# wendongbi/Bridged-GNN

Hardware: AMD Instinct MI355X
Metric: aggregated_edges_per_sec_ktgnn_fwd (higher is better)
Workload: dtype f32; 1 GPU; C4 synthetic bridged graph (local) N=1000000 E'=20991058, 2-layer KT-GNN eval fwd F=128 hidden=128 C=2; parallelism=single, execution=eager launches

## Files before the change

### bridged_gnn_amd/_lib.py

```python
import ctypes as C
import os

import torch

_HERE = os.path.dirname(os.path.abspath(__file__))
SO_PATH = os.path.join(_HERE, "csrc", "libbgnn_hip.so")
_lib = None

_P, _I64, _I32, _F32, _SZ, _INT = C.c_void_p, C.c_int64, C.c_int32, C.c_float, C.c_size_t, C.c_int

SIGNATURES = {
    "bgnn_version": (_INT, []),
    "bgnn_source_hash": (C.c_char_p, []),
    "bgnn_error_string": (C.c_char_p, [_INT]),
    "bgnn_csr_workspace_bytes": (_SZ, [_I64, _I64]),
    "bgnn_build_dst_csr": (_INT, [_P, _I64, _I64, _INT, _P, _P, _P, _P, _P, _SZ, _P]),
    "bgnn_domain_sums_f64": (_INT, [_P, _I64, _I32, _I64, _P, _P, _P]),
    "bgnn_domain_sums_workspace_bytes": (_SZ, [_I32]),
    "bgnn_domain_sums_ws_f64": (_INT, [_P, _I64, _I32, _I64, _P, _P, _P, _SZ, _P]),
    "bgnn_domain_delta_f32": (_INT, [_P, _I32, _P, _P]),
    "bgnn_adaptedconv_transform_f32": (_INT, [_P, _I64, _I32, _I64, _P, _P, _I32, _I32, _P, _P, _P, _P,
                                               _P, _P, _P, _P, _I64, _I64, _P, _P]),
    "bgnn_adaptedconv_transform_sums_f32": (_INT, [_P, _I64, _I32, _I64, _P, _P, _I32, _I32, _P, _P, _P, _P,
                                                    _P, _P, _P, _P, _I64, _I64, _I64, _I64, _P, _P]),
    "bgnn_adaptedconv_transform_need_f32": (_INT, [_P, _I64, _I32, _I64, _P, _P, _I32, _I32, _P, _P, _P, _P,
                                                    _P, _P, _P, _P, _I64, _I64, _P, _P, _P]),
    "bgnn_classifier_stage_f32": (_INT, [_P, _I64, _I32, _I64, _P, _P, _I32, _I32, _P, _P, _P, _P, _P, _P, _P, _P, _I64, _I64,
                                          _P, _P, _I32, _INT, _P, _P, _P, _P, _P, _P]),
    "bgnn_linear_narrow_transform_f32": (_INT, [_P, _I64, _I32, _I64, _P, _P, _I32, _INT, _P, _P, _P, _P, _P, _P]),
    "bgnn_narrow_transform_finish_f32": (_INT, [_P, _I64, _P, _P, _I32, _P, _P, _P, _P, _P, _P, _I64, _P, _P]),
    "bgnn_gram_workspace_bytes": (C.c_size_t, [_I32, _I32]),
    "bgnn_gram_f32": (_INT, [_P, _I64, _I32, _P, _I64, _I32, _I64, _P, _P, C.c_size_t, _P]),
    "bgnn_transform_bwd_prep_workspace_bytes": (C.c_size_t, [_I64, _I32]),
    "bgnn_transform_bwd_prep_f32": (_INT, [_P, _I64, _I64, _I32, _P, _P, _I64, _I32, _P, _P, _P, _P, _P, _P, _I32, _I64, _P, _I64, _P, _P, C.c_size_t, _P]),
    "bgnn_bn_acc_doubles": (_I64, [_I32]),
    "bgnn_bn_relu_dropout_f32": (_INT, [_P, _I64, _I32, _I64, _P, _P, _F32, _INT, _F32, C.c_uint64, _P, _F32, _P, _P, _P, _I64, _P, _P]),
    "bgnn_bn_relu_dropout_bwd_f32": (_INT, [_P, _P, _I64, _I32, _I64, _I64, _P, _P, _P, _F32, _INT, _F32, C.c_uint64, _P, _P, _I64, _P, _P]),
    "bgnn_bn_colstats_f32": (_INT, [_P, _I64, _I32, _I64, _P, _P]),
    "bgnn_bn_apply_rows_f32": (_INT, [_P, _I64, _I32, _I64, _P, _I64, _P, _P, _F32, _INT, _F32, C.c_uint64, _P, _P, _I64, _F32, _P, _P, _P, _I64, _P]),
    "bgnn_bn_bwd_reduce_rows_f32": (_INT, [_P, _P, _I64, _I32, _I64, _I64, _P, _I64, _P, _P, _F32, _INT, _F32, C.c_uint64, _P, _P, _I64, _P, _P]),
    "bgnn_bn_bwd_apply_rows_f32": (_INT, [_P, _P, _I64, _I32, _I64, _I64, _P, _P, _I64, _P, _P, _F32, _INT, _F32, C.c_uint64, _P, _P, _I64, _P, _I64, _P]),
    "bgnn_transform_bwd_consts_f32": (_INT, [_P, _P, _P, _P, _P, _I32, _I32, _P, _P, _P, _P]),
    "bgnn_transform_bwd_finish_f32": (_INT, [_P, _P, _P, _P, _P, _P, _P, _I32, _I32, _I32, _P, _P, _P, _P, _P, _P, _P, _I64, _P]),
    "bgnn_rowdot_f32": (_INT, [_P, _I64, _I64, _I32, _P, _I64, _I32, _P, _P]),
    "bgnn_linear_f32": (_INT, [_P, _I64, _I32, _I64, _P, _P, _I32, _INT, _P, _P, _P, _I64, _P]),
    "bgnn_adaptedconv_aggregate_f32": (_INT, [_P, _P, _I64, _P, _P, _P, _P, _P, _I64, _I64, _I32, _F32,
                                               _P, _I64, _P, _P, _P, _INT, _P, _INT, _I64, _I32, _P, _P, _P]),
    "bgnn_adaptedconv_aggregate_bounded_f32": (_INT, [_P, _P, _I64, _P, _P, _P, _P, _P, _I64, _I64, _I32, _F32,
                                                       _P, _I64, _P, _P, _P, _INT, _P, _INT, _I64, _I32, _P, _P, _I64, _I32, _P]),
    "bgnn_aggregate_hub_workspace_bytes": (C.c_size_t, [_I64, _I32, _I64]),
    "bgnn_adaptedconv_aggregate_hub_f32": (_INT, [_P, _P, _I64, _P, _P, _P, _P, _P, _I64, _I32, _F32, _P, _I64, _P, _P, _INT, _P, _I32, _P,
                                                   _P, _I32, _P, _I64, _P, _P, _P, _I64, _P, _P, C.c_size_t, _P]),
    "bgnn_adaptedconv_aggregate_bwd_f32": (_INT, [_P, _P, _I64, _P, _P, _P, _P, _P, _I64, _I64, _I32, _F32,
                                                   _P, _I64, _P, _P, _I64, _P, _P, _P, _P, _P]),
    "bgnn_aggregate_bwd_pull_workspace_bytes": (C.c_size_t, [_I64, _I64, _I64]),
    "bgnn_adaptedconv_aggregate_bwd_pull_f32": (_INT, [_P, _P, _I64, _P, _P, _P, _P, _P, _P, _P, _P, _I64, _I64, _I32, _F32,
                                                        _P, _I64, _P, _P, _I64, _P, _P, _P, _P, _P, C.c_size_t, _P]),
    "bgnn_aggregate_bwd_pull_hub_workspace_bytes": (C.c_size_t, [_I64, _I64, _I64, _I64, _I64]),
    "bgnn_adaptedconv_aggregate_bwd_pull_hub_f32": (_INT, [_P, _P, _I64, _P, _P, _P, _P, _P, _P, _P, _P, _I64, _I64, _I32, _F32,
                                                            _P, _I64, _P, _P, _I64, _P, _P, _P, _P, _I32,
                                                            _P, _I64, _P, _P, _P, _I64, _P, _I64, _P, _P, _P, _I64, _P, C.c_size_t, _P]),
    "bgnn_aggregate_heads_bwd_workspace_bytes": (C.c_size_t, [_I64, _I64, _I32]),
    "bgnn_adaptedconv_aggregate_heads_bwd_f32": (_INT, [_P, _P, _P, _P, _P, _P, _P, _P, _P, _P, _I64, _I64, _I32, _I32, _F32,
                                                         _P, _P, _P, _INT, _P, _P, _P, _P, _P, C.c_size_t, _P]),
    "bgnn_aggregate_heads_bwd_hub_workspace_bytes": (C.c_size_t, [_I64, _I64, _I32, _I64, _I64]),
    "bgnn_adaptedconv_aggregate_heads_bwd_hub_f32": (_INT, [_P, _P, _P, _P, _P, _P, _P, _P, _P, _I64, _I64, _I32, _I32, _F32,
                                                             _P, _P, _P, _INT, _P, _P, _P, _P, _I32,
                                                             _P, _I64, _P, _P, _P, _I64, _P, _I64, _P, _P, _P, _I64, _P, C.c_size_t, _P]),
    "bgnn_adaptedconv_aggregate_heads_wide_f32": (_INT, [_P, _P, _I64, _P, _P, _P, _P, _P, _I64, _I32, _I32, _F32, _P, _P, _P]),
    "bgnn_aggregate_heads_wide_bwd_workspace_bytes": (C.c_size_t, [_I64, _I32, _I64]),
    "bgnn_adaptedconv_aggregate_heads_wide_bwd_f32": (_INT, [_P, _P, _I64, _P, _P, _P, _P, _P, _P, _P, _I64, _I32, _I32, _F32,
                                                              _P, _P, _P, _P, _P, _P, _P, _P, C.c_size_t, _P]),
    "bgnn_l2_normalize_rows_f32": (_INT, [_P, _I64, _I32, _F32, _P, _P]),
    "bgnn_topk_workspace_bytes": (_SZ, [_I64, _I64, _I32]),
    "bgnn_cosine_topk_f32": (_INT, [_P, _P, _I64, _I64, _I32, _I32, _INT, _P, _P, _P, _P, _SZ, _P]),
    "bgnn_mlp_pair_topk_f32": (_INT, [_P, _P, _P, _P, _P, _F32, _I64, _I64, _I32, _I32, _INT, _P, _P, _P,
                                       _P, _SZ, _P]),
    "bgnn_topk_edges_i64": (_INT, [_P, _I64, _I32, _I64, _I64, _P, _P]),
    "bgnn_topk_edges_coalesced_workspace_bytes": (_SZ, [_I64, _I32]),
    "bgnn_topk_edges_coalesced_i64": (_INT, [_P, _I64, _I32, _I64, _I64, _I64, _P, _P, _SZ, _P]),
    "bgnn_gather_rows_f32": (_INT, [_P, _I64, _I64, _P, _I64, _I32, _P, _I64, _P]),
    "bgnn_coalesce_workspace_bytes": (_SZ, [_I64]),
    "bgnn_coalesce_i64": (_INT, [_P, _I64, _I64, _P, _P, _SZ, _P]),
    "bgnn_sage_mean_aggregate_f32": (_INT, [_P, _I64, _I64, _P, _I64, _P, _P, _I64, _I32, _INT, _INT, _F32, C.c_uint64, _P,
                                             _P, _I64, _P]),
    "bgnn_sage_mean_aggregate_rows_f32": (_INT, [_P, _I64, _I64, _P, _I64, _P, _P, _I64, _I32, _INT, _INT, _F32, C.c_uint64, _P,
                                                  _P, _P, _I64, _P]),
    "bgnn_rows_segment_add_f32": (_INT, [_P, _I64, _I64, _P, _P, _P, _I64, _I32, _INT, _P, _I64, _I64, _P]),
    "bgnn_pair_mlp_workspace_bytes": (_SZ, [_I64]),
    "bgnn_pair_mlp_stats_f32": (_INT, [_P, _I64, _I64, _P, _I64, _I64, _P, _P, _I64, _F32, _P, _P, _P, _P, _SZ, _P]),
    "bgnn_pair_mlp_loss_f32": (_INT, [_P, _I64, _I64, _P, _I64, _I64, _P, _P, _P, _I64, _P, _P, _P, _P, _P, _F32, _P, _P, _P, _P,
                                       _SZ, _P]),
    "bgnn_pair_mlp_segsum_f32": (_INT, [_P, _I64, _I64, _P, _I64, _I64, _P, _P, _P, _I64, _P, _P, _P, _P, _P, _P, _F32, _P, _I64, _P]),
    "bgnn_pair_mlp_eval_f32": (_INT, [_P, _I64, _I64, _P, _I64, _I64, _P, _P, _P, _I64, _P, _P, _P, _P, _P, _P, _P, _SZ, _P]),
    "bgnn_pair_mlp_count_workspace_bytes": (_SZ, [_I64, _I64]),
    "bgnn_pair_mlp_count_f32": (_INT, [_P, _I64, _I64, _P, _I64, _I64, _P, _I64, _P, _I64, _P, _P, _P, _P, _P, _P, _P, _P, _SZ, _P]),
    "bgnn_pair_cos_loss_workspace_bytes": (_SZ, [_I64]),
    "bgnn_pair_cos_count_workspace_bytes": (_SZ, [_I64, _I64]),
    "bgnn_pair_cos_loss_f32": (_INT, [_P, _I64, _I64, _P, _I64, _I64, _P, _P, _P, _I64, _P, _P, _P, _P, _SZ, _P]),
    "bgnn_pair_cos_segsum_f32": (_INT, [_P, _I64, _I64, _P, _P, _P, _I64, _P, _I64, _P, _I64, _P]),
    "bgnn_pair_cos_count_f32": (_INT, [_P, _I64, _I64, _P, _I64, _I64, _P, _I64, _P, _I64, _P, _P, _P, _P, _SZ, _P]),
    "bgnn_sage_mean_aggregate_bwd_workspace_bytes": (_SZ, [_I64, _I32]),
# ... 138 lines not shown
```

### bridged_gnn_amd/csrc/bgnn_aggregate.hip

```cpp
#include <cstdlib>
#include "bgnn_common.h"

namespace {

struct AggParams {
  const float* h_t2s;
  const float* h_s2t;
  int64_t ldh;
  const float* a_t2s;
  const float* a_s2t;
  const int32_t* rowptr;
  const int32_t* col;
  const uint8_t* mask;
  int64_t row_begin;
  int64_t row_end;
  int32_t D;
  float slope;
  float* out;
  int64_t ldo;
  float* alpha;
  const float* ep_scale;
  const float* ep_shift;
  int ep_relu;
  unsigned int* tile_queue;
  double* colsum;
  int32_t heads;
  float* state_ms;
  int mode;
  int64_t park_begin;
  int tq_chunk;
  int tq_interleave;
  int xcd_segments;
  const int32_t* vrow_node;
  const int32_t* vrow_bounds;
  int64_t n_vrows;
  float* vout; float* vms;
  int32_t hub_threshold;
  const char* tbl_base;
  uint32_t tbl_bytes, off_t2s, off_s2t;
  int32_t gather_hint;
  uint32_t dead_off;
};

__device__ __forceinline__ float leaky(float v, float slope) { return v > 0.f ? v : v * slope; }

template <int LF, int EP, int U>
__global__ __launch_bounds__(256) void agg_kernel(AggParams p) {
  constexpr int GL = LF * EP;
  constexpr int GPW = 64 / GL;
  constexpr int RPB = 4 * GPW;
  const int lane = threadIdx.x & 63;
  const int wave = threadIdx.x >> 6;
  const int g = lane / GL;
  const int lg = lane % GL;
  const int sub = lg / LF;
  const int f0 = (lg % LF) * 4;
  const bool fvalid = f0 < p.D;

  const int64_t ntiles = ((p.row_end - p.row_begin) * p.heads + RPB - 1) / RPB;
  bgnn::XcdRange tr = bgnn::xcd_pos_range(ntiles);
  __shared__ float red[2][LF * 4 + 1];
  if (p.colsum != nullptr) {
    for (int t = threadIdx.x; t < 2 * (LF * 4 + 1); t += 256) (&red[0][0])[t] = 0.f;
    __syncthreads();
  }

  __shared__ unsigned int dyn_tile;
  const int64_t xbase = tr.begin - (blockIdx.x / 8);
  int64_t tile = tr.begin - tr.step;
  int64_t chunk_left = 0;
  const int TQ_CHUNK = p.tq_chunk;
  for (;;) {
    if (p.tile_queue != nullptr) {
      if (chunk_left == 0) {
        __syncthreads();
        if (threadIdx.x == 0) dyn_tile = atomicAdd(&p.tile_queue[blockIdx.x % 8], 1u);
        __syncthreads();
        tile = xbase + (int64_t)dyn_tile * TQ_CHUNK;
        chunk_left = TQ_CHUNK;
      } else {
        tile += 1;
      }
      --chunk_left;
    } else {
      tile += tr.step;
    }
    if (tile >= tr.end) break;
    const int64_t gt = bgnn::xcd_tile_of(tile, ntiles);
    if (gt < 0) continue;
    const int64_t i = p.row_begin * p.heads + gt * RPB + wave * GPW + g;
    const bool rvalid = i < p.row_end * p.heads;
    const int64_t ic = rvalid ? i : p.row_begin * p.heads;
    const int64_t node = ic / p.heads;
    const int head = (int)(ic - node * p.heads);
    const bool dom_s = p.mask[node] != 0;
// ... 76 lines not shown
    }

#pragma unroll
    for (int off = LF; off < GL; off <<= 1) {
      const float m2 = __shfl_xor(m, off);
      const float s2 = __shfl_xor(s, off);
      float4 b;
      b.x = __shfl_xor(acc.x, off); b.y = __shfl_xor(acc.y, off);
      b.z = __shfl_xor(acc.z, off); b.w = __shfl_xor(acc.w, off);
      const float mn = fmaxf(m, m2);
      const float c1 = (m == mn) ? 1.f : __expf(m - mn);
      const float c2 = (m2 == mn) ? 1.f : __expf(m2 - mn);
      s = s * c1 + s2 * c2;
      acc.x = acc.x * c1 + b.x * c2; acc.y = acc.y * c1 + b.y * c2;
      acc.z = acc.z * c1 + b.z * c2; acc.w = acc.w * c1 + b.w * c2;
      m = mn;
    }

    if (p.mode == 1 && node >= p.park_begin) {
      if (rvalid && sub == 0) {
        if (lg == 0) { p.state_ms[2 * i] = m; p.state_ms[2 * i + 1] = s; }
        if (f0 < p.ldo) *reinterpret_cast<float4*>(p.out + i * p.ldo + f0) = fvalid ? acc : make_float4(0.f, 0.f, 0.f, 0.f);
      }
      continue;
    }
    const float inv = 1.f / (s + 1e-16f);
    if (p.alpha != nullptr && (lg % LF) == 0) {
      for (int32_t e = beg + sub; e < end; e += EP) p.alpha[e] = __expf(p.alpha[e] - m) * inv;
    }
    if (rvalid && sub == 0 && f0 < p.ldo) {
      float4 o = make_float4(acc.x * inv, acc.y * inv, acc.z * inv, acc.w * inv);
      if (p.ep_scale != nullptr) {
        float sc4[4], sh4[4];
#pragma unroll
        for (int c = 0; c < 4; ++c) {
          const bool ok = f0 + c < p.D;
          sc4[c] = ok ? p.ep_scale[f0 + c] : 0.f;
          sh4[c] = ok ? p.ep_shift[f0 + c] : 0.f;
        }
        o.x = fmaf(o.x, sc4[0], sh4[0]); o.y = fmaf(o.y, sc4[1], sh4[1]);
        o.z = fmaf(o.z, sc4[2], sh4[2]); o.w = fmaf(o.w, sc4[3], sh4[3]);
      }
      if (p.ep_relu) { o.x = fmaxf(o.x, 0.f); o.y = fmaxf(o.y, 0.f); o.z = fmaxf(o.z, 0.f); o.w = fmaxf(o.w, 0.f); }
      if (!fvalid) o = make_float4(0.f, 0.f, 0.f, 0.f);
      *reinterpret_cast<float4*>(p.out + i * p.ldo + f0) = o;
      if (p.colsum != nullptr) {
        float* r = red[dom_s ? 0 : 1];
        unsafeAtomicAdd(&r[f0], o.x); unsafeAtomicAdd(&r[f0 + 1], o.y);
        unsafeAtomicAdd(&r[f0 + 2], o.z); unsafeAtomicAdd(&r[f0 + 3], o.w);
        if (lg == 0) unsafeAtomicAdd(&r[LF * 4], 1.f);
      }
    }
  }
  if (p.colsum != nullptr) {
    __syncthreads();
    for (int t = threadIdx.x; t < 2 * (LF * 4 + 1); t += 256) {
      const int d = t / (LF * 4 + 1), c = t % (LF * 4 + 1);
      const double sum = (double)red[d][c];
      if (c == LF * 4) unsafeAtomicAdd(&p.colsum[2 * p.ldo + d], sum);
      else if (c < p.ldo) unsafeAtomicAdd(&p.colsum[d * p.ldo + c], sum);
    }
  }
}

typedef float f2 __attribute__((ext_vector_type(2)));

template <int CTRL>
__device__ __forceinline__ int dpp_movi(int x) { return __builtin_amdgcn_update_dpp(0, x, CTRL, 0xF, 0xF, true); }

template <int K>
__device__ __forceinline__ float quad_bcast(float x) { return bgnn::dpp_mov<K * 0x55>(x); }
template <int K>
__device__ __forceinline__ int quad_bcasti(int x) { return dpp_movi<K * 0x55>(x); }

template <int CTRL>
__device__ __forceinline__ float bfly(bool hi_side, float t_lo, float t_hi) {
  const float keep = hi_side ? t_hi : t_lo;
  const float send = hi_side ? t_lo : t_hi;
  return keep + bgnn::dpp_mov<CTRL>(send);
}

template <int LF, int U>
__global__ __launch_bounds__(256) void agg_wide_kernel(AggParams p) {
  static_assert(LF == 16 || LF == 32 || LF == 64, "wide rows only");
  static_assert(U == 4 || U == 8, "U");
  constexpr int GPW = 64 / LF;
  constexpr int RPB = 4 * GPW;
  const int lane = threadIdx.x & 63;
  const int wave = threadIdx.x >> 6;
  const int g = lane / LF;
  const int lg = lane % LF;
  const int f0 = lg * 4;
  const bool fvalid = f0 < p.D;
  const int f0c = fvalid ? f0 : 0;
  const int k = lane & (U - 1);
  const bool b0 = lane & 1, b1 = lane & 2, b2 = lane & 4;

  const int64_t nrows_all = (p.row_end - p.row_begin) * p.heads + p.n_vrows;
  const int64_t ntiles = (nrows_all + RPB - 1) / RPB;
  bgnn::XcdRange tr = bgnn::xcd_tile_range(ntiles);
  __shared__ float red[2][LF * 4 + 1];
  if (p.colsum != nullptr) {
    for (int t = threadIdx.x; t < 2 * (LF * 4 + 1); t += 256) (&red[0][0])[t] = 0.f;
    __syncthreads();
  }
  __shared__ unsigned int dyn_tile;
// ... 169 lines not shown
      if constexpr (U == 8) {
        { const float w = quad_bcast<0>(ph); BGNN_ACC(4, w) }
        { const float w = quad_bcast<1>(ph); BGNN_ACC(5, w) }
        { const float w = quad_bcast<2>(ph); BGNN_ACC(6, w) }
        { const float w = quad_bcast<3>(ph); BGNN_ACC(7, w) }
      }
#undef BGNN_ACC
      m = mn;
    };
    auto slot_id = [&](int32_t e) { return e < end ? p.col[e] : -1; };

    int32_t e = beg + k;
    int32_t myid = slot_id(e);
    for (int32_t it = 0; it < niter; ++it) {
      float4 v[U];
      issue(v, myid);
      const int32_t nextid = slot_id(e + U);
      update(v, myid, e);
      e += U;
      myid = nextid;
    }
    s += bgnn::dpp_mov<0xB1>(s);
    s += bgnn::dpp_mov<0x4E>(s);
    if constexpr (U == 8) s += bgnn::dpp_mov<0x124>(s);

    if (virt || (p.mode == 1 && node >= p.park_begin)) {
      if (rvalid) {
        if (lg == 0) { msbase[2 * i] = m; msbase[2 * i + 1] = s; }
        if (f0 < p.ldo)
          *reinterpret_cast<float4*>(obase + i * p.ldo + f0) =
              fvalid ? make_float4(acc01.x, acc01.y, acc23.x, acc23.y) : make_float4(0.f, 0.f, 0.f, 0.f);
      }
      continue;
    }
    const float inv = 1.f / (s + 1e-16f);
    if (p.alpha != nullptr && lg < U) {
      for (int32_t e2 = beg + lg; e2 < end; e2 += U) p.alpha[e2] = __expf(p.alpha[e2] - m) * inv;
    }
    if (rvalid && f0 < p.ldo) {
      float4 o = make_float4(acc01.x * inv, acc01.y * inv, acc23.x * inv, acc23.y * inv);
      if (p.ep_scale != nullptr) {
        o.x = fmaf(o.x, sc4[0], sh4[0]); o.y = fmaf(o.y, sc4[1], sh4[1]);
        o.z = fmaf(o.z, sc4[2], sh4[2]); o.w = fmaf(o.w, sc4[3], sh4[3]);
      }
      if (p.ep_relu) { o.x = fmaxf(o.x, 0.f); o.y = fmaxf(o.y, 0.f); o.z = fmaxf(o.z, 0.f); o.w = fmaxf(o.w, 0.f); }
      if (!fvalid) o = make_float4(0.f, 0.f, 0.f, 0.f);
      *reinterpret_cast<float4*>(p.out + i * p.ldo + f0) = o;
      if (p.colsum != nullptr) {
        if (dom_s) { cs_s.x += o.x; cs_s.y += o.y; cs_s.z += o.z; cs_s.w += o.w; n_s += 1.f; }
        else       { cs_t.x += o.x; cs_t.y += o.y; cs_t.z += o.z; cs_t.w += o.w; n_t += 1.f; }
      }
    }
  }
  if (p.colsum != nullptr) {
    unsafeAtomicAdd(&red[0][f0], cs_s.x); unsafeAtomicAdd(&red[0][f0 + 1], cs_s.y);
    unsafeAtomicAdd(&red[0][f0 + 2], cs_s.z); unsafeAtomicAdd(&red[0][f0 + 3], cs_s.w);
    unsafeAtomicAdd(&red[1][f0], cs_t.x); unsafeAtomicAdd(&red[1][f0 + 1], cs_t.y);
    unsafeAtomicAdd(&red[1][f0 + 2], cs_t.z); unsafeAtomicAdd(&red[1][f0 + 3], cs_t.w);
    if (lg == 0) { unsafeAtomicAdd(&red[0][LF * 4], n_s); unsafeAtomicAdd(&red[1][LF * 4], n_t); }
    __syncthreads();
    for (int t = threadIdx.x; t < 2 * (LF * 4 + 1); t += 256) {
      const int d = t / (LF * 4 + 1), c = t % (LF * 4 + 1);
      const double sum = (double)red[d][c];
      if (c == LF * 4) unsafeAtomicAdd(&p.colsum[2 * p.ldo + d], sum);
      else if (c < p.ldo) unsafeAtomicAdd(&p.colsum[d * p.ldo + c], sum);
    }
  }
}

typedef unsigned int u32x4_t __attribute__((ext_vector_type(4)));

template <int CTRL>
__device__ __forceinline__ uint32_t dpp_movu(uint32_t x) { return (uint32_t)__builtin_amdgcn_update_dpp(0, (int)x, CTRL, 0xF, 0xF, true); }

template <int LF, bool ALPHA>
__global__ __launch_bounds__(256) void agg_wide_fast_kernel(AggParams p) {
  static_assert(LF == 16 || LF == 32 || LF == 64, "wide rows only");
  constexpr int U = 4;
  constexpr int GPW = 64 / LF;
  constexpr int RPB = 4 * GPW;
  const int lane = threadIdx.x & 63;
  const int wave = threadIdx.x >> 6;
  const int g = lane / LF;
  const int lg = lane % LF;
  const int f0 = lg * 4;
  const bool fvalid = f0 < p.D;
  const int f0c = fvalid ? f0 : 0;
  const int k = lane & (U - 1);
  const bool b0 = lane & 1, b1 = lane & 2;

  const int32_t row0 = (int32_t)p.row_begin, row1 = (int32_t)p.row_end;
  const int32_t ntiles = (row1 - row0 + RPB - 1) / RPB;
  __shared__ float red[2][LF * 4 + 1];
  if (p.colsum != nullptr) {
    for (int t = threadIdx.x; t < 2 * (LF * 4 + 1); t += 256) (&red[0][0])[t] = 0.f;
    __syncthreads();
  }
  __shared__ unsigned int dyn_tile;
  const uint32_t nstride = (uint32_t)(p.ldh * 4);
  const uint32_t ostride = (uint32_t)(p.ldo * 4);
  const __amdgpu_buffer_rsrc_t rt = __builtin_amdgcn_make_buffer_rsrc(const_cast<char*>(p.tbl_base), (short)0, (int)p.tbl_bytes, 0x00020000);
  const __amdgpu_buffer_rsrc_t ro = __builtin_amdgcn_make_buffer_rsrc(p.out, (short)0, (int)((uint32_t)row1 * ostride), 0x00020000);
  const f2 sl = {p.slope, p.slope};
  float sc4[4] = {0.f, 0.f, 0.f, 0.f}, sh4[4] = {0.f, 0.f, 0.f, 0.f};
  if (p.ep_scale != nullptr) {
#pragma unroll
// ... 132 lines not shown
    int32_t nw = __builtin_amdgcn_readlane(niter, 0);
    if constexpr (LF <= 32) nw = max(nw, __builtin_amdgcn_readlane(niter, 32));
    if constexpr (LF <= 16) nw = max(nw, max(__builtin_amdgcn_readlane(niter, 16), __builtin_amdgcn_readlane(niter, 48)));
    int32_t e = beg + k;
    bool ok = e < end;
    uint32_t myoff = p.dead_off;
    if (nw > 0) myoff = row_off((uint32_t)p.col[max(min(e, end - 1), 0)], ok);
    for (int32_t it = 0; it < nw; ++it) {
      float4 v[U];
      issue(v, myoff);
      const int32_t e_cur = e;
      e += U;
      const bool ok2 = e < end;
      uint32_t nextid = load_id(e);
      update(v, ok, e_cur);
      ok = ok2;
      take_id(nextid);
      myoff = row_off(nextid, ok);
    }
    s += bgnn::dpp_mov<0xB1>(s);
    s += bgnn::dpp_mov<0x4E>(s);

    const float inv = 1.f / (s + 1e-16f);
    if constexpr (ALPHA) {
      if (lg < U) {
        for (int32_t e2 = beg + lg; e2 < end; e2 += 4 * U) {
          float a[4];
#pragma unroll
          for (int j = 0; j < 4; ++j) a[j] = e2 + j * U < end ? p.alpha[e2 + j * U] : 0.f;
#pragma unroll
          for (int j = 0; j < 4; ++j)
            if (e2 + j * U < end) p.alpha[e2 + j * U] = __expf(a[j] - m) * inv;
        }
      }
    }
    if (rvalid && f0 < p.ldo) {
      float4 o = make_float4(acc01.x * inv, acc01.y * inv, acc23.x * inv, acc23.y * inv);
      if (p.ep_scale != nullptr) {
        o.x = fmaf(o.x, sc4[0], sh4[0]); o.y = fmaf(o.y, sc4[1], sh4[1]);
        o.z = fmaf(o.z, sc4[2], sh4[2]); o.w = fmaf(o.w, sc4[3], sh4[3]);
      }
      if (p.ep_relu) { o.x = fmaxf(o.x, 0.f); o.y = fmaxf(o.y, 0.f); o.z = fmaxf(o.z, 0.f); o.w = fmaxf(o.w, 0.f); }
      if (!fvalid) o = make_float4(0.f, 0.f, 0.f, 0.f);
      __builtin_amdgcn_raw_buffer_store_b128(__builtin_bit_cast(u32x4_t, o), ro, __umul24((uint32_t)i0, ostride) + (uint32_t)f0 * 4u, 0, 0);
      if (p.colsum != nullptr) {
        const float ws = dom_s ? 1.f : 0.f, wt = dom_s ? 0.f : 1.f;
        const f2 ws2 = {ws, ws}, wt2 = {wt, wt}, o01 = {o.x, o.y}, o23 = {o.z, o.w};
        cs_s01 = __builtin_elementwise_fma(o01, ws2, cs_s01); cs_s23 = __builtin_elementwise_fma(o23, ws2, cs_s23);
        cs_t01 = __builtin_elementwise_fma(o01, wt2, cs_t01); cs_t23 = __builtin_elementwise_fma(o23, wt2, cs_t23);
        n_s += ws; n_t += wt;
      }
    }
  }
  if (p.colsum != nullptr) {
    unsafeAtomicAdd(&red[0][f0], cs_s01.x); unsafeAtomicAdd(&red[0][f0 + 1], cs_s01.y);
    unsafeAtomicAdd(&red[0][f0 + 2], cs_s23.x); unsafeAtomicAdd(&red[0][f0 + 3], cs_s23.y);
    unsafeAtomicAdd(&red[1][f0], cs_t01.x); unsafeAtomicAdd(&red[1][f0 + 1], cs_t01.y);
    unsafeAtomicAdd(&red[1][f0 + 2], cs_t23.x); unsafeAtomicAdd(&red[1][f0 + 3], cs_t23.y);
    if (lg == 0) { unsafeAtomicAdd(&red[0][LF * 4], n_s); unsafeAtomicAdd(&red[1][LF * 4], n_t); }
    __syncthreads();
    for (int t = threadIdx.x; t < 2 * (LF * 4 + 1); t += 256) {
      const int d = t / (LF * 4 + 1), c = t % (LF * 4 + 1);
      const double sum = (double)red[d][c];
      if (c == LF * 4) unsafeAtomicAdd(&p.colsum[2 * p.ldo + d], sum);
      else if (c < p.ldo) unsafeAtomicAdd(&p.colsum[d * p.ldo + c], sum);
    }
  }
}

template <int HEADS, int EP, int U>
__global__ __launch_bounds__(256) void agg_heads_lanes_kernel(AggParams p) {
  constexpr int GL = EP * HEADS, GPW = 64 / GL, RPB = 4 * GPW;
  const int lane = threadIdx.x & 63, wave = threadIdx.x >> 6;
  const int g = lane / GL, lg = lane % GL;
  const int sub = lg / HEADS, h = lg % HEADS;
  const bool lane_on = g < GPW;
  const int64_t ntiles = (p.row_end - p.row_begin + p.n_vrows + RPB - 1) / RPB;
  bgnn::XcdRange tr = bgnn::xcd_pos_range(ntiles);
  const int64_t rs = (int64_t)HEADS * p.ldh;
  for (int64_t pos = tr.begin; pos < tr.end; pos += tr.step) {
    const int64_t tile = bgnn::xcd_tile_of(pos, ntiles);
    if (tile < 0) continue;
    const int64_t i = p.row_begin + tile * RPB + wave * GPW + g;
    const bool in_range = lane_on && i < p.row_end + p.n_vrows;
    const bool virt = in_range && i >= p.row_end;
    const int64_t vix = virt ? i - p.row_end : 0;
    const int64_t ic = in_range ? i : p.row_begin;
    const int64_t node = virt ? (int64_t)p.vrow_node[vix] : ic;
    const bool dom_s = p.mask[node] != 0;
    const float* __restrict__ H = dom_s ? p.h_t2s : p.h_s2t;
    const float* __restrict__ av = dom_s ? p.a_t2s : p.a_s2t;
    int32_t beg = in_range ? (virt ? p.vrow_bounds[2 * vix] : p.rowptr[ic]) : 0;
    int32_t end = in_range ? (virt ? p.vrow_bounds[2 * vix + 1] : p.rowptr[ic + 1]) : 0;
    const bool hub = !virt && p.hub_threshold > 0 && end - beg >= p.hub_threshold;
    const bool rvalid = in_range && !hub;
    const int64_t oi = virt ? vix : i;
    float* __restrict__ obase = virt ? p.vout : p.out;
    float* __restrict__ msbase = virt ? p.vms : p.state_ms;
    if (hub) { beg = 0; end = 0; }
    float4 a4;
    a4.x = av[h * p.D];
    a4.y = p.D > 1 ? av[h * p.D + 1] : 0.f;
    a4.z = p.D > 2 ? av[h * p.D + 2] : 0.f;
    a4.w = p.D > 3 ? av[h * p.D + 3] : 0.f;
    const float4 hi = *reinterpret_cast<const float4*>(H + node * rs + h * p.ldh);
    float4 acc = make_float4(0.f, 0.f, 0.f, 0.f);
// ... 349 lines not shown
    r.y = p.D > 1 ? r.y - mx - lse : 0.f;
    r.z = p.D > 2 ? r.z - mx - lse : 0.f;
    r.w = p.D > 3 ? r.w - mx - lse : 0.f;
  }
  *reinterpret_cast<float4*>(p.out + (node * p.heads + h) * p.ldo) = r;
}

static int dispatch_aggregate(const AggParams& p, hipStream_t st, int64_t table_rows = 0) {
  const int32_t D = p.D, heads = p.heads;
  if (heads == 3 && D <= 4 && p.ldh == 4 && p.ldo == 4) return launch_heads<3, 2, 4>(p, st);
  if (heads == 2 && D <= 4 && p.ldh == 4 && p.ldo == 4) return launch_heads<2, 2, 4>(p, st);
  const int nv = (D + 3) / 4;
  if (nv <= 1) return launch<1, 4, 4>(p, st);
  if (nv <= 2) return launch<2, 2, 4>(p, st);
  if (nv <= 4) return launch<4, 1, 8>(p, st);
  if (nv <= 8) return launch<8, 1, 4>(p, st);
  const bool wide_ok = p.slope >= 0.f && p.slope <= 1.f && (int64_t)heads * p.ldh * 4 < (int64_t)1 << 32;
  if (wide_ok) {
    AggParams q = p;
    if (fast_plan(q, table_rows)) {
      if (q.alpha != nullptr) {
        if (nv <= 16) return launch_wide_fast<16, true>(q, st);
        if (nv <= 32) return launch_wide_fast<32, true>(q, st);
        return launch_wide_fast<64, true>(q, st);
      }
      if (nv <= 16) return launch_wide_fast<16, false>(q, st);
      if (nv <= 32) return launch_wide_fast<32, false>(q, st);
      return launch_wide_fast<64, false>(q, st);
    }
    if (nv <= 16) return launch_wide<16, 4>(p, st);
    if (nv <= 32) return launch_wide<32, 4>(p, st);
    return launch_wide<64, 4>(p, st);
  }
  if (nv <= 16) return launch<16, 1, 8>(p, st);
  if (nv <= 32) return launch<32, 1, 4>(p, st);
  return launch<64, 1, 4>(p, st);
}

static bool hub_capable(int32_t D, int64_t ldh, int64_t ldo, int32_t heads, float slope) {
  if ((heads == 3 || heads == 2) && D <= 4 && ldh == 4 && ldo == 4) return true;
  const int nv = (D + 3) / 4;
  return heads == 1 && nv > 8 && slope >= 0.f && slope <= 1.f && ldh * 4 < (int64_t)1 << 32;
}

}

static int aggregate_impl(const float* h_t2s, const float* h_s2t, int64_t ldh,
                          const float* a_t2s, const float* a_s2t,
                          const int32_t* rowptr, const int32_t* col, const uint8_t* mask,
                          int64_t row_begin, int64_t row_end, int32_t D, float negative_slope,
                          float* out, int64_t ldo, float* alpha_opt,
                          const float* ep_scale_opt, const float* ep_shift_opt, int ep_relu,
                          float* state_ms_opt, int part, int64_t park_begin, int32_t heads,
                          double* colsum_opt, uint32_t* tile_queue_opt, int64_t table_rows, int32_t gather_hint, void* stream) {
  if (colsum_opt && heads != 1) return BGNN_E_SHAPE;
  if (part == 1 && (park_begin < row_begin || park_begin > row_end)) return BGNN_E_SHAPE;
  if (part < 0 || part > 3 || (part != 0 && (!state_ms_opt || alpha_opt))) return BGNN_E_NULL;
  if (part == 3 && !((heads == 3 || heads == 2) && D <= 4 && ldh == 4 && ldo == 4)) return BGNN_E_SHAPE;
  if (heads < 1 || heads > 8 || (heads > 1 && (alpha_opt || ep_scale_opt))) return BGNN_E_SHAPE;
  if (ep_relu < 0 || ep_relu > 2) return BGNN_E_SHAPE;
  if (ep_relu == 2 && !((heads == 3 || heads == 2) && D <= 4 && ldh == 4 && ldo == 4)) return BGNN_E_SHAPE;
  if (!h_t2s || !h_s2t || !a_t2s || !a_s2t || !rowptr || !col || !mask || !out) return BGNN_E_NULL;
  if (row_begin < 0 || row_end < row_begin || D <= 0 || D > 256 || ldh < D || ldo < D) return BGNN_E_SHAPE;
  if ((ldh & 3) || (ldo & 3) || !bgnn_aligned16(h_t2s) || !bgnn_aligned16(h_s2t) || !bgnn_aligned16(out))
    return BGNN_E_ALIGN;
  if ((ep_scale_opt == nullptr) != (ep_shift_opt == nullptr)) return BGNN_E_NULL;
  if (row_end == row_begin) return 0;
  AggParams p{h_t2s, h_s2t, ldh, a_t2s, a_s2t, rowptr, col, mask, row_begin, row_end, D, negative_slope,
              out, ldo, alpha_opt, ep_scale_opt, ep_shift_opt, ep_relu, tile_queue_opt, colsum_opt, heads, state_ms_opt, part,
              park_begin, 4};
  p.gather_hint = gather_hint;
  hipStream_t st = (hipStream_t)stream;
  if (tile_queue_opt) {
    hipError_t e = bgnn_zero_async(tile_queue_opt, 8 * sizeof(uint32_t), st);
    if (e != hipSuccess) return (int)e;
  }
  return dispatch_aggregate(p, st, table_rows);
}

extern "C" int bgnn_adaptedconv_aggregate_f32(const float* h_t2s, const float* h_s2t, int64_t ldh,
                                              const float* a_t2s, const float* a_s2t,
                                              const int32_t* rowptr, const int32_t* col, const uint8_t* mask,
                                              int64_t row_begin, int64_t row_end, int32_t D, float negative_slope,
                                              float* out, int64_t ldo, float* alpha_opt,
                                              const float* ep_scale_opt, const float* ep_shift_opt, int ep_relu,
                                              float* state_ms_opt, int part, int64_t park_begin, int32_t heads,
                                              double* colsum_opt, uint32_t* tile_queue_opt, void* stream) {
  return aggregate_impl(h_t2s, h_s2t, ldh, a_t2s, a_s2t, rowptr, col, mask, row_begin, row_end, D, negative_slope, out, ldo, alpha_opt,
                        ep_scale_opt, ep_shift_opt, ep_relu, state_ms_opt, part, park_begin, heads, colsum_opt, tile_queue_opt, 0, 0, stream);
}

extern "C" int bgnn_adaptedconv_aggregate_bounded_f32(const float* h_t2s, const float* h_s2t, int64_t ldh,
                                                      const float* a_t2s, const float* a_s2t,
                                                      const int32_t* rowptr, const int32_t* col, const uint8_t* mask,
                                                      int64_t row_begin, int64_t row_end, int32_t D, float negative_slope,
                                                      float* out, int64_t ldo, float* alpha_opt,
                                                      const float* ep_scale_opt, const float* ep_shift_opt, int ep_relu,
                                                      float* state_ms_opt, int part, int64_t park_begin, int32_t heads,
                                                      double* colsum_opt, uint32_t* tile_queue_opt, int64_t table_rows, int32_t gather_hint,
                                                      void* stream) {
  if (table_rows < row_end || gather_hint < 0 || gather_hint > 2) return BGNN_E_SHAPE;
  return aggregate_impl(h_t2s, h_s2t, ldh, a_t2s, a_s2t, rowptr, col, mask, row_begin, row_end, D, negative_slope, out, ldo, alpha_opt,
                        ep_scale_opt, ep_shift_opt, ep_relu, state_ms_opt, part, park_begin, heads, colsum_opt, tile_queue_opt, table_rows, gather_hint, stream);
}

extern "C" size_t bgnn_aggregate_hub_workspace_bytes(int64_t n_segments, int32_t heads, int64_t ldo) {
  const size_t nv = (size_t)(n_segments > 0 ? n_segments : 0), h = (size_t)(heads > 0 ? heads : 1);
  return bgnn_align_up(sizeof(float) * nv * h * (size_t)(ldo > 0 ? ldo : 0), 256) + bgnn_align_up(sizeof(float) * 2 * nv * h, 256) + 256;
}

extern "C" int bgnn_adaptedconv_aggregate_hub_f32(const float* h_t2s, const float* h_s2t, int64_t ldh,
                                                  const float* a_t2s, const float* a_s2t,
                                                  const int32_t* rowptr, const int32_t* col, const uint8_t* mask,
                                                  int64_t N, int32_t D, float negative_slope, float* out, int64_t ldo,
                                                  const float* ep_scale_opt, const float* ep_shift_opt, int ep_relu,
                                                  float* state_ms_opt, int32_t heads, double* colsum_opt,
                                                  uint32_t* tile_queue_opt, int32_t hub_threshold, const int32_t* hub_rows,
                                                  int64_t n_hubs, const int32_t* hub_seg_ptr, const int32_t* seg_bounds,
                                                  const int32_t* seg_node, int64_t n_segments, float* alpha_opt,
                                                  void* ws, size_t ws_bytes, void* stream) {
  if (!h_t2s || !h_s2t || !a_t2s || !a_s2t || !rowptr || !col || !mask || !out) return BGNN_E_NULL;
  if (alpha_opt && heads != 1) return BGNN_E_SHAPE;
  if (n_hubs > 0 && (!hub_rows || !hub_seg_ptr || !seg_bounds || !seg_node || !ws)) return BGNN_E_NULL;
  if (N < 0 || D <= 0 || D > 256 || ldh < D || ldo < D || (ldh & 3) || (ldo & 3) || hub_threshold < 2 || n_hubs < 0 || n_segments < n_hubs)
    return BGNN_E_SHAPE;
  if (!hub_capable(D, ldh, ldo, heads, negative_slope)) return BGNN_E_SHAPE;
  if (colsum_opt && heads != 1) return BGNN_E_SHAPE;
  if (heads > 1 && ep_scale_opt) return BGNN_E_SHAPE;
  if (ep_relu < 0 || ep_relu > 2 || (ep_relu == 2 && heads == 1)) return BGNN_E_SHAPE;
  if ((ep_scale_opt == nullptr) != (ep_shift_opt == nullptr)) return BGNN_E_NULL;
  if (!bgnn_aligned16(h_t2s) || !bgnn_aligned16(h_s2t) || !bgnn_aligned16(out) || (ws && !bgnn_aligned16(ws))) return BGNN_E_ALIGN;
  if (n_hubs > 0 && ws_bytes < bgnn_aggregate_hub_workspace_bytes(n_segments, heads, ldo)) return BGNN_E_WORKSPACE;
  if (N == 0) return 0;
  hipStream_t st = (hipStream_t)stream;
  const int part = (state_ms_opt && heads > 1) ? 3 : 0;
  AggParams p{h_t2s, h_s2t, ldh, a_t2s, a_s2t, rowptr, col, mask, 0, N, D, negative_slope,
              out, ldo, alpha_opt, ep_scale_opt, ep_shift_opt, ep_relu, tile_queue_opt, colsum_opt, heads, state_ms_opt, part,
              0, 4};
  p.hub_threshold = n_hubs > 0 ? hub_threshold : 0;
  if (tile_queue_opt) {
    hipError_t e = bgnn_zero_async(tile_queue_opt, 8 * sizeof(uint32_t), st);
    if (e != hipSuccess) return (int)e;
  }
  float* part_acc = n_hubs > 0 ? (float*)ws : nullptr;
  float* part_ms = n_hubs > 0 ? (float*)((char*)ws + bgnn_align_up(sizeof(float) * (size_t)n_segments * (size_t)heads * (size_t)ldo, 256)) : nullptr;
  if (n_hubs > 0) {
    p.vrow_node = seg_node; p.vrow_bounds = seg_bounds; p.n_vrows = n_segments; p.vout = part_acc; p.vms = part_ms;
  }
  int rc = dispatch_aggregate(p, st, N);
  if (rc || n_hubs == 0) return rc;
  HubMergeParams mp{hub_rows, hub_seg_ptr, n_hubs, part_acc, part_ms, mask, D, ldo, heads, out, ep_scale_opt, ep_shift_opt,
                    ep_relu, colsum_opt, part == 3 ? state_ms_opt : nullptr, alpha_opt, rowptr};
  if (heads > 1) {
    hipLaunchKernelGGL(hub_merge_heads_kernel, dim3((unsigned)((n_hubs * heads + 255) / 256)), dim3(256), 0, st, mp);
  } else {
    const int nvs = (D + 3) / 4;
    int64_t grid = n_hubs < 2048 ? n_hubs : 2048;
    if (nvs <= 16) hipLaunchKernelGGL(hub_merge_wide_kernel<16>, dim3((unsigned)((grid + 15) / 16)), dim3(256), 0, st, mp);
    else if (nvs <= 32) hipLaunchKernelGGL(hub_merge_wide_kernel<32>, dim3((unsigned)((grid + 7) / 8)), dim3(256), 0, st, mp);
    else hipLaunchKernelGGL(hub_merge_wide_kernel<64>, dim3((unsigned)((grid + 3) / 4)), dim3(256), 0, st, mp);
  }
  BGNN_LAUNCH_CHECK();
  return 0;
}

#ifdef BGNN_TUNING
extern "C" int bgnn_tune_reset_counters(void* stream) { (void)stream; return 0; }
extern "C" int bgnn_tune_aggregate(const float* h_t2s, const float* h_s2t, int64_t ldh, const float* a_t2s,
                                   const float* a_s2t, const int32_t* rowptr, const int32_t* col, const uint8_t* mask,
                                   int64_t row_begin, int64_t row_end, int32_t D, float slope, float* out, int64_t ldo,
                                   int variant, uint32_t* tile_queue, void* stream) {
  AggParams p{h_t2s, h_s2t, ldh, a_t2s, a_s2t, rowptr, col, mask, row_begin, row_end, D, slope,
              out, ldo, nullptr, nullptr, nullptr, 0, tile_queue, nullptr, 1, nullptr, 0};
  hipStream_t st = (hipStream_t)stream;
  if (tile_queue && bgnn_zero_async(tile_queue, 32, st) != hipSuccess) return -1;
  switch (variant) {
    case 40: return launch_wide<32, 4>(p, st);
    case 41: return launch_wide<32, 8>(p, st);
    case 42: return launch_wide<16, 4>(p, st);
    case 43: return launch_wide<16, 8>(p, st);
    case 44: return launch_wide<64, 4>(p, st);
    case 45: return launch_wide<64, 8>(p, st);
    case 0: return launch<32, 1, 4>(p, st);
    case 1: return launch<32, 1, 8>(p, st);
    case 2: return launch<32, 2, 4>(p, st);
    case 3: return launch<32, 2, 2>(p, st);
    case 4: return launch<32, 1, 2>(p, st);
    case 5: return launch<32, 2, 8>(p, st);
    case 6: return launch<64, 1, 4>(p, st);
    case 10: return launch<1, 8, 2>(p, st);
    case 11: return launch<1, 4, 4>(p, st);
    case 12: return launch<1, 2, 4>(p, st);
    case 13: return launch<1, 1, 4>(p, st);
    case 14: return launch<1, 1, 8>(p, st);
    case 15: return launch<1, 4, 2>(p, st);
    case 16: return launch<1, 2, 8>(p, st);
    case 17: return launch<1, 16, 2>(p, st);
    case 20: return launch<16, 2, 4>(p, st);
    case 21: return launch<16, 1, 4>(p, st);
    case 22: return launch<16, 4, 2>(p, st);
    case 23: return launch<16, 1, 8>(p, st);
    case 30: return launch<8, 2, 4>(p, st);
    case 31: return launch<8, 4, 2>(p, st);
    case 32: return launch<8, 1, 4>(p, st);
    case 33: return launch<8, 8, 2>(p, st);
    default: return BGNN_E_RANGE;
  }
}
#endif
```

### bridged_gnn_amd/csrc/bgnn_transform.hip

```cpp
#include <cstdlib>
#include <type_traits>
#include "bgnn_common.h"
#include "bgnn_transform_params.h"

using bgnn_tf::GemmParams;
using bgnn_tf::MAXH;
using bgnn_tf::f32x16;
using bgnn_tf::tanh_fast;

namespace {

constexpr int DS_NT = 1024;
__global__ __launch_bounds__(DS_NT) void domain_sums_kernel(const float* __restrict__ x, int64_t N, int32_t Din,
                                                          int64_t ldx, const uint8_t* __restrict__ mask,
                                                          double* __restrict__ sums, double* __restrict__ part) {
  if (part != nullptr) sums = part + (int64_t)blockIdx.x * (2 * Din + 2);
  const int nc4 = Din >> 2;
  const int cw = nc4 < 256 ? nc4 : 256;
  const int rl = DS_NT / cw;
  const int tid = threadIdx.x;
  const int cl = tid % cw, r0 = tid / cw;
  const bool active = r0 < rl;
  const int64_t rows_per_block = (N + gridDim.x - 1) / gridDim.x;
  const int64_t rb = blockIdx.x * rows_per_block;
  const int64_t re = min(rb + rows_per_block, N);
  extern __shared__ double sh[];
  for (int cb = 0; cb < nc4; cb += cw) {
    const int c4 = cb + cl;
    const bool cok = active && c4 < nc4;
    double as[4] = {0, 0, 0, 0}, at[4] = {0, 0, 0, 0};
    if (cok) {
      int64_t r = rb + r0;
      for (; r + 3 * rl < re; r += 4 * rl) {
        float4 v[4];
        bool m[4];
#pragma unroll
        for (int u = 0; u < 4; ++u) {
          v[u] = *reinterpret_cast<const float4*>(x + (r + u * rl) * ldx + c4 * 4);
          m[u] = mask[r + u * rl] != 0;
        }
#pragma unroll
        for (int u = 0; u < 4; ++u) {
          const double a = v[u].x, b = v[u].y, c = v[u].z, d = v[u].w;
          if (m[u]) { as[0] += a; as[1] += b; as[2] += c; as[3] += d; }
          else      { at[0] += a; at[1] += b; at[2] += c; at[3] += d; }
        }
      }
      for (; r < re; r += rl) {
        const float4 v = *reinterpret_cast<const float4*>(x + r * ldx + c4 * 4);
        if (mask[r]) { as[0] += v.x; as[1] += v.y; as[2] += v.z; as[3] += v.w; }
        else         { at[0] += v.x; at[1] += v.y; at[2] += v.z; at[3] += v.w; }
      }
    }
    if (active) {
#pragma unroll
      for (int e = 0; e < 4; ++e) { sh[((r0 * 2 + 0) * cw + cl) * 4 + e] = as[e]; sh[((r0 * 2 + 1) * cw + cl) * 4 + e] = at[e]; }
    }
    __syncthreads();
    if (cok && r0 == 0) {
      for (int q = 1; q < rl; ++q)
#pragma unroll
// ... 720 lines not shown
  hipStream_t st = (hipStream_t)stream;
  if (ws != nullptr) {
    if (ws_bytes < sizeof(double) * 256 * (size_t)ncol) return BGNN_E_WORKSPACE;
    int64_t grid = (N + 255) / 256;
    if (grid > 256) grid = 256;
    hipLaunchKernelGGL(domain_sums_kernel, dim3((unsigned)grid), dim3(DS_NT), sizeof(double) * rl * 2 * cw * 4, st,
                       x, N, Din, ldx, mask, sums_io, (double*)ws);
    BGNN_LAUNCH_CHECK();
    hipLaunchKernelGGL(domain_sums_reduce_kernel, dim3((unsigned)((ncol + 255) / 256)), dim3(256), 0, st,
                       (const double*)ws, (int)grid, ncol, sums_io);
    BGNN_LAUNCH_CHECK();
    return 0;
  }
  static const int64_t rpb = [] { const char* e = getenv("BGNN_DS_ROWS"); return e ? atoll(e) : 2048ll; }();
  int64_t grid = (N + rpb - 1) / rpb;
  static const int64_t gcap = [] { const char* e = getenv("BGNN_DS_GRID"); return e ? atoll(e) : 256ll; }();
  if (grid > gcap) grid = gcap;
  if (grid < 1) grid = 1;
  hipLaunchKernelGGL(domain_sums_kernel, dim3((unsigned)grid), dim3(DS_NT), sizeof(double) * rl * 2 * cw * 4, st,
                     x, N, Din, ldx, mask, sums_io, (double*)nullptr);
  BGNN_LAUNCH_CHECK();
  return 0;
}

extern "C" int bgnn_domain_sums_f64(const float* x, int64_t N, int32_t Din, int64_t ldx, const uint8_t* mask,
                                    double* sums_io, void* stream) {
  return domain_sums_impl(x, N, Din, ldx, mask, sums_io, nullptr, 0, stream);
}

extern "C" size_t bgnn_domain_sums_workspace_bytes(int32_t Din) {
  return Din > 0 ? sizeof(double) * 256 * (size_t)(2 * Din + 2) : 0;
}

extern "C" int bgnn_domain_sums_ws_f64(const float* x, int64_t N, int32_t Din, int64_t ldx, const uint8_t* mask,
                                       double* sums_io, void* ws, size_t ws_bytes, void* stream) {
  if (!ws) return BGNN_E_NULL;
  return domain_sums_impl(x, N, Din, ldx, mask, sums_io, ws, ws_bytes, stream);
}

extern "C" int bgnn_domain_delta_f32(const double* sums, int32_t Din, float* delta, void* stream) {
  if (!sums || !delta) return BGNN_E_NULL;
  if (Din <= 0) return BGNN_E_SHAPE;
  hipLaunchKernelGGL(domain_delta_kernel, dim3((Din + 255) / 256), dim3(256), 0, (hipStream_t)stream, sums, Din, delta);
  BGNN_LAUNCH_CHECK();
  return 0;
}

static int transform_impl(const float* x, int64_t N, int32_t Din, int64_t ldx,
                          const uint8_t* mask, const float* delta, const double* sums,
                          int32_t n_heads, int32_t D, const float* Wp, const float* bias_p,
                          const float* gates, const float* gate_const_opt,
                          float* h_s2t_0, float* h_t2s_0, float* h_s2t_1, float* h_t2s_1,
                          int64_t ldh, int64_t row_stride, float* small_ws, void* stream,
                          int64_t n_tail_t2s = 0, int64_t n_tail_s2t = 0, const int32_t* tile_need = nullptr) {
  if (n_tail_t2s < 0 || n_tail_s2t < 0 || n_tail_t2s + n_tail_s2t > N) return BGNN_E_SHAPE;
  if (!x || !mask || (!delta && !sums) || !Wp || !bias_p || !gates || !h_s2t_0 || !h_t2s_0 || !small_ws) return BGNN_E_NULL;
  if (n_heads < 1 || n_heads > MAXH || (n_heads == 2 && (!h_s2t_1 || !h_t2s_1))) return BGNN_E_NULL;
  if (N < 0 || Din <= 0 || D <= 0 || ldx < Din || ldh < D) return BGNN_E_SHAPE;
  if ((Din & 3) || (ldx & 3) || (ldh & 3) || (row_stride & 3) || row_stride < ldh) return BGNN_E_SHAPE;
  if (!bgnn_aligned16(x) || !bgnn_aligned16(Wp) || !bgnn_aligned16(gates)) return BGNN_E_ALIGN;
  if (N == 0) return 0;
  hipStream_t st = (hipStream_t)stream;
  const int NC = n_heads * 2 * (int)ldh;
  float* wd = small_ws;
  float* gc = small_ws + NC;
  hipLaunchKernelGGL(wd_kernel, dim3((unsigned)((NC + 2 * n_heads + 3) / 4)), dim3(256), 0, st, Wp, NC, Din, delta, sums, gates,
                     gate_const_opt, n_heads, wd, gc);
  BGNN_LAUNCH_CHECK();
  GemmParams p{};
  p.x = x; p.ldx = ldx; p.N = N; p.Din = Din; p.mask = mask; p.Wp = Wp; p.bias = bias_p; p.wd = wd; p.g = gates; p.gc = gc;
  p.out[0][0] = h_s2t_0; p.out[0][1] = h_t2s_0; p.out[1][0] = h_s2t_1; p.out[1][1] = h_t2s_1;
  p.ldh = ldh; p.row_stride = row_stride; p.NC = NC; p.n_heads = n_heads; p.relu = 0; p.colsum = nullptr; p.col_off = 0;
  const int64_t nrt = (N + BM - 1) / BM;
  const int64_t nrt8 = (nrt + 7) / 8 * 8;
  static const int n_cu = [] {
    int dev = 0; hipDeviceProp_t prop;
    return (hipGetDevice(&dev) == hipSuccess && hipGetDeviceProperties(&prop, dev) == hipSuccess) ? prop.multiProcessorCount : 256;
  }();
  static const bool use_wreg = [] { const char* e = getenv("BGNN_GEMM_WREG"); return !e || atoi(e) != 0; }();
  p.tail_t2s_begin = 0; p.tail_s2t_begin = 0;
  if ((n_tail_t2s || n_tail_s2t) && use_wreg && n_heads == 1 && NC % 64 == 0 && Din <= 128) {
    p.tail_t2s_begin = N - n_tail_t2s - n_tail_s2t;
    p.tail_s2t_begin = N - n_tail_s2t;
    if (p.tail_s2t_begin == 0) p.tail_s2t_begin = 1, p.tail_t2s_begin = p.tail_t2s_begin > 1 ? 1 : p.tail_t2s_begin;
  }
  static const bool use_stream = [] { const char* e = getenv("BGNN_GEMM_STREAM"); return !e || atoi(e) != 0; }();
  p.tile_need = tile_need;
  if (use_stream && bgnn_tf_stream_supported(p, 0)) return bgnn_tf_stream_launch(p, 0, st, n_cu);
  if (use_wreg && NC % 64 == 0 && Din <= 128) {
    const int nct = NC % 256 == 0 ? 8 : NC % 128 == 0 ? 4 : 2;
    const int nw = nct == 2 ? 4 : 8;
    const int bmw = 32 * (nw / nct);
    const int64_t ntiles = (N + bmw - 1) / bmw;
    const int ncg = (NC + 32 * nct - 1) / (32 * nct);
    const int64_t gx = (int64_t)n_cu * (nw == 4 ? 2 : 1);
    const dim3 grid((unsigned)(ntiles < gx ? ntiles : gx), (unsigned)ncg);
    static const bool bf3 = [] { const char* e = getenv("BGNN_GEMM_BF3"); return !e || atoi(e) != 0; }();
#define BGNN_WREG(DK, NCT, NW) do { if (bf3 && NCT >= 4) hipLaunchKernelGGL((transform_wreg_kernel<DK, NCT, NW, true, 0>), grid, dim3(64 * NW), 0, st, p); \
                                     else hipLaunchKernelGGL((transform_wreg_kernel<DK, NCT, NW, false, 0>), grid, dim3(64 * NW), 0, st, p); } while (0)
#define BGNN_WREG_DK(NCT, NW) do { if (Din <= 64) BGNN_WREG(64, NCT, NW); else BGNN_WREG(128, NCT, NW); } while (0)
    if (nct == 2) BGNN_WREG_DK(2, 4); else if (nct == 4) BGNN_WREG_DK(4, 8); else BGNN_WREG_DK(8, 8);
#undef BGNN_WREG_DK
#undef BGNN_WREG
  } else if (use_wreg && NC <= 24 && Din <= 128) {
    const int64_t nt = (N + 31) / 32, nb = (nt + 3) / 4;
    const unsigned grid = (unsigned)(nb < 2 * n_cu ? nb : 2 * n_cu);
    if (Din <= 64) hipLaunchKernelGGL((transform_skinny_kernel<64>), dim3(grid), dim3(256), 0, st, p);
    else hipLaunchKernelGGL((transform_skinny_kernel<128>), dim3(grid), dim3(256), 0, st, p);
  } else if (NC <= 32) {
    hipLaunchKernelGGL((transform_gemm_kernel<32, 4, 1, 1, 1>), dim3((unsigned)nrt8), dim3(256), 0, st, p);
  } else if (NC <= 64) {
    hipLaunchKernelGGL((transform_gemm_kernel<64, 2, 2, 2, 1>), dim3((unsigned)nrt8), dim3(256), 0, st, p);
  } else {
    const int nct = (NC + 127) / 128;
    hipLaunchKernelGGL((transform_gemm_kernel<128, 2, 2, 2, 2>), dim3((unsigned)(nrt8 * nct)), dim3(256), 0, st, p);
  }
  BGNN_LAUNCH_CHECK();
  return 0;
}

extern "C" int bgnn_adaptedconv_transform_f32(const float* x, int64_t N, int32_t Din, int64_t ldx,
                                              const uint8_t* mask, const float* delta,
                                              int32_t n_heads, int32_t D, const float* Wp, const float* bias_p,
                                              const float* gates, const float* gate_const_opt,
                                              float* h_s2t_0, float* h_t2s_0, float* h_s2t_1, float* h_t2s_1,
                                              int64_t ldh, int64_t row_stride, float* small_ws, void* stream) {
  if (!delta) return BGNN_E_NULL;
  if (!bgnn_aligned16(delta)) return BGNN_E_ALIGN;
  return transform_impl(x, N, Din, ldx, mask, delta, nullptr, n_heads, D, Wp, bias_p, gates, gate_const_opt,
                        h_s2t_0, h_t2s_0, h_s2t_1, h_t2s_1, ldh, row_stride, small_ws, stream);
}

extern "C" int bgnn_adaptedconv_transform_sums_f32(const float* x, int64_t N, int32_t Din, int64_t ldx,
                                                   const uint8_t* mask, const double* sums,
                                                   int32_t n_heads, int32_t D, const float* Wp, const float* bias_p,
                                                   const float* gates, const float* gate_const_opt,
                                                   float* h_s2t_0, float* h_t2s_0, float* h_s2t_1, float* h_t2s_1,
                                                   int64_t ldh, int64_t row_stride, int64_t n_tail_t2s, int64_t n_tail_s2t,
                                                   float* small_ws, void* stream) {
  if (!sums) return BGNN_E_NULL;
  return transform_impl(x, N, Din, ldx, mask, nullptr, sums, n_heads, D, Wp, bias_p, gates, gate_const_opt,
                        h_s2t_0, h_t2s_0, h_s2t_1, h_t2s_1, ldh, row_stride, small_ws, stream, n_tail_t2s, n_tail_s2t);
}

extern "C" int bgnn_adaptedconv_transform_need_f32(const float* x, int64_t N, int32_t Din, int64_t ldx,
                                                   const uint8_t* mask, const double* sums,
                                                   int32_t n_heads, int32_t D, const float* Wp, const float* bias_p,
                                                   const float* gates, const float* gate_const_opt,
                                                   float* h_s2t_0, float* h_t2s_0, float* h_s2t_1, float* h_t2s_1,
                                                   int64_t ldh, int64_t row_stride, const int32_t* tile_need_opt,
                                                   float* small_ws, void* stream) {
  if (!sums) return BGNN_E_NULL;
  return transform_impl(x, N, Din, ldx, mask, nullptr, sums, n_heads, D, Wp, bias_p, gates, gate_const_opt,
                        h_s2t_0, h_t2s_0, h_s2t_1, h_t2s_1, ldh, row_stride, small_ws, stream, 0, 0, tile_need_opt);
}

extern "C" int bgnn_linear_f32(const float* x, int64_t N, int32_t Din, int64_t ldx, const float* W, const float* bias,
                               int32_t Dout, int relu, const uint8_t* mask_opt, double* colsum_opt,
                               float* out, int64_t ldo, void* stream) {
  if (!x || !W || !bias || !out || (colsum_opt && !mask_opt)) return BGNN_E_NULL;
  if (N < 0 || Din <= 0 || Din > 128 || (Din & 3) || (ldx & 3) || ldx < Din || Dout <= 0 || (Dout & 63) || ldo < Dout || (ldo & 3))
    return BGNN_E_SHAPE;
  if (!bgnn_aligned16(x) || !bgnn_aligned16(W) || !bgnn_aligned16(bias) || !bgnn_aligned16(out)) return BGNN_E_ALIGN;
  if (N == 0) return 0;
  hipStream_t st = (hipStream_t)stream;
  GemmParams p{};
  p.x = x; p.ldx = ldx; p.N = N; p.Din = Din; p.mask = mask_opt; p.Wp = W; p.bias = bias; p.wd = nullptr; p.g = nullptr; p.gc = nullptr;
  p.out[0][0] = out; p.out[0][1] = out; p.out[1][0] = out; p.out[1][1] = out;
  p.ldh = Dout;
  p.row_stride = ldo; p.NC = Dout; p.n_heads = 1; p.relu = relu; p.colsum = colsum_opt;
  static const int n_cu = [] {
    int dev = 0; hipDeviceProp_t prop;
    return (hipGetDevice(&dev) == hipSuccess && hipGetDeviceProperties(&prop, dev) == hipSuccess) ? prop.multiProcessorCount : 256;
  }();
  const int nct = Dout % 256 == 0 ? 8 : Dout % 128 == 0 ? 4 : 2;
  const int nw = nct == 2 ? 4 : 8;
  const int bmw = 32 * (nw / nct);
  const int64_t ntiles = (N + bmw - 1) / bmw;
  const int64_t gx = (int64_t)n_cu * (nw == 4 ? 2 : 1);
  const dim3 grid((unsigned)(ntiles < gx ? ntiles : gx), (unsigned)(Dout / (32 * nct)));
#define BGNN_LIN(DK, NCT, NW, BF) hipLaunchKernelGGL((transform_wreg_kernel<DK, NCT, NW, BF, 1>), grid, dim3(64 * NW), 0, st, p)
#define BGNN_LIN_DK(NCT, NW, BF) do { if (Din <= 64) BGNN_LIN(64, NCT, NW, BF); else BGNN_LIN(128, NCT, NW, BF); } while (0)
  if (nct == 2) BGNN_LIN_DK(2, 4, false); else if (nct == 4) BGNN_LIN_DK(4, 8, true); else BGNN_LIN_DK(8, 8, true);
#undef BGNN_LIN_DK
#undef BGNN_LIN
  BGNN_LAUNCH_CHECK();
  return 0;
}

namespace {
__global__ __launch_bounds__(256) void narrow_finish_kernel(const float* __restrict__ raw, int64_t N,
                                                            const uint8_t* __restrict__ mask,
                                                            const float* __restrict__ bias, const float* __restrict__ wd,
                                                            const float* __restrict__ gc, float* __restrict__ out_s2t,
                                                            float* __restrict__ out_t2s, int64_t row_stride) {
  const float4 b0 = *reinterpret_cast<const float4*>(bias), b1 = *reinterpret_cast<const float4*>(bias + 4);
  const float4 w0 = *reinterpret_cast<const float4*>(wd), w1 = *reinterpret_cast<const float4*>(wd + 4);
  const float g0 = gc[0], g1 = gc[1];
  for (int64_t r = blockIdx.x * (int64_t)blockDim.x + threadIdx.x; r < N; r += (int64_t)gridDim.x * blockDim.x) {
    const float4 a = *reinterpret_cast<const float4*>(raw + r * 12);
    const float4 b = *reinterpret_cast<const float4*>(raw + r * 12 + 4);
    const float2 pg = *reinterpret_cast<const float2*>(raw + r * 12 + 8);
    const bool sdom = mask[r] != 0;
    const float c0 = sdom ? -tanh_fast(pg.x + g0) : 0.f;
    const float c1 = sdom ? 0.f : tanh_fast(pg.y + g1);
    float4 o0, o1;
    o0.x = fmaf(c0, w0.x, a.x + b0.x); o0.y = fmaf(c0, w0.y, a.y + b0.y);
    o0.z = fmaf(c0, w0.z, a.z + b0.z); o0.w = fmaf(c0, w0.w, a.w + b0.w);
    o1.x = fmaf(c1, w1.x, b.x + b1.x); o1.y = fmaf(c1, w1.y, b.y + b1.y);
    o1.z = fmaf(c1, w1.z, b.z + b1.z); o1.w = fmaf(c1, w1.w, b.w + b1.w);
    *reinterpret_cast<float4*>(out_s2t + r * row_stride) = o0;
    *reinterpret_cast<float4*>(out_t2s + r * row_stride) = o1;
  }
}
}

extern "C" int bgnn_linear_narrow_transform_f32(const float* x, int64_t N, int32_t Din, int64_t ldx, const float* W,
                                                const float* bias, int32_t Dout, int relu, const uint8_t* mask,
                                                double* colsum, const float* Wp2, const float* gates2,
                                                float* raw, void* stream) {
  if (!x || !W || !bias || !mask || !colsum || !Wp2 || !gates2 || !raw) return BGNN_E_NULL;
  if (N < 0 || Din <= 0 || Din > 128 || (Din & 3) || (ldx & 3) || ldx < Din || (Dout != 64 && Dout != 128 && Dout != 256))
    return BGNN_E_SHAPE;
  if (!bgnn_aligned16(x) || !bgnn_aligned16(W) || !bgnn_aligned16(bias) || !bgnn_aligned16(raw)) return BGNN_E_ALIGN;
  if (N == 0) return 0;
  hipStream_t st = (hipStream_t)stream;
  GemmParams p{};
  p.x = x; p.ldx = ldx; p.N = N; p.Din = Din; p.mask = mask; p.Wp = W; p.bias = bias;
  p.ldh = Dout; p.row_stride = Dout; p.NC = Dout; p.n_heads = 1; p.relu = relu ? 1 : 0; p.colsum = colsum;
  p.w2 = Wp2; p.g2 = gates2; p.raw = raw;
  static const int n_cu = [] {
    int dev = 0; hipDeviceProp_t prop;
    return (hipGetDevice(&dev) == hipSuccess && hipGetDeviceProperties(&prop, dev) == hipSuccess) ? prop.multiProcessorCount : 256;
  }();
  static const bool use_stream2 = [] { const char* e = getenv("BGNN_GEMM_STREAM2"); return e && atoi(e) != 0; }();
  if (use_stream2 && bgnn_tf_stream_supported(p, 2)) return bgnn_tf_stream_launch(p, 2, st, n_cu);
  const int nct = Dout == 256 ? 8 : Dout == 128 ? 4 : 2;
  const int nw = nct == 2 ? 4 : 8;
  const int bmw = 32 * (nw / nct);
  const int64_t ntiles = (N + bmw - 1) / bmw;
  const int64_t gx = (int64_t)n_cu * (nw == 4 ? 2 : 1);
  const dim3 grid((unsigned)(ntiles < gx ? ntiles : gx), 1u);
#define BGNN_LIN2(DK, NCT, NW, BF) hipLaunchKernelGGL((transform_wreg_kernel<DK, NCT, NW, BF, 2>), grid, dim3(64 * NW), 0, st, p)
#define BGNN_LIN2_DK(NCT, NW, BF) do { if (Din <= 64) BGNN_LIN2(64, NCT, NW, BF); else BGNN_LIN2(128, NCT, NW, BF); } while (0)
  if (nct == 2) BGNN_LIN2_DK(2, 4, false); else if (nct == 4) BGNN_LIN2_DK(4, 8, true); else BGNN_LIN2_DK(8, 8, true);
#undef BGNN_LIN2_DK
#undef BGNN_LIN2
  BGNN_LAUNCH_CHECK();
  return 0;
}

extern "C" int bgnn_classifier_stage_f32(const float* x, int64_t N, int32_t Din, int64_t ldx, const uint8_t* mask,
                                         const double* sums_x, int32_t sk_heads, int32_t sk_D, const float* sk_Wp,
                                         const float* sk_bias, const float* sk_gates, const float* sk_gate_const_opt,
                                         float* h_s2t_0, float* h_t2s_0, float* h_s2t_1, float* h_t2s_1, int64_t sk_ldh,
                                         int64_t sk_row_stride, const float* W, const float* bias, int32_t Dout, int relu,
                                         double* colsum, const float* Wp2, const float* gates2, float* raw, float* small_ws,
                                         void* stream) {
  if (!x || !mask || !sums_x || !sk_Wp || !sk_bias || !sk_gates || !h_s2t_0 || !h_t2s_0 || !W || !bias || !colsum || !Wp2 || !gates2 ||
      !raw || !small_ws) return BGNN_E_NULL;
  if (sk_heads < 1 || sk_heads > MAXH || (sk_heads == 2 && (!h_s2t_1 || !h_t2s_1))) return BGNN_E_NULL;
  if (N < 0 || Din <= 0 || (Din & 3) || (ldx & 3) || ldx < Din || sk_D <= 0 || sk_ldh < sk_D || (sk_ldh & 3) || (sk_row_stride & 3) ||
      sk_row_stride < sk_ldh) return BGNN_E_SHAPE;
  if (!bgnn_aligned16(x) || !bgnn_aligned16(sk_Wp) || !bgnn_aligned16(sk_bias) || !bgnn_aligned16(raw) || !bgnn_aligned16(small_ws))
    return BGNN_E_ALIGN;
  if (N == 0) return 0;
  hipStream_t st = (hipStream_t)stream;
  const int sk_NC = sk_heads * 2 * (int)sk_ldh;
  float* wd = small_ws;
  float* gc = small_ws + sk_NC;
  GemmParams p{};
  p.x = x; p.ldx = ldx; p.N = N; p.Din = Din; p.mask = mask; p.Wp = W; p.bias = bias;
  p.ldh = Dout; p.row_stride = Dout; p.NC = Dout; p.n_heads = 1; p.relu = relu ? 1 : 0; p.colsum = colsum;
  p.w2 = Wp2; p.g2 = gates2; p.raw = raw;
  p.sk_Wp = sk_Wp; p.sk_bias = sk_bias; p.sk_wd = wd; p.sk_g = sk_gates; p.sk_gc = gc;
  p.sk_out[0][0] = h_s2t_0; p.sk_out[0][1] = h_t2s_0; p.sk_out[1][0] = h_s2t_1; p.sk_out[1][1] = h_t2s_1;
  p.sk_ldh = sk_ldh; p.sk_row_stride = sk_row_stride; p.sk_NC = sk_NC; p.sk_heads = sk_heads;
  if (!bgnn_tf_cls_supported(p)) return BGNN_E_SHAPE;
  hipLaunchKernelGGL(wd_kernel, dim3((unsigned)((sk_NC + 2 * sk_heads + 3) / 4)), dim3(256), 0, st, sk_Wp, sk_NC, Din, (const float*)nullptr,
                     sums_x, sk_gates, sk_gate_const_opt, sk_heads, wd, gc);
  BGNN_LAUNCH_CHECK();
  static const int n_cu = [] {
    int dev = 0; hipDeviceProp_t prop;
    return (hipGetDevice(&dev) == hipSuccess && hipGetDeviceProperties(&prop, dev) == hipSuccess) ? prop.multiProcessorCount : 256;
  }();
  return bgnn_tf_cls_launch(p, st, n_cu);
}

extern "C" int bgnn_narrow_transform_finish_f32(const float* raw, int64_t N, const uint8_t* mask, const double* sums,
                                                int32_t Din, const float* Wp2, const float* bias2, const float* gates2,
                                                const float* gate_const_opt, float* h_s2t, float* h_t2s,
                                                int64_t row_stride, float* small_ws, void* stream) {
  if (!raw || !mask || !sums || !Wp2 || !bias2 || !gates2 || !h_s2t || !h_t2s || !small_ws) return BGNN_E_NULL;
  if (N < 0 || Din <= 0 || (Din & 3) || row_stride < 4 || (row_stride & 3)) return BGNN_E_SHAPE;
  if (!bgnn_aligned16(raw) || !bgnn_aligned16(h_s2t) || !bgnn_aligned16(h_t2s) || !bgnn_aligned16(bias2) ||
      !bgnn_aligned16(small_ws)) return BGNN_E_ALIGN;
  if (N == 0) return 0;
  hipStream_t st = (hipStream_t)stream;
  float* wd = small_ws;
  float* gc = small_ws + 8;
  hipLaunchKernelGGL(wd_kernel, dim3(3), dim3(256), 0, st, Wp2, 8, Din, (const float*)nullptr, sums, gates2, gate_const_opt, 1, wd, gc);
  BGNN_LAUNCH_CHECK();
  const int64_t nb = (N + 255) / 256;
  hipLaunchKernelGGL(narrow_finish_kernel, dim3((unsigned)(nb < 4096 ? nb : 4096)), dim3(256), 0, st, raw, N, mask, bias2, wd, gc,
                     h_s2t, h_t2s, row_stride);
  BGNN_LAUNCH_CHECK();
  return 0;
}
```

### bridged_gnn_amd/csrc/bgnn_transform_cls.hip

```cpp
#include <cstdio>
#include <cstdlib>
#include "bgnn_common.h"
#include "bgnn_transform_params.h"

using bgnn_tf::GemmParams;
using bgnn_tf::MAXH;
using bgnn_tf::f32x16;
using bgnn_tf::tanh_fast;

namespace {

typedef _Float16 h8 __attribute__((ext_vector_type(8)));
typedef _Float16 h4 __attribute__((ext_vector_type(4)));

constexpr int CLS_TARGET_EXP = 10;
constexpr int DK = 128, KB16 = DK / 16, NCT = 4;
constexpr int PIECE = 32 * DK * 2;
constexpr int SLOT = 32 * 36 * 4 + 2 * 32 * 4;
constexpr int T_LD = 36;

__device__ __forceinline__ int chunk_off(int r, int c) { return r * 256 + ((c ^ (r & 15)) << 4); }
__device__ __forceinline__ void pow2_scales(float mx, float& sc, float& inv) {
  int E = (__builtin_bit_cast(int, mx) >> 23) & 0xff;
  E = E < 40 ? 40 : E;
  sc = __builtin_bit_cast(float, (127 + CLS_TARGET_EXP + 127 - E) << 23);
  inv = __builtin_bit_cast(float, (E - CLS_TARGET_EXP) << 23);
}

constexpr int CLS_NW = 4;

__global__ __launch_bounds__(64 * CLS_NW) void cls_stage_kernel(GemmParams p) {
  __shared__ __attribute__((aligned(16))) unsigned char wl[(NCT + 1) * 2 * PIECE];
  __shared__ __attribute__((aligned(16))) unsigned char slots[CLS_NW * SLOT];
  __shared__ __attribute__((aligned(16))) h8 w2lds[NCT][2][2][64];
  __shared__ __attribute__((aligned(16))) float skc[2][32];
  __shared__ __attribute__((aligned(16))) float bias1[DK];
  __shared__ uint32_t wmax[3];
  __shared__ float red[2][DK + 1];
  const int tid = threadIdx.x, lane = tid & 63;
  const int wave = __builtin_amdgcn_readfirstlane(tid >> 6);
  const int fr = lane & 31, fh = lane >> 5;
  const int NC = p.NC;
  const bool din_full = p.Din == DK;
#ifdef CLS_STAMP
  uint32_t st_acc[8] = {0, 0, 0, 0, 0, 0, 0, 0};
  uint32_t st_last = 0;
#define CLS_MARK(k) do { const uint32_t t__ = (uint32_t)__builtin_amdgcn_s_memtime(); st_acc[k] += t__ - st_last; st_last = t__; } while (0)
#else
#define CLS_MARK(k) do { } while (0)
#endif

  if (tid < 3) wmax[tid] = 0u;
  for (int t = tid; t < 2 * (DK + 1); t += 64 * CLS_NW) (&red[0][0])[t] = 0.f;
  if (tid < 32) { skc[0][tid] = tid < p.sk_NC ? p.sk_bias[tid] : 0.f; skc[1][tid] = tid < p.sk_NC ? p.sk_wd[tid] : 0.f; }
  if (tid < DK) bias1[tid] = tid < NC ? p.bias[tid] : 0.f;
  __syncthreads();
  auto src_row = [&](int ct, int r) -> const float* {
    if (ct < NCT) return (32 * ct + r) < NC ? p.Wp + (int64_t)(32 * ct + r) * p.Din : nullptr;
    if (r < p.sk_NC) return p.sk_Wp + (int64_t)r * p.Din;
    if (r >= 24 && ((r - 24) & 3) < 2 * p.sk_heads) return p.sk_g + (int64_t)((r - 24) & 3) * 2 * p.Din;
    return nullptr;
  };
  float mx1 = 0.f, mxs = 0.f;
  for (int it = tid; it < (NCT + 1) * 32 * 16; it += 64 * CLS_NW) {
    const int ct = it / 512, r = (it >> 4) & 31, c = it & 15;
    const float* s = src_row(ct, r);
    float m = 0.f;
    if (s != nullptr) {
#pragma unroll
      for (int e = 0; e < 8; ++e) { const int k = 8 * c + e; m = fmaxf(m, k < p.Din ? fabsf(s[k]) : 0.f); }
    }
    if (ct < NCT) mx1 = fmaxf(mx1, m); else mxs = fmaxf(mxs, m);
  }
  float w2v[NCT][16];
  float mx2 = 0.f;
#pragma unroll
  for (int ct = 0; ct < NCT; ++ct)
#pragma unroll
    for (int r = 0; r < 16; ++r) {
      const int c = 32 * ct + 8 * (r >> 2) + 4 * fh + (r & 3);
      float v = 0.f;
      if (c < NC) {
        if (fr < 8) v = p.w2[(int64_t)fr * NC + c];
        else if (fr < 10) v = p.g2[(int64_t)(fr - 8) * 2 * NC + c];
      }
      w2v[ct][r] = v;
      mx2 = fmaxf(mx2, fabsf(v));
    }
  mx1 = bgnn::group_max<64>(mx1); mxs = bgnn::group_max<64>(mxs); mx2 = bgnn::group_max<64>(mx2);
  if (lane == 0) {
    atomicMax(&wmax[0], __builtin_bit_cast(unsigned, mx1));
    atomicMax(&wmax[1], __builtin_bit_cast(unsigned, mxs));
    atomicMax(&wmax[2], __builtin_bit_cast(unsigned, mx2));
  }
  __syncthreads();
  float scW, cinvW, scS, cinvS, sc2w, cinv2;
  pow2_scales(__builtin_bit_cast(float, wmax[0]), scW, cinvW);
  pow2_scales(__builtin_bit_cast(float, wmax[1]), scS, cinvS);
  pow2_scales(__builtin_bit_cast(float, wmax[2]), sc2w, cinv2);
  for (int it = tid; it < (NCT + 1) * 32 * 16; it += 64 * CLS_NW) {
    const int ct = it / 512, r = (it >> 4) & 31, c = it & 15;
    const float* s = src_row(ct, r);
    const float sc = ct < NCT ? scW : scS;
    h8 hi, lo;
#pragma unroll
    for (int e = 0; e < 8; ++e) {
      const int k = 8 * c + e;
      const float v = (s != nullptr && k < p.Din) ? s[k] : 0.f;
      const _Float16 h = (_Float16)(v * sc);
      hi[e] = h;
      lo[e] = (_Float16)fmaf(v, sc, -(float)h);
    }
    unsigned char* base = wl + (ct * 2) * PIECE + chunk_off(r, c);
    *reinterpret_cast<h8*>(base) = hi;
    *reinterpret_cast<h8*>(base + PIECE) = lo;
  }
  if (wave == 0) {
#pragma unroll
    for (int ct = 0; ct < NCT; ++ct) {
      h8 hh[2], ll[2];
#pragma unroll
      for (int r = 0; r < 16; ++r) {
        const _Float16 h = (_Float16)(w2v[ct][r] * sc2w);
        hh[r >> 3][r & 7] = h;
        ll[r >> 3][r & 7] = (_Float16)fmaf(w2v[ct][r], sc2w, -(float)h);
      }
#pragma unroll
      for (int kb = 0; kb < 2; ++kb) { w2lds[ct][kb][0][lane] = hh[kb]; w2lds[ct][kb][1][lane] = ll[kb]; }
    }
  }
  __syncthreads();

  float* optr[3];
  int hsel[3];
#pragma unroll
  for (int q = 0; q < 3; ++q) {
    const int c = 8 * q + 4 * fh;
    optr[q] = nullptr; hsel[q] = 0;
    if (c < p.sk_NC) {
      const int ld2 = 2 * (int)p.sk_ldh;
      const int h = c / ld2, rem = c % ld2, t = rem >= p.sk_ldh ? 1 : 0;
      float* base = h == 0 ? (t == 0 ? p.sk_out[0][0] : p.sk_out[0][1]) : (t == 0 ? p.sk_out[1][0] : p.sk_out[1][1]);
      optr[q] = base + (rem - t * (int)p.sk_ldh);
      hsel[q] = h * 2 + t;
    }
  }
  float gcs[4];
#pragma unroll
  for (int h = 0; h < 4; ++h) gcs[h] = h < 2 * p.sk_heads ? p.sk_gc[h] : 0.f;

  unsigned char* const sb = slots + wave * SLOT;
  float* const tsc = reinterpret_cast<float*>(sb);
  float* const cfs = reinterpret_cast<float*>(sb + 32 * T_LD * 4);
  const int roff0 = chunk_off(fr, fh);
  auto roff = [&](int kb) { return roff0 ^ (kb << 5); };
  const int64_t ntiles = (p.N + 31) / 32;
  const int64_t stride = (int64_t)gridDim.x * CLS_NW;
  int64_t tile = (int64_t)blockIdx.x * CLS_NW + wave;
  float4 ra[KB16][2];
  uint8_t rmk = 0;
  auto gload = [&](int64_t tl) {
    int64_t r = tl * 32 + fr;
    r = r < p.N ? r : p.N - 1;
    const float* src = p.x + r * p.ldx;
#pragma unroll
    for (int kb = 0; kb < KB16; ++kb)
#pragma unroll
      for (int c = 0; c < 2; ++c) {
        const int k = 16 * kb + 8 * fh + 4 * c;
        ra[kb][c] = *reinterpret_cast<const float4*>(src + (din_full || k < p.Din ? k : 0));
      }
    rmk = p.mask[r];
  };
  float cs_s[NCT], cs_t[NCT], cnt_s = 0.f, cnt_t = 0.f;
#pragma unroll
  for (int ct = 0; ct < NCT; ++ct) cs_s[ct] = cs_t[ct] = 0.f;

  if (tile < ntiles) gload(tile);
  for (; tile < ntiles; tile += stride) {
    CLS_MARK(0);
    const bool sdom = rmk != 0;
    const int64_t row = tile * 32 + fr;
    const bool valid = row < p.N;
    float mx = 0.f;
#pragma unroll
    for (int kb = 0; kb < KB16; ++kb)
#pragma unroll
      for (int c = 0; c < 2; ++c) {
        if (!din_full && 16 * kb + 8 * fh + 4 * c >= p.Din) ra[kb][c] = make_float4(0.f, 0.f, 0.f, 0.f);
        mx = fmaxf(fmaxf(fabsf(ra[kb][c].x), fabsf(ra[kb][c].y)), mx);
        mx = fmaxf(fmaxf(fabsf(ra[kb][c].z), fabsf(ra[kb][c].w)), mx);
      }
    mx = fmaxf(mx, __shfl_xor(mx, 32));
    float scx, s_row;
    pow2_scales(mx, scx, s_row);
    h8 xh[KB16], xl[KB16];
#pragma unroll
    for (int kb = 0; kb < KB16; ++kb)
#pragma unroll
      for (int c = 0; c < 2; ++c) {
        const float f[4] = {ra[kb][c].x, ra[kb][c].y, ra[kb][c].z, ra[kb][c].w};
#pragma unroll
// ... 145 lines not shown
      } else {
#pragma unroll
        for (int j = 0; j < 8; ++j) stage2_step(q2, ct, j);
        CLS_MARK(7);
      }
    }
    if (valid) {
      float* rr = p.raw + row * 12;
      if (fh == 0) {
        *reinterpret_cast<float4*>(rr) = make_float4(o2[0], o2[1], o2[2], o2[3]);
        *reinterpret_cast<float4*>(rr + 8) = make_float4(o2[4], o2[5], 0.f, 0.f);
      } else {
        *reinterpret_cast<float4*>(rr + 4) = make_float4(o2[0], o2[1], o2[2], o2[3]);
      }
    }
  }
#ifdef CLS_STAMP
  if (lane == 0 && p.wd != nullptr) {
    float* o = const_cast<float*>(p.wd) + ((int64_t)blockIdx.x * CLS_NW + wave) * 8;
    for (int k = 0; k < 8; ++k) o[k] = (float)st_acc[k];
  }
  return;
#endif
  if (p.colsum != nullptr) {
#pragma unroll
    for (int ct = 0; ct < NCT; ++ct) {
      const float a = cs_s[ct] + __shfl_xor(cs_s[ct], 32), b = cs_t[ct] + __shfl_xor(cs_t[ct], 32);
      if (fh == 0) {
        unsafeAtomicAdd(&red[0][32 * ct + fr], a);
        unsafeAtomicAdd(&red[1][32 * ct + fr], b);
      }
    }
    {
      float a = cnt_s, b = cnt_t;
#pragma unroll
      for (int m = 32; m >= 1; m >>= 1) { a += __shfl_xor(a, m); b += __shfl_xor(b, m); }
      if (lane == 0) { unsafeAtomicAdd(&red[0][DK], a); unsafeAtomicAdd(&red[1][DK], b); }
    }
    __syncthreads();
    for (int t = tid; t < 2 * (DK + 1); t += 64 * CLS_NW) {
      const int d = t / (DK + 1), c = t % (DK + 1);
      const double v = (double)red[d][c];
      if (c == DK) unsafeAtomicAdd(&p.colsum[2 * NC + d], v);
      else if (c < NC) unsafeAtomicAdd(&p.colsum[d * NC + c], v);
    }
  }
}

}

bool bgnn_tf_cls_supported(const GemmParams& p) {
  if (p.NC != 128 || p.Din > 128 || p.Din <= 64 || (p.Din & 3) || !p.mask || !p.w2 || !p.g2 || !p.raw) return false;
  if (p.sk_NC < 0 || p.sk_NC > 24 || (p.sk_NC & 3) || p.sk_heads < 0 || p.sk_heads > 2) return false;
  if (p.sk_NC > 0 && (!p.sk_Wp || !p.sk_bias || !p.sk_wd || !p.sk_g || !p.sk_gc || (p.sk_ldh & 3) || p.sk_NC != p.sk_heads * 2 * p.sk_ldh)) return false;
  return true;
}

int bgnn_tf_cls_launch(const GemmParams& p, hipStream_t st, int n_cu) {
  if (!bgnn_tf_cls_supported(p)) return BGNN_E_SHAPE;
  const int64_t nt = (p.N + 31) / 32, nb = (nt + CLS_NW - 1) / CLS_NW;
#ifdef CLS_STAMP
  {
    GemmParams q = p;
    static float* dbuf = nullptr;
    if (!dbuf) (void)hipMalloc((void**)&dbuf, sizeof(float) * 256 * 8 * 8);
    q.wd = dbuf;
    const unsigned g = (unsigned)(nb < n_cu ? nb : n_cu);
    hipLaunchKernelGGL(cls_stage_kernel, dim3(g), dim3(64 * CLS_NW), 0, st, q);
    (void)hipDeviceSynchronize();
    static float host[256 * 8 * 8];
    (void)hipMemcpy(host, dbuf, sizeof(float) * g * CLS_NW * 8, hipMemcpyDeviceToHost);
    double acc[8] = {0};
    for (unsigned w = 0; w < g * CLS_NW; ++w) for (int k = 0; k < 8; ++k) acc[k] += host[w * 8 + k];
    const double d = (double)nt;
    fprintf(stderr, "[cls stamp] cycles per tile: loop %.0f convert %.0f skinny-chain %.0f skinny-epilogue %.0f first-chain %.0f activation(x4) %.0f chain+stage2(x3) %.0f last-stage2 %.0f\n",
            acc[0] / d, acc[1] / d, acc[2] / d, acc[3] / d, acc[4] / d, acc[5] / d, acc[6] / d, acc[7] / d);
    return 0;
  }
#endif
  hipLaunchKernelGGL(cls_stage_kernel, dim3((unsigned)(nb < n_cu ? nb : n_cu)), dim3(64 * CLS_NW), 0, st, p);
  BGNN_LAUNCH_CHECK();
  return 0;
}
```

### bridged_gnn_amd/csrc/bgnn_transform_params.h

```cpp
#pragma once
#include "bgnn_common.h"

namespace bgnn_tf {

typedef float f32x16 __attribute__((ext_vector_type(16)));
constexpr int MAXH = 2;

struct GemmParams {
  const float* x; int64_t ldx; int64_t N; int32_t Din;
  const uint8_t* mask;
  const float* Wp;
  const float* bias;
  const float* wd;
  const float* g;
  const float* gc;
  float* out[MAXH][2];
  int64_t ldh; int64_t row_stride; int32_t NC; int32_t n_heads;
  int32_t relu;
  double* colsum;
  int32_t col_off;
  const float* w2;
  const float* g2;
  float* raw;
  int64_t tail_t2s_begin, tail_s2t_begin;
  const int32_t* tile_need;
  const float* sk_Wp; const float* sk_bias; const float* sk_wd; const float* sk_g; const float* sk_gc;
  float* sk_out[MAXH][2]; int64_t sk_ldh; int64_t sk_row_stride; int32_t sk_NC; int32_t sk_heads;
};

__device__ __forceinline__ float tanh_fast(float z) { return 1.f - 2.f * __builtin_amdgcn_rcpf(__expf(2.f * z) + 1.f); }

}

int bgnn_tf_stream_launch(const bgnn_tf::GemmParams& p, int mode, hipStream_t st, int n_cu);
bool bgnn_tf_stream_supported(const bgnn_tf::GemmParams& p, int mode);

int bgnn_tf_cls_launch(const bgnn_tf::GemmParams& p, hipStream_t st, int n_cu);
bool bgnn_tf_cls_supported(const bgnn_tf::GemmParams& p);
```

### bridged_gnn_amd/csrc/bgnn_transform_stream.hip

```cpp
#include <cstdio>
#include <cstdlib>
#include "bgnn_common.h"
#include "bgnn_transform_params.h"

using bgnn_tf::GemmParams;
using bgnn_tf::f32x16;
using bgnn_tf::tanh_fast;

namespace {

typedef _Float16 h8 __attribute__((ext_vector_type(8)));
typedef _Float16 h4 __attribute__((ext_vector_type(4)));
typedef float f2 __attribute__((ext_vector_type(2)));
typedef unsigned int u32x4 __attribute__((ext_vector_type(4)));

#ifndef TS_SLOTS
#define TS_SLOTS 6
#endif
#ifndef TS_AHEAD
#define TS_AHEAD 2
#endif
#ifndef TS_DEPTH
#define TS_DEPTH 2
#endif
constexpr int TS_TARGET_EXP = 10;

__device__ __forceinline__ __amdgpu_buffer_rsrc_t make_rsrc(const void* base, int64_t bytes) {
  const int64_t cap = 0x7fffffff;
  const int nrec = (int)(bytes < 0 ? 0 : (bytes > cap ? cap : bytes));
  return __builtin_amdgcn_make_buffer_rsrc(const_cast<void*>(base), (short)0, nrec, 0x00020000);
}

template <int DK>
struct Slot {
  static constexpr int PIECE = 32 * DK * 2;
  static constexpr int COEF = 2 * PIECE;
  static constexpr int BYTES = COEF + 5 * 32 * 4;
  __device__ static __forceinline__ int chunk_off(int r, int c) {
    if constexpr (DK == 128) return r * 256 + ((c ^ (r & 15)) << 4);
    else return (r >> 1) * 256 + (((((r & 1) << 3) | c) ^ ((r >> 1) & 15)) << 4);
  }
};

__device__ __forceinline__ unsigned lds_addr(const void* p) {
  return (unsigned)(uintptr_t)(__attribute__((address_space(3))) const void*)p;
}
__device__ __forceinline__ void lds_inc(uint32_t* ctr) {
  if ((threadIdx.x & 63) == 0) asm volatile("ds_add_u32 %0, %1" :: "v"(lds_addr(ctr)), "v"(1u) : "memory");
}
__device__ __forceinline__ void lds_arrive(uint32_t* ctr) {
  __builtin_amdgcn_fence(__ATOMIC_RELEASE, "workgroup", "local");
  lds_inc(ctr);
}
__device__ __forceinline__ uint32_t lds_peek(uint32_t* flag) {
  return __hip_atomic_load(flag, __ATOMIC_RELAXED, __HIP_MEMORY_SCOPE_WORKGROUP);
}
__device__ __forceinline__ void lds_wait_ge(uint32_t* flag, uint32_t v) {
  while (lds_peek(flag) < v) __builtin_amdgcn_s_sleep(1);
  __builtin_amdgcn_fence(__ATOMIC_ACQUIRE, "workgroup", "local");
}
// ... 5 lines not shown
  __builtin_amdgcn_fence(__ATOMIC_ACQUIRE, "workgroup", "local");
}

__device__ __forceinline__ void pow2_scales(float mx, float& sc, float& inv) {
  int E = (__builtin_bit_cast(int, mx) >> 23) & 0xff;
  E = E < 40 ? 40 : E;
  sc = __builtin_bit_cast(float, (127 + TS_TARGET_EXP + 127 - E) << 23);
  inv = __builtin_bit_cast(float, (E - TS_TARGET_EXP) << 23);
}

__device__ __forceinline__ void split4(const float4 v, const float sc, h4& hi, h4& lo) {
  const float f[4] = {v.x, v.y, v.z, v.w};
#pragma unroll
  for (int e = 0; e < 4; ++e) {
    const _Float16 h = (_Float16)(f[e] * sc);
    hi[e] = h;
    lo[e] = (_Float16)fmaf(f[e], sc, -(float)h);
  }
}

template <int DK, int NW, int NCW, int SLOTS, int AHEAD, int DEPTH, int MODE>
__global__ __launch_bounds__(64 * NW) void transform_stream_kernel(GemmParams p) {
  using SL = Slot<DK>;
  static_assert(AHEAD >= 1 && AHEAD < SLOTS && NCW <= NW && 32 % (4 * NW) == 0, "pipeline shape");
  constexpr int KB16 = DK / 16;
  constexpr int CPT = DK / 64;
  constexpr int GPW = 32 / (4 * NW);
  constexpr int RPW = 32 / NW;
  __shared__ __attribute__((aligned(16))) unsigned char ring[SLOTS * SL::BYTES];
  __shared__ uint32_t ready[SLOTS], done[SLOTS];
  __shared__ __attribute__((aligned(16))) float gtab[MODE == 0 ? 2 * DK : 4];
  const int tid = threadIdx.x, lane = tid & 63;
  const int wave = __builtin_amdgcn_readfirstlane(tid >> 6);
  if (tid < SLOTS) { ready[tid] = 0u; done[tid] = 0u; }
  const int64_t ntiles = (p.N + 31) / 32;
  const int64_t nlocal = (ntiles - blockIdx.x + gridDim.x - 1) / gridDim.x;
  const bool consumer = wave < NCW;
#ifdef TS_STAMP
  uint32_t st_acc[8] = {0, 0, 0, 0, 0, 0, 0, 0};
  uint32_t st_last = (uint32_t)__builtin_amdgcn_s_memtime();
#define TS_MARK(k) do { const uint32_t t__ = (uint32_t)__builtin_amdgcn_s_memtime(); st_acc[k] += t__ - st_last; st_last = t__; } while (0)
#else
#define TS_MARK(k) do { } while (0)
#endif

  const int l16 = lane & 15, rsub = lane >> 4;
  float gcs[2] = {0.f, 0.f};
  if constexpr (MODE == 0) {
    for (int k = tid; k < DK; k += 64 * NW) {
      gtab[2 * k] = k < p.Din ? p.g[k] : 0.f;
      gtab[2 * k + 1] = k < p.Din ? p.g[2 * p.Din + k] : 0.f;
    }
  }
  if constexpr (MODE == 0) { gcs[0] = p.gc[0]; gcs[1] = p.gc[1]; }
  __syncthreads();
  const bool din_full = p.Din == DK;
  int woff[GPW][CPT], xoff[GPW][CPT], moff[GPW], coff[GPW];
#pragma unroll
  for (int g = 0; g < GPW; ++g) {
    const int row = RPW * wave + 4 * g + rsub;
    moff[g] = row;
    coff[g] = l16 < 4 ? 32 * l16 + row : 128 + row;
#pragma unroll
    for (int c = 0; c < CPT; ++c) {
      const int c4 = l16 + 16 * c, k = c4 * 4;
      woff[g][c] = SL::chunk_off(row, c4 >> 1) + ((c4 & 1) << 3);
      xoff[g][c] = (int)((row * p.ldx + (din_full || k < p.Din ? k : 0)) * 4);
    }
  }
  u32x4 ra[DEPTH][GPW][CPT];
  uint8_t rm[DEPTH][GPW];
  const int64_t tstep = (int64_t)gridDim.x * 32;
  int64_t rq_left = p.N - (int64_t)blockIdx.x * 32;
  const float* rq_x = p.x + (int64_t)blockIdx.x * 32 * p.ldx;
  const uint8_t* rq_m = p.mask + (int64_t)blockIdx.x * 32;
  const bool has_mask = MODE == 0 || p.mask != nullptr;
  auto request = [&](int set) {
    const int rows_here = rq_left > 32 ? 32 : (rq_left < 0 ? 0 : (int)rq_left);
    const __amdgpu_buffer_rsrc_t rx = __builtin_amdgcn_make_buffer_rsrc(const_cast<float*>(rq_x), (short)0, rows_here * (int)p.ldx * 4, 0x00020000);
    const __amdgpu_buffer_rsrc_t rmk = __builtin_amdgcn_make_buffer_rsrc(const_cast<uint8_t*>(rq_m), (short)0, has_mask ? rows_here : 0, 0x00020000);
#pragma unroll
    for (int g = 0; g < GPW; ++g) {
#pragma unroll
      for (int c = 0; c < CPT; ++c) ra[set][g][c] = __builtin_amdgcn_raw_buffer_load_b128(rx, xoff[g][c], 0, 0);
      rm[set][g] = __builtin_amdgcn_raw_buffer_load_b8(rmk, moff[g], 0, 0);
    }
    rq_left -= tstep; rq_x += tstep * p.ldx; rq_m += tstep;
  };
  struct StageState { float f[4 * CPT]; bool sdom; f2 d; float mx, sc, inv, t; h4 hi[CPT], lo[CPT]; };
  constexpr int STAGE_STEPS = CPT + 4 + 3 * CPT + 4;
  auto stage_step = [&](StageState& q, int m, unsigned char* sb, int g) {
    if (m < CPT) {
      if constexpr (MODE == 0) {
        const float4 ga = *reinterpret_cast<const float4*>(&gtab[8 * (l16 + 16 * m)]);
        const float4 gb = *reinterpret_cast<const float4*>(&gtab[8 * (l16 + 16 * m) + 4]);
        q.d = __builtin_elementwise_fma(f2{q.f[4 * m], q.f[4 * m]}, f2{ga.x, ga.y}, q.d);
        q.d = __builtin_elementwise_fma(f2{q.f[4 * m + 1], q.f[4 * m + 1]}, f2{ga.z, ga.w}, q.d);
        q.d = __builtin_elementwise_fma(f2{q.f[4 * m + 2], q.f[4 * m + 2]}, f2{gb.x, gb.y}, q.d);
        q.d = __builtin_elementwise_fma(f2{q.f[4 * m + 3], q.f[4 * m + 3]}, f2{gb.z, gb.w}, q.d);
      }
    } else if (m == CPT) {
#pragma unroll
      for (int c = 0; c < CPT; ++c) {
        q.mx = fmaxf(fmaxf(fabsf(q.f[4 * c]), fabsf(q.f[4 * c + 1])), q.mx);
        q.mx = fmaxf(fmaxf(fabsf(q.f[4 * c + 2]), fabsf(q.f[4 * c + 3])), q.mx);
      }
    } else if (m == CPT + 1) {
// ... 53 lines not shown
    TS_MARK(1);
    unsigned char* const sb = ring + slot * SL::BYTES;
#pragma unroll
    for (int g = 0; g < GPW; ++g) {
      StageState q;
      stage_init(q, rv[g], mk[g]);
#pragma unroll
      for (int m = 0; m < STAGE_STEPS; ++m) stage_step(q, m, sb, g);
    }
    lds_arrive(&ready[slot]);
    TS_MARK(3);
  };

  const int fr = lane & 31, fh = lane >> 5;
  const int col_base = p.col_off + wave * 32;
  const int n = col_base + fr;
  h8 whi[KB16], wlo[KB16];
  float cinv = 0.f;
  float bias_n = 0.f, wd_n = 0.f;
  const float* otab = nullptr;
  int ooff = 0;
  int my_table = 0;
  const int roff0 = SL::chunk_off(fr, fh);
  static_assert(DK == 128, "fragment offsets: roff0 ^ (kb << 5) holds for 256-byte rows");
  auto roff = [&](int kb) { return roff0 ^ (kb << 5); };
  if (consumer) {
    float4 w[KB16][2];
    float mx = 0.f;
#pragma unroll
    for (int kb = 0; kb < KB16; ++kb)
#pragma unroll
      for (int hf = 0; hf < 2; ++hf) {
        const int k = 16 * kb + 8 * fh + 4 * hf;
        float4 t = make_float4(0.f, 0.f, 0.f, 0.f);
        if (n < p.NC && k < p.Din) t = *reinterpret_cast<const float4*>(p.Wp + (int64_t)n * p.Din + k);
        w[kb][hf] = t;
        mx = fmaxf(fmaxf(mx, fmaxf(fabsf(t.x), fabsf(t.y))), fmaxf(fabsf(t.z), fabsf(t.w)));
      }
    mx = fmaxf(mx, __shfl_xor(mx, 32));
    float sc;
    pow2_scales(mx, sc, cinv);
#pragma unroll
    for (int kb = 0; kb < KB16; ++kb)
#pragma unroll
      for (int hf = 0; hf < 2; ++hf) {
        h4 hi, lo;
        split4(w[kb][hf], sc, hi, lo);
#pragma unroll
        for (int e = 0; e < 4; ++e) { whi[kb][4 * hf + e] = hi[e]; wlo[kb][4 * hf + e] = lo[e]; }
      }
    const int ld2 = 2 * (int)p.ldh;
    const int h = col_base / ld2, rem = col_base % ld2, t = rem >= p.ldh ? 1 : 0;
    bias_n = p.bias[n];
    if constexpr (MODE == 0) wd_n = p.wd[n];
    otab = h == 0 ? (t == 0 ? p.out[0][0] : p.out[0][1]) : (t == 0 ? p.out[1][0] : p.out[1][1]);
    ooff = (int)((4 * fh * p.row_stride + (rem - t * (int)p.ldh) + fr) * 4);
    if constexpr (MODE == 0) my_table = __builtin_amdgcn_readfirstlane(t);
  }
  const int rs4 = (int)(p.row_stride * 4);
  auto consume = [&](int64_t i, int slot, uint32_t round, float (&res)[16]) -> bool {
    if (!consumer || i >= nlocal) return false;
    const int64_t tile = blockIdx.x + i * (int64_t)gridDim.x;
    const unsigned char* const sb = ring + slot * SL::BYTES;
    TS_MARK(0);
    lds_wait_ge(&ready[slot], (uint32_t)NW * (round + 1));
    TS_MARK(4);
    bool skip = false;
    if constexpr (MODE == 0) {
      const int64_t tb = tile * 32, te = tb + 32;
      skip = p.tail_s2t_begin > 0 && ((my_table == 0 && tb >= p.tail_t2s_begin && te <= p.tail_s2t_begin) || (my_table == 1 && tb >= p.tail_s2t_begin));
      if (p.tile_need != nullptr) skip = skip || ((p.tile_need[tile] >> my_table) & 1) == 0;
    }
    if (skip) {
      lds_arrive(&done[slot]);
      return false;
    }
    f32x16 acc;
#pragma unroll
    for (int r = 0; r < 16; ++r) acc[r] = 0.f;
    constexpr int NB = KB16 / 2;
    h8 fa[2][2][2];
    auto fetch = [&](int b, int buf) {
#pragma unroll
      for (int t = 0; t < 2; ++t) {
        fa[buf][t][0] = *reinterpret_cast<const h8*>(sb + roff(2 * b + t));
        fa[buf][t][1] = *reinterpret_cast<const h8*>(sb + SL::PIECE + roff(2 * b + t));
      }
    };
    fetch(0, 0);
    if constexpr (NB > 1) fetch(1, 1);
#pragma unroll
    for (int b = 0; b < NB; ++b) {
      __builtin_amdgcn_sched_barrier(0);
#pragma unroll
      for (int t = 0; t < 2; ++t) {
        const int kb = 2 * b + t;
        acc = __builtin_amdgcn_mfma_f32_32x32x16_f16(fa[b & 1][t][1], whi[kb], acc, 0, 0, 0);
        acc = __builtin_amdgcn_mfma_f32_32x32x16_f16(fa[b & 1][t][0], wlo[kb], acc, 0, 0, 0);
        acc = __builtin_amdgcn_mfma_f32_32x32x16_f16(fa[b & 1][t][0], whi[kb], acc, 0, 0, 0);
      }
      __builtin_amdgcn_sched_barrier(0);
      if (b + 2 < NB) fetch(b + 2, b & 1);
    }
    const float* cf = reinterpret_cast<const float*>(sb + SL::COEF);
    float4 cq[4], sq[4];
#pragma unroll
    for (int q = 0; q < 4; ++q) {
// ... 552 lines not shown
        if (s >= 0) {
          stage(s, rv, mk, ss, sr);
          bump(ss, sr);
        }
        if (i >= 0) {
          if (my_turn) live = consume(i, cs, cr, o0, o1);
          bump(cs, cr);
        }
      }
      TS_MARK(6);
      store_raw(live, o0, o1);
      pf_done = lds_peek(&done[ss]);
      pf_ready = lds_peek(&ready[cs]);
      TS_MARK(7);
    }
  }
#ifdef TS_STAMP
  if (lane == 0 && p.sk_out[0][0] != nullptr) {
    float* o = p.sk_out[0][0] + ((int64_t)blockIdx.x * NW + wave) * 8;
#pragma unroll
    for (int k2 = 0; k2 < 8; ++k2) o[k2] = (float)st_acc[k2];
  }
#endif
  if (consumer && p.colsum != nullptr) {
#pragma unroll
    for (int r = 0; r < 16; ++r) {
      float a = cs_s[r], b = cs_t[r];
#pragma unroll
      for (int m = 16; m >= 1; m >>= 1) { a += __shfl_xor(a, m); b += __shfl_xor(b, m); }
      if (fr == 0) {
        const int c = col_base + 8 * (r >> 2) + 4 * fh + (r & 3);
        unsafeAtomicAdd(&p.colsum[c], (double)a);
        unsafeAtomicAdd(&p.colsum[NC + c], (double)b);
      }
    }
    if (cw == 0) {
      float a = cnt_s, b = cnt_t;
#pragma unroll
      for (int m = 32; m >= 1; m >>= 1) { a += __shfl_xor(a, m); b += __shfl_xor(b, m); }
      if (lane == 0) { unsafeAtomicAdd(&p.colsum[2 * NC], (double)a); unsafeAtomicAdd(&p.colsum[2 * NC + 1], (double)b); }
    }
  }
}

}

static bool stream2_supported(const GemmParams& p);

bool bgnn_tf_stream_supported(const GemmParams& p, int mode) {
  if (mode == 2) return stream2_supported(p);
  if (mode != 0) return false;
  if (p.n_heads != 1 || p.Din > 128 || p.Din <= 64 || (p.Din & 3) || (p.ldh & 31)) return false;
  if (p.NC != 2 * p.ldh || (p.NC != 256 && p.NC != 128) || p.col_off != 0) return false;
  if (p.ldx * 4 * 32 > 0x7fffffff || p.row_stride * 4 * 36 > 0x7fffffff) return false;
  return true;
}

static bool stream2_supported(const GemmParams& p) {
  return p.NC == 128 && p.Din <= 128 && p.Din > 64 && (p.Din & 3) == 0 && p.mask && p.w2 && p.g2 && p.raw && p.ldx * 4 * 32 <= 0x7fffffff;
}

int bgnn_tf_stream_launch(const GemmParams& p, int mode, hipStream_t st, int n_cu) {
  if (mode == 2) {
    if (!stream2_supported(p)) return BGNN_E_SHAPE;
    const int64_t nt = (p.N + 31) / 32;
    const dim3 g2((unsigned)(nt < n_cu ? nt : n_cu), 1u);
#ifdef TS_STAMP
    {
      GemmParams q = p;
      static float* dbuf2 = nullptr;
      if (!dbuf2) (void)hipMalloc((void**)&dbuf2, sizeof(float) * 256 * 8 * 8);
      q.sk_out[0][0] = dbuf2;
      hipLaunchKernelGGL((transform_stream2_kernel<128, 8, 4, TS_SLOTS, TS_AHEAD, TS_DEPTH>), g2, dim3(512), 0, st, q);
      static int calls2 = 0;
      if (++calls2 % 12 == 0) {
        (void)hipDeviceSynchronize();
        static float host[256 * 8 * 8];
        (void)hipMemcpy(host, dbuf2, sizeof(float) * g2.x * 8 * 8, hipMemcpyDeviceToHost);
        double acc[8] = {0};
        for (unsigned w = 0; w < g2.x * 8; ++w) for (int k = 0; k < 8; ++k) acc[k] += host[w * 8 + k];
        const double d = (double)g2.x * 8 * ((double)nt / g2.x);
        fprintf(stderr, "[ts2 stamp] cycles per tile and wave (mean): other %.0f  flags %.0f  request %.0f  chain(+stage, fused turn) %.0f  post %.0f  reduce/flush %.0f  pre-store %.0f  stores+peek %.0f\n",
                acc[0] / d, acc[1] / d, acc[2] / d, acc[3] / d, acc[4] / d, acc[5] / d, acc[6] / d, acc[7] / d);
      }
      BGNN_LAUNCH_CHECK();
      return 0;
    }
#endif
    hipLaunchKernelGGL((transform_stream2_kernel<128, 8, 4, TS_SLOTS, TS_AHEAD, TS_DEPTH>), g2, dim3(512), 0, st, p);
    BGNN_LAUNCH_CHECK();
    return 0;
  }
  if (!bgnn_tf_stream_supported(p, mode)) return BGNN_E_SHAPE;
  const int64_t ntiles = (p.N + 31) / 32;
  const dim3 grid((unsigned)(ntiles < n_cu ? ntiles : n_cu), 1u);
#ifdef TS_STAMP
  GemmParams q = p;
  static float* dbuf = nullptr;
  if (!dbuf) (void)hipMalloc((void**)&dbuf, sizeof(float) * 256 * 8 * 8);
  q.raw = dbuf;
  if (p.NC == 256) hipLaunchKernelGGL((transform_stream_kernel<128, 8, 8, TS_SLOTS, TS_AHEAD, TS_DEPTH, 0>), grid, dim3(512), 0, st, q);
  else hipLaunchKernelGGL((transform_stream_kernel<128, 8, 4, TS_SLOTS, TS_AHEAD, TS_DEPTH, 0>), grid, dim3(512), 0, st, q);
  static int calls = 0;
  if (++calls % 12 == 0) {
    (void)hipDeviceSynchronize();
    static float host[256 * 8 * 8];
// ... 17 lines not shown
```

### bridged_gnn_amd/ktgnn.py

```python
import math
import os
import weakref

import torch
import torch.nn.functional as F
from torch import nn

from . import ops

__all__ = ["Linear", "AdaptedConv", "KTGNN_no_complement"]


def _plist(module):
    pl = module.__dict__.get("_bgnn_plist")
    if pl is None:
        pl = list(module.parameters())
        module.__dict__["_bgnn_plist"] = pl
    return pl


def _forget_plists(root):
    for m in root.modules():
        m.__dict__.pop("_bgnn_plist", None)

# ... 640 lines not shown
                        x = self.bns[ind](x)
                    x = F.relu(x)
                    x = F.dropout(x, p=self.dropout, training=self.training)
        self._arena = arena
        return (x, sums) if want_sums else x

    def _input_sums_miss(self, x, central_mask):
        if torch.cuda.is_current_stream_capturing() or not getattr(self, "cache_input_sums", True):
            return True
        c = getattr(self, "_xsum_cache", None)
        return not (c is not None and c[0]() is x and c[1] == x._version and c[2]() is central_mask and c[3] == central_mask._version)

    def _input_domain_sums(self, x, central_mask, arena):
        if torch.cuda.is_current_stream_capturing() or not getattr(self, "cache_input_sums", True):
            return ops.domain_sums(x, _as_u8(central_mask).contiguous(), out=arena.take(2 * x.shape[1] + 2))
        c = getattr(self, "_xsum_cache", None)
        if (c is not None and c[0]() is x and c[1] == x._version and c[2]() is central_mask and c[3] == central_mask._version):
            return c[4]
        sums = ops.domain_sums(x, _as_u8(central_mask).contiguous(), out=arena.take(2 * x.shape[1] + 2)).clone()
        self._xsum_cache = (weakref.ref(x), x._version, weakref.ref(central_mask), central_mask._version, sums)
        return sums

    def _transformer_to_target_tables(self, x, mask_u8, out, arena=None, sums_out=None):
        return self._stage.target_tables(x, mask_u8, out, arena, sums_out)

    def _composed_target_pack(self, din_pad):
        return self._stage.composed_target_pack(din_pad)

    def forward(self, data):
        x, central_mask = data.x, data.central_mask
        csr = self._prepare(data)
        x, sums_h = self._hidden(x, csr, central_mask, want_sums=True)
        x = x.contiguous()
        mask_u8 = _as_u8(central_mask).contiguous()
        stage = self._stage
        train = self.training and torch.is_grad_enabled()
        walk = stage.train_walk(opt_in=True) if (train and stage.plain and x.dtype == torch.float32) else None
        if walk is not None:
            sums_x = ops.domain_sums(_pad_cols4(x.detach()), mask_u8)
            tabs = stage.train_tables(x, mask_u8, sums_x, bn_relu_dropout_train)
            return (*stage.train_aggregate(walk, csr, mask_u8, tabs), None)
        if not stage.plain or torch.is_grad_enabled() or self.training:
            logits_base = self.clf_base(x, None, central_mask=central_mask, csr=csr)
            logits_target = self.clf_target(x, None, central_mask=central_mask, csr=csr)
            needs_grad = torch.is_grad_enabled() and (x.requires_grad or any(p.requires_grad for p in _plist(self.clf_transformer)))
            if train:
                l0, bn, _, l3 = self.clf_transformer
                xt = l3(bn_relu_dropout_train(l0(x), bn, True, 0.0))
            else:
                xt = self.clf_transformer(x) if (self.training or needs_grad) else stage.transformer_eval(x)
            logits_hat = self.clf_target(xt.contiguous(), None, central_mask=central_mask, csr=csr)
            return (F.log_softmax(logits_base, dim=1), F.log_softmax(logits_target, dim=1),
                    F.log_softmax(logits_hat, dim=1), None)
        t2s = torch.empty(x.shape[0], 3 * stage.ld, dtype=torch.float32, device=x.device)
        s2t = torch.empty_like(t2s)
        stage.eval_tables(x, mask_u8, sums_h, stage.views(t2s, s2t), self._arena)
        a_t2s, a_s2t = stage.attention()
        out3 = ops.adaptedconv_aggregate(t2s, s2t, a_t2s, a_s2t, csr, mask_u8, stage.C, stage.slope, heads=3,
                                         log_softmax=stage.fused_log_softmax)
        return (*stage.finish(out3), None)

    def graphed(self, data, warmup=2):
        if self.training:
            raise RuntimeError("graphed() captures the eval forward; call model.eval() first")
        with torch.no_grad():
            for _ in range(max(int(warmup), 1)):
                self.forward(data)
            torch.cuda.synchronize()
            g = torch.cuda.CUDAGraph()
            with torch.cuda.graph(g):
                out = self.forward(data)

        def replay():
            g.replay()
            return out
        replay.graph = g
        return replay

    def _drop_param_caches(self):
        for c in list(self.convs) + [self.clf_base, self.clf_target]:
            c._pack_key = None
        self._stage.drop_caches()
        for bn in list(self.bns) + [self.clf_transformer[1]]:
            bn._bgnn_affine = None
        _forget_plists(self)

    def invalidate_input_cache(self):
        self._xsum_cache = None

    def graphed_train_step(self, data, loss_fn, optimizer, warmup=3):
        if not self.training:
            raise RuntimeError("graphed_train_step() captures a training step; call model.train() first")
        if any(not g["capturable"] for g in optimizer.param_groups if "capturable" in g):
            raise RuntimeError("graphed_train_step() needs a capturable optimizer, e.g. torch.optim.Adam(params, capturable=True)")
        dev = data.x.device
        step = torch.zeros(1, dtype=torch.int64, device=dev)
        side = torch.cuda.Stream(device=dev)
        side.wait_stream(torch.cuda.current_stream(dev))
        _DROPOUT_STEP[0] = step
        try:
            with torch.cuda.stream(side):
                for _ in range(max(int(warmup), 1)):
                    step.add_(1)
                    optimizer.zero_grad(set_to_none=True)
                    loss_fn(self(data)).backward()
                    optimizer.step()
            torch.cuda.current_stream(dev).wait_stream(side)
            torch.cuda.synchronize(dev)
# ... 24 lines not shown
```

### bridged_gnn_amd/ops.py

```python
import os

import torch

from . import _lib as L

__all__ = ["DstCSR", "build_dst_csr", "domain_delta", "pack_transform_heads", "adaptedconv_transform", "adaptedconv_aggregate", "linear", "linear_supported", "linear_narrow_supported", "linear_narrow_transform", "narrow_transform_finish", "gram", "gram_supported", "rowdot", "transform_bwd_prep", "topk_edges_coalesced",
           "l2_normalize_rows", "cosine_topk", "mlp_pair_topk", "topk_edges", "coalesce", "gather_rows", "pad4",
           "sage_mean_aggregate", "sage_mean_aggregate_bwd", "rows_segment_add", "gcn_aggregate", "gcn_aggregate_bwd", "wide_heads_supported",
           "adaptedconv_aggregate_heads_wide", "adaptedconv_aggregate_heads_wide_bwd", "pair_csr", "pair_mlp_stats", "pair_mlp_loss",
           "pair_mlp_segsum", "pair_mlp_eval", "pair_mlp_count", "PAIR_MLP_WIDTH", "pair_cos_loss", "pair_cos_segsum", "pair_cos_count",
           "PAIR_COS_WIDTH"]


def pad4(n):
    return (int(n) + 3) // 4 * 4


HUB_THRESHOLD = 128
HUB_SEGMENT = 64


class DstCSR:

    def __init__(self, rowptr, col, eperm, num_edges, num_nodes):
# ... 163 lines not shown

    @staticmethod
    def backward(ctx, g):
        return g.expand(ctx.shape)


def domain_delta(sums, Din):
    delta = torch.empty(Din, dtype=torch.float32, device=sums.device)
    rc = L.lib().bgnn_domain_delta_f32(L.ptr(sums), Din, L.ptr(delta), L.stream())
    L.check(rc, "bgnn_domain_delta_f32")
    return delta


def linear_supported(din, dout):
    return din <= 128 and din % 4 == 0 and dout % 64 == 0


def linear(x, weight, bias, relu=False, mask_u8=None, colsum=None):
    N, din = x.shape
    dout = weight.shape[0]
    out = torch.empty(N, dout, dtype=torch.float32, device=x.device)
    rc = L.lib().bgnn_linear_f32(L.ptr_rows(x), N, din, x.stride(0), L.ptr(weight), L.ptr(bias), dout, 1 if relu else 0,
                                 L.ptr(mask_u8), L.ptr(colsum), L.ptr(out), dout, L.stream())
    L.check(rc, "bgnn_linear_f32")
    return out


def linear_narrow_supported(din, dout, packed):
    Wp, bp, gates, D, ldh, gconst = packed
    return (din <= 128 and din % 4 == 0 and dout in (64, 128, 256) and gates.shape[0] == 1 and ldh == 4
            and Wp.shape == (8, dout))


def linear_narrow_transform(x, weight, bias, mask_u8, colsum, packed, relu=True):
    N, din = x.shape
    dout = weight.shape[0]
    Wp, bp, gates, D, ldh, gconst = packed
    raw = torch.empty(N, 12, dtype=torch.float32, device=x.device)
    rc = L.lib().bgnn_linear_narrow_transform_f32(L.ptr_rows(x), N, din, x.stride(0), L.ptr(weight), L.ptr(bias), dout,
                                                  1 if relu else 0, L.ptr(mask_u8), L.ptr(colsum), L.ptr(Wp), L.ptr(gates),
                                                  L.ptr(raw), L.stream())
    L.check(rc, "bgnn_linear_narrow_transform_f32")
    return raw


def classifier_stage_supported(x, packed_pair, weight, packed_t):
    Wp, bp, gates, D, ldh, gconst = packed_pair
    din = x.shape[1]
    return (x.is_cuda and x.dtype == torch.float32 and x.stride(1) == 1 and 64 < din <= 128 and din % 4 == 0
            and weight.shape == (128, din) and Wp.shape[0] <= 24 and Wp.shape[1] == din and packed_t[0].shape == (8, 128)
            and os.environ.get("BGNN_FUSED_CLS", "1") != "0")


def classifier_stage(x, mask_u8, sums_x, packed_pair, outs, weight, bias, colsum, packed_t, relu=True):
    N, din = x.shape
    Wp, bp, gates, D, ldh, gconst = packed_pair
    H = gates.shape[0]
    Wp2, _, gates2, _, _, _ = packed_t
    raw = torch.empty(N, 12, dtype=torch.float32, device=x.device)
    small = torch.empty(H * (2 * ldh + 2) + 8, dtype=torch.float32, device=x.device)
    row_stride = outs[0][0].stride(0)
    for a, b in outs:
        assert a.shape[0] >= N and b.shape[0] >= N and a.stride(0) == row_stride and b.stride(0) == row_stride
    o1 = outs[1] if H > 1 else (None, None)
    rc = L.lib().bgnn_classifier_stage_f32(L.ptr_rows(x), N, din, x.stride(0), L.ptr(mask_u8), L.ptr(sums_x), H, D, L.ptr(Wp), L.ptr(bp),
                                           L.ptr(gates), L.ptr(gconst), L.ptr_rows(outs[0][1]), L.ptr_rows(outs[0][0]),
                                           L.ptr_rows(o1[1]), L.ptr_rows(o1[0]), ldh, row_stride, L.ptr(weight), L.ptr(bias),
                                           weight.shape[0], 1 if relu else 0, L.ptr(colsum), L.ptr(Wp2), L.ptr(gates2), L.ptr(raw),
                                           L.ptr(small), L.stream())
    L.check(rc, "bgnn_classifier_stage_f32")
    return raw


def narrow_transform_finish(raw, mask_u8, sums, packed, out):
    Wp, bp, gates, D, ldh, gconst = packed
    h_t2s, h_s2t = out
    N = raw.shape[0]
    assert h_t2s.stride(0) == h_s2t.stride(0) and sums.dtype == torch.float64 and sums.numel() == 2 * Wp.shape[1] + 2
    small = torch.empty(16, dtype=torch.float32, device=raw.device)
    rc = L.lib().bgnn_narrow_transform_finish_f32(L.ptr(raw), N, L.ptr(mask_u8), L.ptr(sums), Wp.shape[1], L.ptr(Wp), L.ptr(bp),
                                                  L.ptr(gates), L.ptr(gconst), L.ptr_rows(h_s2t), L.ptr_rows(h_t2s),
                                                  h_t2s.stride(0), L.ptr(small), L.stream())
    L.check(rc, "bgnn_narrow_transform_finish_f32")
    return out


def transform_bwd_prep(x, G_s2t, G_t2s, D, mask_u8, gx, gconst, wd, counts, out=None, want_ex=False):
    N, din = x.shape
    p = pad4(2 * D + 3)
    assert counts.dtype == torch.float64 and counts.numel() == 2
    if out is None:
        Gall = torch.empty(N, p, dtype=torch.float32, device=x.device)
        side = None if want_ex else torch.empty(N, 4, dtype=torch.float32, device=x.device)
    else:
        Gall, side = out
        assert Gall.shape == (N, p) and (side is None or side.shape == (N, 4))
    assert G_s2t.stride(0) == G_t2s.stride(0) and G_s2t.stride(1) == 1 and G_t2s.stride(1) == 1
    lib = L.lib()
    ex = ws = None
    wsb = 0
    if want_ex:
        ex = torch.empty(p, 4, dtype=torch.float32, device=x.device)
        wsb = lib.bgnn_transform_bwd_prep_workspace_bytes(N, p)
        ws = torch.empty(wsb, dtype=torch.uint8, device=x.device)
    rc = lib.bgnn_transform_bwd_prep_f32(L.ptr_rows(x), x.stride(0), N, din, L.ptr_rows(G_s2t), L.ptr_rows(G_t2s),
                                         G_s2t.stride(0), D, L.ptr(mask_u8), L.ptr(gx), L.ptr(gconst), L.ptr(wd),
                                         L.ptr(counts), L.ptr_rows(Gall), p, Gall.stride(0),
                                         L.ptr_rows(side) if side is not None else None, side.stride(0) if side is not None else 4,
                                         L.ptr(ex), L.ptr(ws), wsb, L.stream())
    L.check(rc, "bgnn_transform_bwd_prep_f32")
    return (Gall, ex) if want_ex else (Gall, side)


def transform_bwd_consts(W_s, W_t, g1, g2, delta, din):
    D = W_s.shape[0]
    dev = W_s.device
    gx = torch.empty(2, din, dtype=torch.float32, device=dev)
    gconst = torch.empty(2, dtype=torch.float32, device=dev)
    wd = torch.empty(2, 2 * D, dtype=torch.float32, device=dev)
    rc = L.lib().bgnn_transform_bwd_consts_f32(L.ptr(W_s), L.ptr(W_t), L.ptr(g1), L.ptr(g2), L.ptr(delta), D, din,
                                               L.ptr(gx), L.ptr(gconst), L.ptr(wd), L.stream())
    L.check(rc, "bgnn_transform_bwd_consts_f32")
    return gx, gconst, wd


def transform_bwd_finish(dWall, ex, W_s, W_t, g1, g2, delta, din, wcat_t):
    D = W_s.shape[0]
    p = dWall.shape[0]
    dev = W_s.device
    dW_s, dW_t = torch.empty(D, din, dtype=torch.float32, device=dev), torch.empty(D, din, dtype=torch.float32, device=dev)
    dg1, dg2 = torch.empty(2 * din, dtype=torch.float32, device=dev), torch.empty(2 * din, dtype=torch.float32, device=dev)
# ... 91 lines not shown
    rc = L.lib().bgnn_bn_bwd_reduce_rows_f32(L.ptr_rows(x), L.ptr_rows(grad_y), N, D, x.stride(0), grad_y.stride(0), *a, L.ptr(gacc), L.stream())
    L.check(rc, "bgnn_bn_bwd_reduce_rows_f32")
    return gacc.view(-1, 2 * D).sum(0)


def bn_bwd_apply_rows(x, grad_y, totals, gtotals, n_total, gamma, beta, eps, relu, p_drop, seed, row_ids=None, row_base=0, seed_dev=None):
    N, D = x.shape
    if gtotals.dtype != torch.float64 or gtotals.numel() != 2 * D:
        raise RuntimeError(f"gtotals must be {2 * D} doubles (sum g' | sum g'.xhat over all ranks' rows)")
    gx = torch.empty(N, D, dtype=torch.float32, device=x.device)
    a = _bn_rows_args(x, totals, n_total, gamma, beta, eps, relu, p_drop, seed, seed_dev, row_ids, row_base)
    rc = L.lib().bgnn_bn_bwd_apply_rows_f32(L.ptr_rows(x), L.ptr_rows(grad_y), N, D, x.stride(0), grad_y.stride(0), a[0], L.ptr(gtotals), *a[1:],
                                            L.ptr(gx), D, L.stream())
    L.check(rc, "bgnn_bn_bwd_apply_rows_f32")
    return gx


def rowdot(X, V):
    N, d = X.shape
    nv = V.shape[0]
    out = torch.empty(N, nv, dtype=torch.float32, device=X.device)
    rc = L.lib().bgnn_rowdot_f32(L.ptr_rows(X), X.stride(0), N, d, L.ptr(V), V.stride(0), nv, L.ptr(out), L.stream())
    L.check(rc, "bgnn_rowdot_f32")
    return out


def pack_transform_heads(heads, din_pad):
    D = heads[0]["W_s"].shape[0]
    din = heads[0]["W_s"].shape[1]
    ldh = pad4(D)
    dev = heads[0]["W_s"].device
    H = len(heads)
    Wp = torch.zeros(H * 2 * ldh, din_pad, dtype=torch.float32, device=dev)
    bp = torch.zeros(H * 2 * ldh, dtype=torch.float32, device=dev)
    gates = torch.zeros(H, 2, 2 * din_pad, dtype=torch.float32, device=dev)
    gconst = torch.zeros(H, 2, dtype=torch.float32, device=dev)
    for h, hd in enumerate(heads):
        if hd.get("gate_const") is not None:
            gconst[h, 0], gconst[h, 1] = hd["gate_const"]
        base = h * 2 * ldh
        Wp[base: base + D, :din] = hd["W_t"]
        Wp[base + ldh: base + ldh + D, :din] = hd["W_s"]
        if hd.get("b_t") is not None:
            bp[base: base + D] = hd["b_t"]
        if hd.get("b_s") is not None:
            bp[base + ldh: base + ldh + D] = hd["b_s"]
        for t, key in enumerate(("g_s2t", "g_t2s")):
            g = hd[key].reshape(-1)
            gates[h, t, :din] = g[:din]
            gates[h, t, din_pad: din_pad + din] = g[din:]
    return Wp, bp, gates, D, ldh, gconst


def adaptedconv_transform(x, mask_u8, delta, packed, out=None, sums=None, tail_single=(0, 0), tile_need=None):
    lib = L.lib()
    Wp, bp, gates, D, ldh, gconst = packed
    H = gates.shape[0]
    N, Din = x.shape
    dev = x.device
    if out is None:
        out = [(torch.empty(N, ldh, dtype=torch.float32, device=dev), torch.empty(N, ldh, dtype=torch.float32, device=dev))
               for _ in range(H)]
    row_stride = out[0][0].stride(0)
    for a, b in out:
        assert a.shape[0] >= N and b.shape[0] >= N and a.stride(0) == row_stride and b.stride(0) == row_stride
    small = torch.empty(H * (2 * ldh + 2) + 8, dtype=torch.float32, device=dev)
    o1 = out[1] if H > 1 else (None, None)
    if delta is None:
        if sums is None or sums.dtype != torch.float64 or sums.numel() != 2 * Din + 2:
            raise ValueError("adaptedconv_transform needs delta [Din] or the float64 domain sums [2*Din+2]")
        fn, first, name = lib.bgnn_adaptedconv_transform_sums_f32, sums, "bgnn_adaptedconv_transform_sums_f32"
    else:
        fn, first, name = lib.bgnn_adaptedconv_transform_f32, delta, "bgnn_adaptedconv_transform_f32"
    tail = (int(tail_single[0]), int(tail_single[1])) if delta is None else ()
    if delta is not None and tuple(tail_single) != (0, 0):
        raise ValueError("tail_single needs the sums form of the transform")
    if tile_need is not None:
        if delta is not None or tuple(tail_single) != (0, 0):
            raise ValueError("tile_need needs the sums form of the transform and no tail_single")
        if tile_need.dtype != torch.int32 or tile_need.numel() != (N + 31) // 32:
            raise ValueError("tile_need: one int32 per 32-row tile")
        fn, name, tail = lib.bgnn_adaptedconv_transform_need_f32, "bgnn_adaptedconv_transform_need_f32", (L.ptr(tile_need),)
    rc = fn(L.ptr(x), N, Din, x.stride(0), L.ptr(mask_u8), L.ptr(first), H, D, L.ptr(Wp), L.ptr(bp), L.ptr(gates), L.ptr(gconst),
            L.ptr_rows(out[0][1]), L.ptr_rows(out[0][0]), L.ptr_rows(o1[1]), L.ptr_rows(o1[0]), ldh, row_stride, *tail,
            L.ptr(small), L.stream())
    L.check(rc, name)
    return out


_P2_STATIC = os.environ.get("BGNN_P2_STATIC", "1") != "0"


def _tile_queue(dev):
    return torch.empty(8, dtype=torch.int32, device=dev)


def heads_log_softmax_supported(heads, D):
    return heads in (2, 3) and D <= 4


def _hub_shape_ok(D, ldh, ldo, heads, slope):
    if heads in (2, 3) and D <= 4 and ldh == 4 and ldo == 4:
        return True
    return heads == 1 and D > 32 and 0.0 <= slope <= 1.0


def adaptedconv_aggregate(h_t2s, h_s2t, a_t2s, a_s2t, csr, mask_u8, D, negative_slope=0.1, n_dst=None,
                          want_alpha=False, ep_scale=None, ep_shift=None, ep_relu=False, out=None,
                          row_begin=0, row_end=None, state_ms=None, part=0, heads=1, colsum=None, log_softmax=False,
                          park_begin=None):
    lib = L.lib()
    n_dst = csr.num_nodes if n_dst is None else int(n_dst)
    row_end = n_dst if row_end is None else int(row_end)
    ldh = h_t2s.stride(0) // heads
    ldo = pad4(D)
    dev = h_t2s.device
    if out is None:
        out = torch.empty(n_dst, heads * ldo, dtype=torch.float32, device=dev)
    assert h_t2s.stride(0) == h_s2t.stride(0) and h_t2s.stride(0) % heads == 0 and out.stride(0) % heads == 0
    alpha = torch.empty(csr.num_edges, dtype=torch.float32, device=dev) if want_alpha else None
    tq = _tile_queue(dev) if heads == 1 else None
    if row_end <= int(row_begin):
        return (out, alpha) if want_alpha else out
    if ((not want_alpha or heads == 1) and part in (0, 3) and int(row_begin) == 0 and row_end == csr.num_nodes == n_dst and h_t2s.shape[0] == n_dst
            and (ep_scale is None or heads == 1) and _hub_shape_ok(D, ldh, out.stride(0) // heads, heads, negative_slope)
            and os.environ.get("BGNN_HUB_ROWS", "1") != "0"):
        hubs = csr.hub_tables()
        if hubs is not None:
            hub_rows, seg_ptr, seg_bounds, seg_node = hubs
            nseg = int(seg_node.numel())
            wsb = lib.bgnn_aggregate_hub_workspace_bytes(nseg, heads, out.stride(0) // heads)
            ws = torch.empty(wsb, dtype=torch.uint8, device=dev)
            rc = lib.bgnn_adaptedconv_aggregate_hub_f32(
                L.ptr_rows(h_t2s), L.ptr_rows(h_s2t), ldh, L.ptr(a_t2s), L.ptr(a_s2t), L.ptr(csr.rowptr), L.ptr(csr.col),
                L.ptr(mask_u8), n_dst, D, float(negative_slope), L.ptr_rows(out), out.stride(0) // heads,
                L.ptr(ep_scale), L.ptr(ep_shift), 2 if log_softmax else (1 if ep_relu else 0),
                L.ptr(state_ms) if part == 3 else None, int(heads), L.ptr(colsum),
                L.ptr(tq), HUB_THRESHOLD, L.ptr(hub_rows), int(hub_rows.numel()),
                L.ptr(seg_ptr), L.ptr(seg_bounds), L.ptr(seg_node), nseg, L.ptr(alpha), L.ptr(ws), wsb, L.stream())
            L.check(rc, "bgnn_adaptedconv_aggregate_hub_f32")
            return (out, alpha) if want_alpha else out
    rc = lib.bgnn_adaptedconv_aggregate_bounded_f32(
        L.ptr_rows(h_t2s), L.ptr_rows(h_s2t), ldh, L.ptr(a_t2s), L.ptr(a_s2t), L.ptr(csr.rowptr), L.ptr(csr.col),
        L.ptr(mask_u8), int(row_begin), row_end, D, float(negative_slope), L.ptr_rows(out), out.stride(0) // heads, L.ptr(alpha),
        L.ptr(ep_scale), L.ptr(ep_shift), 2 if log_softmax else (1 if ep_relu else 0), L.ptr(state_ms), int(part),
        int(row_begin) if park_begin is None else int(park_begin), int(heads), L.ptr(colsum),
        L.ptr(tq) if not (part == 2 and _P2_STATIC) else None, min(int(h_t2s.shape[0]), int(h_s2t.shape[0])),
        csr.gather_hint() if (heads == 1 and D > 32 and part == 0) else 0, L.stream())
    L.check(rc, "bgnn_adaptedconv_aggregate_bounded_f32")
    return (out, alpha) if want_alpha else out


def adaptedconv_aggregate_bwd(h_t2s, h_s2t, a_t2s, a_s2t, csr, mask_u8, D, out, alpha, grad_out, negative_slope=0.1):
    lib = L.lib()
    dev = h_t2s.device
    da_t2s = torch.zeros(D, dtype=torch.float32, device=dev)
    da_s2t = torch.zeros(D, dtype=torch.float32, device=dev)
    grad_out = grad_out.contiguous()
    if D <= 128 and grad_out.stride(0) % 4 == 0 and grad_out.data_ptr() % 16 == 0 and h_t2s.shape[0] == csr.num_nodes:
        t_rowptr, t_eid, t_dst = csr.transposed()
        dh_t2s, dh_s2t = torch.empty_like(h_t2s), torch.empty_like(h_s2t)
        narrow = D <= 4 and h_t2s.stride(0) == 4 and out.stride(0) == 4 and grad_out.stride(0) == 4
        dh_, sh_ = (csr.hub_tables(), csr.transposed_hub_tables()) if (not narrow and os.environ.get("BGNN_HUB_ROWS", "1") != "0") else (None, None)
        if dh_ is not None or sh_ is not None:
            none4 = (None, None, None, None)
            d_rows, d_ptr, d_bounds, d_node = dh_ if dh_ is not None else none4
            s_rows, s_ptr, s_bounds, s_node = sh_ if sh_ is not None else none4
            nd = 0 if dh_ is None else int(d_node.numel())
            ns = 0 if sh_ is None else int(s_node.numel())
            wsb = lib.bgnn_aggregate_bwd_pull_hub_workspace_bytes(csr.num_nodes, csr.num_edges, h_t2s.stride(0), nd, ns)
            ws = torch.empty(wsb, dtype=torch.uint8, device=dev)
            rc = lib.bgnn_adaptedconv_aggregate_bwd_pull_hub_f32(
                L.ptr(h_t2s), L.ptr(h_s2t), h_t2s.stride(0), L.ptr(a_t2s), L.ptr(a_s2t), L.ptr(csr.rowptr), L.ptr(csr.col),
                L.ptr(mask_u8), L.ptr(t_rowptr), L.ptr(t_eid), L.ptr(t_dst), csr.num_nodes, csr.num_edges, D, float(negative_slope),
                L.ptr(out), out.stride(0), L.ptr(alpha), L.ptr(grad_out), grad_out.stride(0),
                L.ptr(dh_t2s), L.ptr(dh_s2t), L.ptr(da_t2s), L.ptr(da_s2t), HUB_THRESHOLD,
                L.ptr(d_rows), 0 if dh_ is None else int(d_rows.numel()), L.ptr(d_ptr), L.ptr(d_bounds), L.ptr(d_node), nd,
                L.ptr(s_rows), 0 if sh_ is None else int(s_rows.numel()), L.ptr(s_ptr), L.ptr(s_bounds), L.ptr(s_node), ns,
                L.ptr(ws), wsb, L.stream())
            L.check(rc, "bgnn_adaptedconv_aggregate_bwd_pull_hub_f32")
            return dh_t2s, dh_s2t, da_t2s, da_s2t
        wsb = lib.bgnn_aggregate_bwd_pull_workspace_bytes(csr.num_nodes, csr.num_edges, h_t2s.stride(0))
        ws = torch.empty(wsb, dtype=torch.uint8, device=dev)
        rc = lib.bgnn_adaptedconv_aggregate_bwd_pull_f32(
            L.ptr(h_t2s), L.ptr(h_s2t), h_t2s.stride(0), L.ptr(a_t2s), L.ptr(a_s2t), L.ptr(csr.rowptr), L.ptr(csr.col),
            L.ptr(mask_u8), L.ptr(t_rowptr), L.ptr(t_eid), L.ptr(t_dst), csr.num_nodes, csr.num_edges, D, float(negative_slope),
            L.ptr(out), out.stride(0), L.ptr(alpha), L.ptr(grad_out), grad_out.stride(0),
            L.ptr(dh_t2s), L.ptr(dh_s2t), L.ptr(da_t2s), L.ptr(da_s2t), L.ptr(ws), wsb, L.stream())
        L.check(rc, "bgnn_adaptedconv_aggregate_bwd_pull_f32")
        return dh_t2s, dh_s2t, da_t2s, da_s2t
    dh_t2s, dh_s2t = torch.zeros_like(h_t2s), torch.zeros_like(h_s2t)
    rc = lib.bgnn_adaptedconv_aggregate_bwd_f32(
        L.ptr(h_t2s), L.ptr(h_s2t), h_t2s.stride(0), L.ptr(a_t2s), L.ptr(a_s2t), L.ptr(csr.rowptr), L.ptr(csr.col),
        L.ptr(mask_u8), 0, csr.num_nodes, D, float(negative_slope), L.ptr(out), out.stride(0), L.ptr(alpha),
        L.ptr(grad_out), grad_out.stride(0), L.ptr(dh_t2s), L.ptr(dh_s2t), L.ptr(da_t2s), L.ptr(da_s2t), L.stream())
    L.check(rc, "bgnn_adaptedconv_aggregate_bwd_f32")
    return dh_t2s, dh_s2t, da_t2s, da_s2t


def adaptedconv_aggregate_heads_bwd(t2s, s2t, a_t2s, a_s2t, csr, mask_u8, D, heads, out, state_ms, grad_out, log_softmax,
                                    negative_slope=0.1):
    lib = L.lib()
# ... 641 lines not shown
```

### include/bgnn.h

```cpp
#ifndef BGNN_H_
#define BGNN_H_
#include <stddef.h>
#include <stdint.h>

#ifdef __cplusplus
extern "C" {
#endif

#define BGNN_VERSION 113
#define BGNN_E_NULL (-1)
#define BGNN_E_SHAPE (-2)
#define BGNN_E_WORKSPACE (-3)
#define BGNN_E_ALIGN (-4)
#define BGNN_E_RANGE (-5)

int bgnn_version(void);
const char* bgnn_error_string(int code);
const char* bgnn_source_hash(void);

size_t bgnn_csr_workspace_bytes(int64_t N, int64_t E);
int bgnn_build_dst_csr(const int64_t* edge_index, int64_t E, int64_t N, int rewrite_self_loops,
                       int32_t* rowptr, int32_t* col, int32_t* eperm_opt, int64_t* E_out_dev,
                       void* ws, size_t ws_bytes, void* stream);

int bgnn_domain_sums_f64(const float* x, int64_t N, int32_t Din, int64_t ldx, const uint8_t* mask,
                         double* sums_io , void* stream);
size_t bgnn_domain_sums_workspace_bytes(int32_t Din);
int bgnn_domain_sums_ws_f64(const float* x, int64_t N, int32_t Din, int64_t ldx, const uint8_t* mask,
                            double* sums_io , void* ws, size_t ws_bytes, void* stream);
int bgnn_domain_delta_f32(const double* sums , int32_t Din, float* delta, void* stream);
int bgnn_linear_f32(const float* x, int64_t N, int32_t Din, int64_t ldx, const float* W, const float* bias,
                    int32_t Dout, int relu, const uint8_t* mask_opt, double* colsum_opt,
                    float* out, int64_t ldo, void* stream);
int bgnn_linear_narrow_transform_f32(const float* x, int64_t N, int32_t Din, int64_t ldx, const float* W,
                                     const float* bias, int32_t Dout, int relu, const uint8_t* mask,
                                     double* colsum, const float* Wp2, const float* gates2, float* raw, void* stream);
int bgnn_classifier_stage_f32(const float* x, int64_t N, int32_t Din, int64_t ldx, const uint8_t* mask,
                              const double* sums_x, int32_t sk_heads, int32_t sk_D, const float* sk_Wp,
                              const float* sk_bias, const float* sk_gates, const float* sk_gate_const_opt,
                              float* h_s2t_0, float* h_t2s_0, float* h_s2t_1, float* h_t2s_1, int64_t sk_ldh,
                              int64_t sk_row_stride, const float* W, const float* bias, int32_t Dout, int relu,
                              double* colsum, const float* Wp2, const float* gates2, float* raw, float* small_ws,
                              void* stream);
int bgnn_narrow_transform_finish_f32(const float* raw, int64_t N, const uint8_t* mask, const double* sums,
                                     int32_t Din, const float* Wp2, const float* bias2, const float* gates2,
                                     const float* gate_const_opt, float* h_s2t, float* h_t2s, int64_t row_stride,
                                     float* small_ws, void* stream);
size_t bgnn_gram_workspace_bytes(int32_t p, int32_t q);
int bgnn_gram_f32(const float* A, int64_t lda, int32_t p, const float* B, int64_t ldb, int32_t q, int64_t N,
                  float* out , void* ws, size_t ws_bytes, void* stream);
int64_t bgnn_bn_acc_doubles(int32_t D);
int bgnn_bn_relu_dropout_f32(const float* x, int64_t N, int32_t D, int64_t ldx, const float* gamma_opt,
                             const float* beta_opt, float eps, int relu, float p_drop, uint64_t seed, const uint64_t* seed_dev_opt,
                             float momentum, float* running_mean_opt, float* running_var_opt,
                             float* y, int64_t ldy, double* stats, void* stream);
int bgnn_bn_relu_dropout_bwd_f32(const float* x, const float* grad_y, int64_t N, int32_t D, int64_t ldx, int64_t ldg,
                                 const double* stats, const float* gamma_opt, const float* beta_opt, float eps,
                                 int relu, float p_drop, uint64_t seed, const uint64_t* seed_dev_opt, float* grad_x, int64_t ldgx,
                                 double* gsum, void* stream);
int bgnn_bn_colstats_f32(const float* x, int64_t n_rows, int32_t D, int64_t ldx, double* acc, void* stream);
int bgnn_bn_apply_rows_f32(const float* x, int64_t n_rows, int32_t D, int64_t ldx, const double* totals, int64_t n_total,
                           const float* gamma_opt, const float* beta_opt, float eps, int relu, float p_drop, uint64_t seed,
                           const uint64_t* seed_dev_opt, const int64_t* row_ids_opt, int64_t row_base,
                           float momentum, float* running_mean_opt, float* running_var_opt,
                           float* y, int64_t ldy, void* stream);
int bgnn_bn_bwd_reduce_rows_f32(const float* x, const float* grad_y, int64_t n_rows, int32_t D, int64_t ldx, int64_t ldg,
                                const double* totals, int64_t n_total, const float* gamma_opt, const float* beta_opt,
                                float eps, int relu, float p_drop, uint64_t seed, const uint64_t* seed_dev_opt,
                                const int64_t* row_ids_opt, int64_t row_base, double* gacc, void* stream);
int bgnn_bn_bwd_apply_rows_f32(const float* x, const float* grad_y, int64_t n_rows, int32_t D, int64_t ldx, int64_t ldg,
                               const double* totals, const double* gtotals, int64_t n_total, const float* gamma_opt,
                               const float* beta_opt, float eps, int relu, float p_drop, uint64_t seed,
                               const uint64_t* seed_dev_opt, const int64_t* row_ids_opt, int64_t row_base,
                               float* grad_x, int64_t ldgx, void* stream);
size_t bgnn_transform_bwd_prep_workspace_bytes(int64_t N, int32_t p);
int bgnn_transform_bwd_prep_f32(const float* x, int64_t ldx, int64_t N, int32_t din, const float* G_s2t, const float* G_t2s,
                                int64_t ldg, int32_t D, const uint8_t* mask, const float* gx ,
                                const float* gconst , const float* wd , const double* counts ,
                                float* Gall, int32_t p, int64_t ld_gall, float* side_opt, int64_t ld_side,
                                float* ex_opt , void* ws_opt, size_t ws_bytes, void* stream);
int bgnn_transform_bwd_consts_f32(const float* W_s, const float* W_t, const float* g1, const float* g2, const float* delta,
                                  int32_t D, int32_t din, float* gx, float* gconst, float* wd, void* stream);
int bgnn_transform_bwd_finish_f32(const float* dWall, const float* ex, const float* W_s, const float* W_t, const float* g1,
                                  const float* g2, const float* delta, int32_t D, int32_t din, int32_t p, float* dW_s,
                                  float* dW_t, float* dg1, float* dg2, float* db_s_opt, float* db_t_opt, float* wcat_t,
                                  int64_t ld_wcat, void* stream);
int bgnn_rowdot_f32(const float* X, int64_t ldx, int64_t N, int32_t d, const float* V, int64_t ldv, int32_t nv,
                    float* out , void* stream);
int bgnn_adaptedconv_transform_f32(const float* x, int64_t N, int32_t Din, int64_t ldx,
                                   const uint8_t* mask, const float* delta,
                                   int32_t n_heads, int32_t D, const float* Wp, const float* bias_p,
                                   const float* gates, const float* gate_const_opt,
                                   float* h_s2t_0, float* h_t2s_0, float* h_s2t_1, float* h_t2s_1,
                                   int64_t ldh, int64_t row_stride, float* small_ws, void* stream);
int bgnn_adaptedconv_transform_sums_f32(const float* x, int64_t N, int32_t Din, int64_t ldx,
                                        const uint8_t* mask, const double* sums,
                                        int32_t n_heads, int32_t D, const float* Wp, const float* bias_p,
                                        const float* gates, const float* gate_const_opt,
                                        float* h_s2t_0, float* h_t2s_0, float* h_s2t_1, float* h_t2s_1,
                                        int64_t ldh, int64_t row_stride, int64_t n_tail_t2s, int64_t n_tail_s2t,
                                        float* small_ws, void* stream);
int bgnn_adaptedconv_transform_need_f32(const float* x, int64_t N, int32_t Din, int64_t ldx,
                                        const uint8_t* mask, const double* sums,
                                        int32_t n_heads, int32_t D, const float* Wp, const float* bias_p,
                                        const float* gates, const float* gate_const_opt,
                                        float* h_s2t_0, float* h_t2s_0, float* h_s2t_1, float* h_t2s_1,
                                        int64_t ldh, int64_t row_stride, const int32_t* tile_need_opt,
                                        float* small_ws, void* stream);

int bgnn_adaptedconv_aggregate_f32(const float* h_t2s, const float* h_s2t, int64_t ldh,
                                   const float* a_t2s, const float* a_s2t,
                                   const int32_t* rowptr, const int32_t* col, const uint8_t* mask,
                                   int64_t row_begin, int64_t row_end, int32_t D, float negative_slope,
                                   float* out, int64_t ldo, float* alpha_opt,
                                   const float* ep_scale_opt, const float* ep_shift_opt, int ep_relu,
                                   float* state_ms_opt, int part, int64_t park_begin, int32_t heads, double* colsum_opt,
                                   uint32_t* tile_queue_opt, void* stream);

int bgnn_adaptedconv_aggregate_bounded_f32(const float* h_t2s, const float* h_s2t, int64_t ldh,
                                           const float* a_t2s, const float* a_s2t,
                                           const int32_t* rowptr, const int32_t* col, const uint8_t* mask,
                                           int64_t row_begin, int64_t row_end, int32_t D, float negative_slope,
                                           float* out, int64_t ldo, float* alpha_opt,
                                           const float* ep_scale_opt, const float* ep_shift_opt, int ep_relu,
                                           float* state_ms_opt, int part, int64_t park_begin, int32_t heads, double* colsum_opt,
                                           uint32_t* tile_queue_opt, int64_t table_rows, int32_t gather_hint, void* stream);

size_t bgnn_aggregate_hub_workspace_bytes(int64_t n_segments, int32_t heads, int64_t ldo);
int bgnn_adaptedconv_aggregate_hub_f32(const float* h_t2s, const float* h_s2t, int64_t ldh,
                                       const float* a_t2s, const float* a_s2t,
                                       const int32_t* rowptr, const int32_t* col, const uint8_t* mask,
                                       int64_t N, int32_t D, float negative_slope, float* out, int64_t ldo,
                                       const float* ep_scale_opt, const float* ep_shift_opt, int ep_relu,
                                       float* state_ms_opt, int32_t heads, double* colsum_opt,
                                       uint32_t* tile_queue_opt, int32_t hub_threshold, const int32_t* hub_rows,
                                       int64_t n_hubs, const int32_t* hub_seg_ptr, const int32_t* seg_bounds,
                                       const int32_t* seg_node, int64_t n_segments, float* alpha_opt,
                                       void* ws, size_t ws_bytes, void* stream);

int bgnn_adaptedconv_aggregate_bwd_f32(const float* h_t2s, const float* h_s2t, int64_t ldh,
                                       const float* a_t2s, const float* a_s2t,
                                       const int32_t* rowptr, const int32_t* col, const uint8_t* mask,
                                       int64_t row_begin, int64_t row_end, int32_t D, float negative_slope,
                                       const float* out, int64_t ldo, const float* alpha,
                                       const float* grad_out, int64_t ldg,
                                       float* dh_t2s, float* dh_s2t, float* da_t2s, float* da_s2t,
                                       void* stream);

size_t bgnn_aggregate_bwd_pull_workspace_bytes(int64_t N, int64_t E, int64_t ldh);
int bgnn_adaptedconv_aggregate_bwd_pull_f32(const float* h_t2s, const float* h_s2t, int64_t ldh,
                                            const float* a_t2s, const float* a_s2t,
                                            const int32_t* rowptr, const int32_t* col, const uint8_t* mask,
                                            const int32_t* t_rowptr, const int32_t* t_eid, const int32_t* t_dst,
                                            int64_t N, int64_t E, int32_t D, float negative_slope,
                                            const float* out, int64_t ldo, const float* alpha,
                                            const float* grad_out, int64_t ldg,
                                            float* dh_t2s, float* dh_s2t, float* da_t2s, float* da_s2t,
                                            void* ws, size_t ws_bytes, void* stream);

size_t bgnn_aggregate_bwd_pull_hub_workspace_bytes(int64_t N, int64_t E, int64_t ldh, int64_t d_segments, int64_t s_segments);
int bgnn_adaptedconv_aggregate_bwd_pull_hub_f32(const float* h_t2s, const float* h_s2t, int64_t ldh,
                                                const float* a_t2s, const float* a_s2t,
                                                const int32_t* rowptr, const int32_t* col, const uint8_t* mask,
                                                const int32_t* t_rowptr, const int32_t* t_eid, const int32_t* t_dst,
                                                int64_t N, int64_t E, int32_t D, float negative_slope,
                                                const float* out, int64_t ldo, const float* alpha,
                                                const float* grad_out, int64_t ldg,
                                                float* dh_t2s, float* dh_s2t, float* da_t2s, float* da_s2t,
                                                int32_t hub_threshold,
                                                const int32_t* d_hub_rows, int64_t d_n_hubs, const int32_t* d_hub_seg_ptr,
                                                const int32_t* d_seg_bounds, const int32_t* d_seg_node, int64_t d_n_segments,
                                                const int32_t* s_hub_rows, int64_t s_n_hubs, const int32_t* s_hub_seg_ptr,
                                                const int32_t* s_seg_bounds, const int32_t* s_seg_node, int64_t s_n_segments,
                                                void* ws, size_t ws_bytes, void* stream);

size_t bgnn_aggregate_heads_bwd_workspace_bytes(int64_t N, int64_t E, int32_t heads);
int bgnn_adaptedconv_aggregate_heads_bwd_f32(const float* h_t2s, const float* h_s2t, const float* a_t2s, const float* a_s2t,
                                             const int32_t* rowptr, const int32_t* col, const uint8_t* mask,
                                             const int32_t* t_rowptr, const int32_t* t_eid, const int32_t* t_dst,
// ... 168 lines not shown
```

Baseline: 50.34 billion edges/s.

## Self-reset tile queues in-kernel and fuse wd/gate constant computation into consumers

Aggregation kernels now reset their tile-queue counters themselves. A per-XCD and global retire counter lets the last finishing block zero the queue, which removes the separate memset launched before each aggregation. The wd/gc constant kernel is folded into the streaming transform GEMM and the narrow finish kernel, so each block computes those constants from the domain sums. This cuts several small launches per forward pass. The cost is extra atomics at block exit and redundant per-block constant computation, and the queue is only correct if every kernel completes its retire sequence.

```diff
diff --git a/bridged_gnn_amd/_lib.py b/bridged_gnn_amd/_lib.py
--- a/bridged_gnn_amd/_lib.py
+++ b/bridged_gnn_amd/_lib.py
@@ -25,6 +25,11 @@
                                                     _P, _P, _P, _P, _I64, _I64, _I64, _I64, _P, _P]),
     "bgnn_adaptedconv_transform_need_f32": (_INT, [_P, _I64, _I32, _I64, _P, _P, _I32, _I32, _P, _P, _P, _P,
                                                     _P, _P, _P, _P, _I64, _I64, _P, _P, _P]),
+    "bgnn_adaptedconv_transform_fused_f32": (_INT, [_P, _I64, _I32, _I64, _P, _P, _I32, _I32, _P, _P, _P, _P,
+                                                     _P, _P, _P, _P, _I64, _I64, _P, _P, _P]),
+    "bgnn_classifier_stage_fused_f32": (_INT, [_P, _I64, _I32, _I64, _P, _P, _I32, _I32, _P, _P, _P, _P, _P, _P, _P, _P, _I64, _I64,
+                                                _P, _P, _I32, _INT, _P, _P, _P, _P, _P]),
+    "bgnn_narrow_transform_finish_fused_f32": (_INT, [_P, _I64, _P, _P, _I32, _P, _P, _P, _P, _P, _P, _I64, _P]),
     "bgnn_classifier_stage_f32": (_INT, [_P, _I64, _I32, _I64, _P, _P, _I32, _I32, _P, _P, _P, _P, _P, _P, _P, _P, _I64, _I64,
                                           _P, _P, _I32, _INT, _P, _P, _P, _P, _P, _P]),
     "bgnn_linear_narrow_transform_f32": (_INT, [_P, _I64, _I32, _I64, _P, _P, _I32, _INT, _P, _P, _P, _P, _P, _P]),
@@ -48,6 +53,10 @@
                                                _P, _I64, _P, _P, _P, _INT, _P, _INT, _I64, _I32, _P, _P, _P]),
     "bgnn_adaptedconv_aggregate_bounded_f32": (_INT, [_P, _P, _I64, _P, _P, _P, _P, _P, _I64, _I64, _I32, _F32,
                                                        _P, _I64, _P, _P, _P, _INT, _P, _INT, _I64, _I32, _P, _P, _I64, _I32, _P]),
+    "bgnn_adaptedconv_aggregate_queued_f32": (_INT, [_P, _P, _I64, _P, _P, _P, _P, _P, _I64, _I64, _I32, _F32,
+                                                      _P, _I64, _P, _P, _P, _INT, _P, _INT, _I64, _I32, _P, _P, _I64, _I32, _P]),
+    "bgnn_adaptedconv_aggregate_hub_queued_f32": (_INT, [_P, _P, _I64, _P, _P, _P, _P, _P, _I64, _I32, _F32, _P, _I64, _P, _P, _INT, _P, _I32, _P,
+                                                          _P, _I32, _P, _I64, _P, _P, _P, _I64, _P, _P, C.c_size_t, _P]),
     "bgnn_aggregate_hub_workspace_bytes": (C.c_size_t, [_I64, _I32, _I64]),
     "bgnn_adaptedconv_aggregate_hub_f32": (_INT, [_P, _P, _I64, _P, _P, _P, _P, _P, _I64, _I32, _F32, _P, _I64, _P, _P, _INT, _P, _I32, _P,
                                                    _P, _I32, _P, _I64, _P, _P, _P, _I64, _P, _P, C.c_size_t, _P]),
diff --git a/bridged_gnn_amd/csrc/bgnn_aggregate.hip b/bridged_gnn_amd/csrc/bgnn_aggregate.hip
--- a/bridged_gnn_amd/csrc/bgnn_aggregate.hip
+++ b/bridged_gnn_amd/csrc/bgnn_aggregate.hip
@@ -40,7 +40,19 @@
   uint32_t tbl_bytes, off_t2s, off_s2t;
   int32_t gather_hint;
   uint32_t dead_off;
+  int tq_retire;
 };
+
+__device__ __forceinline__ void tq_retire_block(unsigned int* q) {
+  if (threadIdx.x != 0) return;
+  const unsigned xcd = blockIdx.x % 8, G = (gridDim.x + 7 - xcd) / 8, nx = gridDim.x < 8 ? gridDim.x : 8;
+  __threadfence();
+  if (atomicAdd(&q[32 + xcd], 1u) != G - 1) return;
+  __threadfence();
+  if (atomicAdd(&q[48], 1u) != nx - 1) return;
+  for (int i = 0; i < 8; ++i) { atomicExch(&q[i], 0u); atomicExch(&q[32 + i], 0u); }
+  atomicExch(&q[48], 0u);
+}
 
 __device__ __forceinline__ float leaky(float v, float slope) { return v > 0.f ? v : v * slope; }
 
@@ -223,6 +235,7 @@
       }
     }
   }
+  if (p.tq_retire) tq_retire_block(p.tile_queue);
   if (p.colsum != nullptr) {
     __syncthreads();
     for (int t = threadIdx.x; t < 2 * (LF * 4 + 1); t += 256) {
@@ -498,6 +511,7 @@
       }
     }
   }
+  if (p.tq_retire) tq_retire_block(p.tile_queue);
   if (p.colsum != nullptr) {
     unsafeAtomicAdd(&red[0][f0], cs_s.x); unsafeAtomicAdd(&red[0][f0 + 1], cs_s.y);
     unsafeAtomicAdd(&red[0][f0 + 2], cs_s.z); unsafeAtomicAdd(&red[0][f0 + 3], cs_s.w);
@@ -736,6 +750,7 @@
       }
     }
   }
+  if (p.tq_retire) tq_retire_block(p.tile_queue);
   if (p.colsum != nullptr) {
     unsafeAtomicAdd(&red[0][f0], cs_s01.x); unsafeAtomicAdd(&red[0][f0 + 1], cs_s01.y);
     unsafeAtomicAdd(&red[0][f0 + 2], cs_s23.x); unsafeAtomicAdd(&red[0][f0 + 3], cs_s23.y);
@@ -1191,7 +1206,8 @@
                           float* out, int64_t ldo, float* alpha_opt,
                           const float* ep_scale_opt, const float* ep_shift_opt, int ep_relu,
                           float* state_ms_opt, int part, int64_t park_begin, int32_t heads,
-                          double* colsum_opt, uint32_t* tile_queue_opt, int64_t table_rows, int32_t gather_hint, void* stream) {
+                          double* colsum_opt, uint32_t* tile_queue_opt, int64_t table_rows, int32_t gather_hint, void* stream,
+                          bool tq_retire = false) {
   if (colsum_opt && heads != 1) return BGNN_E_SHAPE;
   if (part == 1 && (park_begin < row_begin || park_begin > row_end)) return BGNN_E_SHAPE;
   if (part < 0 || part > 3 || (part != 0 && (!state_ms_opt || alpha_opt))) return BGNN_E_NULL;
@@ -1209,8 +1225,9 @@
               out, ldo, alpha_opt, ep_scale_opt, ep_shift_opt, ep_relu, tile_queue_opt, colsum_opt, heads, state_ms_opt, part,
               park_begin, 4};
   p.gather_hint = gather_hint;
+  p.tq_retire = (tq_retire && tile_queue_opt) ? 1 : 0;
   hipStream_t st = (hipStream_t)stream;
-  if (tile_queue_opt) {
+  if (tile_queue_opt && !tq_retire) {
     hipError_t e = bgnn_zero_async(tile_queue_opt, 8 * sizeof(uint32_t), st);
     if (e != hipSuccess) return (int)e;
   }
@@ -1243,21 +1260,36 @@
                         ep_scale_opt, ep_shift_opt, ep_relu, state_ms_opt, part, park_begin, heads, colsum_opt, tile_queue_opt, table_rows, gather_hint, stream);
 }
 
+extern "C" int bgnn_adaptedconv_aggregate_queued_f32(const float* h_t2s, const float* h_s2t, int64_t ldh,
+                                                     const float* a_t2s, const float* a_s2t,
+                                                     const int32_t* rowptr, const int32_t* col, const uint8_t* mask,
+                                                     int64_t row_begin, int64_t row_end, int32_t D, float negative_slope,
+                                                     float* out, int64_t ldo, float* alpha_opt,
+                                                     const float* ep_scale_opt, const float* ep_shift_opt, int ep_relu,
+                                                     float* state_ms_opt, int part, int64_t park_begin, int32_t heads,
+                                                     double* colsum_opt, uint32_t* tile_queue_opt, int64_t table_rows, int32_t gather_hint,
+                                                     void* stream) {
+  if (table_rows < row_end || gather_hint < 0 || gather_hint > 2) return BGNN_E_SHAPE;
+  return aggregate_impl(h_t2s, h_s2t, ldh, a_t2s, a_s2t, rowptr, col, mask, row_begin, row_end, D, negative_slope, out, ldo, alpha_opt,
+                        ep_scale_opt, ep_shift_opt, ep_relu, state_ms_opt, part, park_begin, heads, colsum_opt, tile_queue_opt, table_rows, gather_hint, stream,
+                        true);
+}
+
 extern "C" size_t bgnn_aggregate_hub_workspace_bytes(int64_t n_segments, int32_t heads, int64_t ldo) {
   const size_t nv = (size_t)(n_segments > 0 ? n_segments : 0), h = (size_t)(heads > 0 ? heads : 1);
   return bgnn_align_up(sizeof(float) * nv * h * (size_t)(ldo > 0 ? ldo : 0), 256) + bgnn_align_up(sizeof(float) * 2 * nv * h, 256) + 256;
 }
 
-extern "C" int bgnn_adaptedconv_aggregate_hub_f32(const float* h_t2s, const float* h_s2t, int64_t ldh,
-                                                  const float* a_t2s, const float* a_s2t,
-                                                  const int32_t* rowptr, const int32_t* col, const uint8_t* mask,
-                                                  int64_t N, int32_t D, float negative_slope, float* out, int64_t ldo,
-                                                  const float* ep_scale_opt, const float* ep_shift_opt, int ep_relu,
-                                                  float* state_ms_opt, int32_t heads, double* colsum_opt,
-                                                  uint32_t* tile_queue_opt, int32_t hub_threshold, const int32_t* hub_rows,
-                                                  int64_t n_hubs, const int32_t* hub_seg_ptr, const int32_t* seg_bounds,
-                                                  const int32_t* seg_node, int64_t n_segments, float* alpha_opt,
-                                                  void* ws, size_t ws_bytes, void* stream) {
+static int aggregate_hub_impl(const float* h_t2s, const float* h_s2t, int64_t ldh,
+                              const float* a_t2s, const float* a_s2t,
+                              const int32_t* rowptr, const int32_t* col, const uint8_t* mask,
+                              int64_t N, int32_t D, float negative_slope, float* out, int64_t ldo,
+                              const float* ep_scale_opt, const float* ep_shift_opt, int ep_relu,
+                              float* state_ms_opt, int32_t heads, double* colsum_opt,
+                              uint32_t* tile_queue_opt, int32_t hub_threshold, const int32_t* hub_rows,
+                              int64_t n_hubs, const int32_t* hub_seg_ptr, const int32_t* seg_bounds,
+                              const int32_t* seg_node, int64_t n_segments, float* alpha_opt,
+                              void* ws, size_t ws_bytes, void* stream, bool tq_retire) {
   if (!h_t2s || !h_s2t || !a_t2s || !a_s2t || !rowptr || !col || !mask || !out) return BGNN_E_NULL;
   if (alpha_opt && heads != 1) return BGNN_E_SHAPE;
   if (n_hubs > 0 && (!hub_rows || !hub_seg_ptr || !seg_bounds || !seg_node || !ws)) return BGNN_E_NULL;
@@ -1277,7 +1309,8 @@
               out, ldo, alpha_opt, ep_scale_opt, ep_shift_opt, ep_relu, tile_queue_opt, colsum_opt, heads, state_ms_opt, part,
               0, 4};
   p.hub_threshold = n_hubs > 0 ? hub_threshold : 0;
-  if (tile_queue_opt) {
+  p.tq_retire = (tq_retire && tile_queue_opt) ? 1 : 0;
+  if (tile_queue_opt && !tq_retire) {
     hipError_t e = bgnn_zero_async(tile_queue_opt, 8 * sizeof(uint32_t), st);
     if (e != hipSuccess) return (int)e;
   }
@@ -1302,6 +1335,19 @@
   BGNN_LAUNCH_CHECK();
   return 0;
 }
+
+#define BGNN_HUB_ARGS_DECL const float* h_t2s, const float* h_s2t, int64_t ldh, const float* a_t2s, const float* a_s2t, \
+    const int32_t* rowptr, const int32_t* col, const uint8_t* mask, int64_t N, int32_t D, float negative_slope, float* out, int64_t ldo, \
+    const float* ep_scale_opt, const float* ep_shift_opt, int ep_relu, float* state_ms_opt, int32_t heads, double* colsum_opt, \
+    uint32_t* tile_queue_opt, int32_t hub_threshold, const int32_t* hub_rows, int64_t n_hubs, const int32_t* hub_seg_ptr, \
+    const int32_t* seg_bounds, const int32_t* seg_node, int64_t n_segments, float* alpha_opt, void* ws, size_t ws_bytes, void* stream
+#define BGNN_HUB_ARGS h_t2s, h_s2t, ldh, a_t2s, a_s2t, rowptr, col, mask, N, D, negative_slope, out, ldo, ep_scale_opt, ep_shift_opt, ep_relu, \
+    state_ms_opt, heads, colsum_opt, tile_queue_opt, hub_threshold, hub_rows, n_hubs, hub_seg_ptr, seg_bounds, seg_node, n_segments, alpha_opt, \
+    ws, ws_bytes, stream
+extern "C" int bgnn_adaptedconv_aggregate_hub_f32(BGNN_HUB_ARGS_DECL) { return aggregate_hub_impl(BGNN_HUB_ARGS, false); }
+extern "C" int bgnn_adaptedconv_aggregate_hub_queued_f32(BGNN_HUB_ARGS_DECL) { return aggregate_hub_impl(BGNN_HUB_ARGS, true); }
+#undef BGNN_HUB_ARGS_DECL
+#undef BGNN_HUB_ARGS
 
 #ifdef BGNN_TUNING
 extern "C" int bgnn_tune_reset_counters(void* stream) { (void)stream; return 0; }
diff --git a/bridged_gnn_amd/csrc/bgnn_transform.hip b/bridged_gnn_amd/csrc/bgnn_transform.hip
--- a/bridged_gnn_amd/csrc/bgnn_transform.hip
+++ b/bridged_gnn_amd/csrc/bgnn_transform.hip
@@ -7,6 +7,8 @@
 using bgnn_tf::MAXH;
 using bgnn_tf::f32x16;
 using bgnn_tf::tanh_fast;
+using bgnn_tf::WdDelta;
+using bgnn_tf::WD_MAXC;
 
 namespace {
 
@@ -833,7 +835,7 @@
                           const float* gates, const float* gate_const_opt,
                           float* h_s2t_0, float* h_t2s_0, float* h_s2t_1, float* h_t2s_1,
                           int64_t ldh, int64_t row_stride, float* small_ws, void* stream,
-                          int64_t n_tail_t2s = 0, int64_t n_tail_s2t = 0, const int32_t* tile_need = nullptr) {
+                          int64_t n_tail_t2s = 0, int64_t n_tail_s2t = 0, const int32_t* tile_need = nullptr, bool fuse_wd = false) {
   if (n_tail_t2s < 0 || n_tail_s2t < 0 || n_tail_t2s + n_tail_s2t > N) return BGNN_E_SHAPE;
   if (!x || !mask || (!delta && !sums) || !Wp || !bias_p || !gates || !h_s2t_0 || !h_t2s_0 || !small_ws) return BGNN_E_NULL;
   if (n_heads < 1 || n_heads > MAXH || (n_heads == 2 && (!h_s2t_1 || !h_t2s_1))) return BGNN_E_NULL;
@@ -845,9 +847,6 @@
   const int NC = n_heads * 2 * (int)ldh;
   float* wd = small_ws;
   float* gc = small_ws + NC;
-  hipLaunchKernelGGL(wd_kernel, dim3((unsigned)((NC + 2 * n_heads + 3) / 4)), dim3(256), 0, st, Wp, NC, Din, delta, sums, gates,
-                     gate_const_opt, n_heads, wd, gc);
-  BGNN_LAUNCH_CHECK();
   GemmParams p{};
   p.x = x; p.ldx = ldx; p.N = N; p.Din = Din; p.mask = mask; p.Wp = Wp; p.bias = bias_p; p.wd = wd; p.g = gates; p.gc = gc;
   p.out[0][0] = h_s2t_0; p.out[0][1] = h_t2s_0; p.out[1][0] = h_s2t_1; p.out[1][1] = h_t2s_1;
@@ -867,6 +866,14 @@
   }
   static const bool use_stream = [] { const char* e = getenv("BGNN_GEMM_STREAM"); return !e || atoi(e) != 0; }();
   p.tile_need = tile_need;
+  if (fuse_wd && sums && use_stream) {
+    GemmParams q = p;
+    q.wd = nullptr; q.gc = nullptr; q.sums = sums; q.gate_const = gate_const_opt;
+    if (bgnn_tf_stream_supported(q, 0)) return bgnn_tf_stream_launch(q, 0, st, n_cu);
+  }
+  hipLaunchKernelGGL(wd_kernel, dim3((unsigned)((NC + 2 * n_heads + 3) / 4)), dim3(256), 0, st, Wp, NC, Din, delta, sums, gates,
+                     gate_const_opt, n_heads, wd, gc);
+  BGNN_LAUNCH_CHECK();
   if (use_stream && bgnn_tf_stream_supported(p, 0)) return bgnn_tf_stream_launch(p, 0, st, n_cu);
   if (use_wreg && NC % 64 == 0 && Din <= 128) {
     const int nct = NC % 256 == 0 ? 8 : NC % 128 == 0 ? 4 : 2;
@@ -934,6 +941,18 @@
   if (!sums) return BGNN_E_NULL;
   return transform_impl(x, N, Din, ldx, mask, nullptr, sums, n_heads, D, Wp, bias_p, gates, gate_const_opt,
                         h_s2t_0, h_t2s_0, h_s2t_1, h_t2s_1, ldh, row_stride, small_ws, stream, 0, 0, tile_need_opt);
+}
+
+extern "C" int bgnn_adaptedconv_transform_fused_f32(const float* x, int64_t N, int32_t Din, int64_t ldx,
+                                                    const uint8_t* mask, const double* sums,
+                                                    int32_t n_heads, int32_t D, const float* Wp, const float* bias_p,
+                                                    const float* gates, const float* gate_const_opt,
+                                                    float* h_s2t_0, float* h_t2s_0, float* h_s2t_1, float* h_t2s_1,
+                                                    int64_t ldh, int64_t row_stride, const int32_t* tile_need_opt,
+                                                    float* small_ws, void* stream) {
+  if (!sums) return BGNN_E_NULL;
+  return transform_impl(x, N, Din, ldx, mask, nullptr, sums, n_heads, D, Wp, bias_p, gates, gate_const_opt,
+                        h_s2t_0, h_t2s_0, h_s2t_1, h_t2s_1, ldh, row_stride, small_ws, stream, 0, 0, tile_need_opt, true);
 }
 
 extern "C" int bgnn_linear_f32(const float* x, int64_t N, int32_t Din, int64_t ldx, const float* W, const float* bias,
@@ -970,14 +989,34 @@
 }
 
 namespace {
+template <bool OWN_WD>
 __global__ __launch_bounds__(256) void narrow_finish_kernel(const float* __restrict__ raw, int64_t N,
                                                             const uint8_t* __restrict__ mask,
                                                             const float* __restrict__ bias, const float* __restrict__ wd,
                                                             const float* __restrict__ gc, float* __restrict__ out_s2t,
-                                                            float* __restrict__ out_t2s, int64_t row_stride) {
+                                                            float* __restrict__ out_t2s, int64_t row_stride,
+                                                            const double* __restrict__ sums, const float* __restrict__ gate_const,
+                                                            int32_t Din) {
   const float4 b0 = *reinterpret_cast<const float4*>(bias), b1 = *reinterpret_cast<const float4*>(bias + 4);
-  const float4 w0 = *reinterpret_cast<const float4*>(wd), w1 = *reinterpret_cast<const float4*>(wd + 4);
-  const float g0 = gc[0], g1 = gc[1];
+  float4 w0, w1;
+  float g0, g1;
+  if constexpr (OWN_WD) {
+    __shared__ __attribute__((aligned(16))) float cst[12];
+    const int lane = threadIdx.x & 63, wave = threadIdx.x >> 6;
+    WdDelta wdd;
+    wdd.load(sums, Din, lane);
+    for (int j = wave; j < 10; j += 4) {
+      const float* row = j < 8 ? wd + (int64_t)j * Din : gc + (int64_t)(j - 8) * 2 * Din + Din;
+      const float acc = wdd.dot(row, Din, lane);
+      if (lane == 0) cst[j] = j < 8 ? acc : acc + (gate_const ? gate_const[j - 8] : 0.f);
+    }
+    __syncthreads();
+    w0 = *reinterpret_cast<const float4*>(cst); w1 = *reinterpret_cast<const float4*>(cst + 4);
+    g0 = cst[8]; g1 = cst[9];
+  } else {
+    w0 = *reinterpret_cast<const float4*>(wd); w1 = *reinterpret_cast<const float4*>(wd + 4);
+    g0 = gc[0]; g1 = gc[1];
+  }
   for (int64_t r = blockIdx.x * (int64_t)blockDim.x + threadIdx.x; r < N; r += (int64_t)gridDim.x * blockDim.x) {
     const float4 a = *reinterpret_cast<const float4*>(raw + r * 12);
     const float4 b = *reinterpret_cast<const float4*>(raw + r * 12 + 4);
@@ -1031,15 +1070,16 @@
   return 0;
 }
 
-extern "C" int bgnn_classifier_stage_f32(const float* x, int64_t N, int32_t Din, int64_t ldx, const uint8_t* mask,
-                                         const double* sums_x, int32_t sk_heads, int32_t sk_D, const float* sk_Wp,
-                                         const float* sk_bias, const float* sk_gates, const float* sk_gate_const_opt,
-                                         float* h_s2t_0, float* h_t2s_0, float* h_s2t_1, float* h_t2s_1, int64_t sk_ldh,
-                                         int64_t sk_row_stride, const float* W, const float* bias, int32_t Dout, int relu,
-                                         double* colsum, const float* Wp2, const float* gates2, float* raw, float* small_ws,
-                                         void* stream) {
+static int classifier_stage_impl(const float* x, int64_t N, int32_t Din, int64_t ldx, const uint8_t* mask,
+                                 const double* sums_x, int32_t sk_heads, int32_t sk_D, const float* sk_Wp,
+                                 const float* sk_bias, const float* sk_gates, const float* sk_gate_const_opt,
+                                 float* h_s2t_0, float* h_t2s_0, float* h_s2t_1, float* h_t2s_1, int64_t sk_ldh,
+                                 int64_t sk_row_stride, const float* W, const float* bias, int32_t Dout, int relu,
+                                 double* colsum, const float* Wp2, const float* gates2, float* raw, float* small_ws,
+                                 void* stream) {
+  const bool fuse_wd = small_ws == nullptr;
   if (!x || !mask || !sums_x || !sk_Wp || !sk_bias || !sk_gates || !h_s2t_0 || !h_t2s_0 || !W || !bias || !colsum || !Wp2 || !gates2 ||
-      !raw || !small_ws) return BGNN_E_NULL;
+      !raw) return BGNN_E_NULL;
   if (sk_heads < 1 || sk_heads > MAXH || (sk_heads == 2 && (!h_s2t_1 || !h_t2s_1))) return BGNN_E_NULL;
   if (N < 0 || Din <= 0 || (Din & 3) || (ldx & 3) || ldx < Din || sk_D <= 0 || sk_ldh < sk_D || (sk_ldh & 3) || (sk_row_stride & 3) ||
       sk_row_stride < sk_ldh) return BGNN_E_SHAPE;
@@ -1048,8 +1088,8 @@
   if (N == 0) return 0;
   hipStream_t st = (hipStream_t)stream;
   const int sk_NC = sk_heads * 2 * (int)sk_ldh;
-  float* wd = small_ws;
-  float* gc = small_ws + sk_NC;
+  float* wd = fuse_wd ? nullptr : small_ws;
+  float* gc = fuse_wd ? nullptr : small_ws + sk_NC;
   GemmParams p{};
   p.x = x; p.ldx = ldx; p.N = N; p.Din = Din; p.mask = mask; p.Wp = W; p.bias = bias;
   p.ldh = Dout; p.row_stride = Dout; p.NC = Dout; p.n_heads = 1; p.relu = relu ? 1 : 0; p.colsum = colsum;
@@ -1057,16 +1097,35 @@
   p.sk_Wp = sk_Wp; p.sk_bias = sk_bias; p.sk_wd = wd; p.sk_g = sk_gates; p.sk_gc = gc;
   p.sk_out[0][0] = h_s2t_0; p.sk_out[0][1] = h_t2s_0; p.sk_out[1][0] = h_s2t_1; p.sk_out[1][1] = h_t2s_1;
   p.sk_ldh = sk_ldh; p.sk_row_stride = sk_row_stride; p.sk_NC = sk_NC; p.sk_heads = sk_heads;
+  p.sums = sums_x; p.sk_gate_const = sk_gate_const_opt;
   if (!bgnn_tf_cls_supported(p)) return BGNN_E_SHAPE;
-  hipLaunchKernelGGL(wd_kernel, dim3((unsigned)((sk_NC + 2 * sk_heads + 3) / 4)), dim3(256), 0, st, sk_Wp, sk_NC, Din, (const float*)nullptr,
-                     sums_x, sk_gates, sk_gate_const_opt, sk_heads, wd, gc);
-  BGNN_LAUNCH_CHECK();
+  if (!fuse_wd) {
+    hipLaunchKernelGGL(wd_kernel, dim3((unsigned)((sk_NC + 2 * sk_heads + 3) / 4)), dim3(256), 0, st, sk_Wp, sk_NC, Din, (const float*)nullptr,
+                       sums_x, sk_gates, sk_gate_const_opt, sk_heads, wd, gc);
+    BGNN_LAUNCH_CHECK();
+  }
   static const int n_cu = [] {
     int dev = 0; hipDeviceProp_t prop;
     return (hipGetDevice(&dev) == hipSuccess && hipGetDeviceProperties(&prop, dev) == hipSuccess) ? prop.multiProcessorCount : 256;
   }();
   return bgnn_tf_cls_launch(p, st, n_cu);
 }
+
+#define BGNN_CLS_ARGS_DECL const float* x, int64_t N, int32_t Din, int64_t ldx, const uint8_t* mask, const double* sums_x, int32_t sk_heads, \
+    int32_t sk_D, const float* sk_Wp, const float* sk_bias, const float* sk_gates, const float* sk_gate_const_opt, float* h_s2t_0, \
+    float* h_t2s_0, float* h_s2t_1, float* h_t2s_1, int64_t sk_ldh, int64_t sk_row_stride, const float* W, const float* bias, int32_t Dout, \
+    int relu, double* colsum, const float* Wp2, const float* gates2, float* raw
+#define BGNN_CLS_ARGS x, N, Din, ldx, mask, sums_x, sk_heads, sk_D, sk_Wp, sk_bias, sk_gates, sk_gate_const_opt, h_s2t_0, h_t2s_0, h_s2t_1, \
+    h_t2s_1, sk_ldh, sk_row_stride, W, bias, Dout, relu, colsum, Wp2, gates2, raw
+extern "C" int bgnn_classifier_stage_f32(BGNN_CLS_ARGS_DECL, float* small_ws, void* stream) {
+  if (!small_ws) return BGNN_E_NULL;
+  return classifier_stage_impl(BGNN_CLS_ARGS, small_ws, stream);
+}
+extern "C" int bgnn_classifier_stage_fused_f32(BGNN_CLS_ARGS_DECL, void* stream) {
+  return classifier_stage_impl(BGNN_CLS_ARGS, nullptr, stream);
+}
+#undef BGNN_CLS_ARGS_DECL
+#undef BGNN_CLS_ARGS
 
 extern "C" int bgnn_narrow_transform_finish_f32(const float* raw, int64_t N, const uint8_t* mask, const double* sums,
                                                 int32_t Din, const float* Wp2, const float* bias2, const float* gates2,
@@ -1083,8 +1142,23 @@
   hipLaunchKernelGGL(wd_kernel, dim3(3), dim3(256), 0, st, Wp2, 8, Din, (const float*)nullptr, sums, gates2, gate_const_opt, 1, wd, gc);
   BGNN_LAUNCH_CHECK();
   const int64_t nb = (N + 255) / 256;
-  hipLaunchKernelGGL(narrow_finish_kernel, dim3((unsigned)(nb < 4096 ? nb : 4096)), dim3(256), 0, st, raw, N, mask, bias2, wd, gc,
-                     h_s2t, h_t2s, row_stride);
+  hipLaunchKernelGGL(narrow_finish_kernel<false>, dim3((unsigned)(nb < 4096 ? nb : 4096)), dim3(256), 0, st, raw, N, mask, bias2, wd, gc,
+                     h_s2t, h_t2s, row_stride, (const double*)nullptr, (const float*)nullptr, Din);
   BGNN_LAUNCH_CHECK();
   return 0;
 }
+
+extern "C" int bgnn_narrow_transform_finish_fused_f32(const float* raw, int64_t N, const uint8_t* mask, const double* sums,
+                                                      int32_t Din, const float* Wp2, const float* bias2, const float* gates2,
+                                                      const float* gate_const_opt, float* h_s2t, float* h_t2s,
+                                                      int64_t row_stride, void* stream) {
+  if (!raw || !mask || !sums || !Wp2 || !bias2 || !gates2 || !h_s2t || !h_t2s) return BGNN_E_NULL;
+  if (N < 0 || Din <= 0 || Din > 64 * WD_MAXC || (Din & 3) || row_stride < 4 || (row_stride & 3)) return BGNN_E_SHAPE;
+  if (!bgnn_aligned16(raw) || !bgnn_aligned16(h_s2t) || !bgnn_aligned16(h_t2s) || !bgnn_aligned16(bias2)) return BGNN_E_ALIGN;
+  if (N == 0) return 0;
+  const int64_t nb = (N + 255) / 256;
+  hipLaunchKernelGGL(narrow_finish_kernel<true>, dim3((unsigned)(nb < 2048 ? nb : 2048)), dim3(256), 0, (hipStream_t)stream, raw, N, mask,
+                     bias2, Wp2, gates2, h_s2t, h_t2s, row_stride, sums, gate_const_opt, Din);
+  BGNN_LAUNCH_CHECK();
+  return 0;
+}
diff --git a/bridged_gnn_amd/csrc/bgnn_transform_cls.hip b/bridged_gnn_amd/csrc/bgnn_transform_cls.hip
--- a/bridged_gnn_amd/csrc/bgnn_transform_cls.hip
+++ b/bridged_gnn_amd/csrc/bgnn_transform_cls.hip
@@ -7,6 +7,7 @@
 using bgnn_tf::MAXH;
 using bgnn_tf::f32x16;
 using bgnn_tf::tanh_fast;
+using bgnn_tf::WdDelta;
 
 namespace {
 
@@ -37,6 +38,7 @@
   __shared__ __attribute__((aligned(16))) float bias1[DK];
   __shared__ uint32_t wmax[3];
   __shared__ float red[2][DK + 1];
+  __shared__ float skgc[2 * MAXH];
   const int tid = threadIdx.x, lane = tid & 63;
   const int wave = __builtin_amdgcn_readfirstlane(tid >> 6);
   const int fr = lane & 31, fh = lane >> 5;
@@ -52,7 +54,24 @@
 
   if (tid < 3) wmax[tid] = 0u;
   for (int t = tid; t < 2 * (DK + 1); t += 64 * CLS_NW) (&red[0][0])[t] = 0.f;
-  if (tid < 32) { skc[0][tid] = tid < p.sk_NC ? p.sk_bias[tid] : 0.f; skc[1][tid] = tid < p.sk_NC ? p.sk_wd[tid] : 0.f; }
+  const bool own_wd = p.sk_NC > 0 && p.sk_wd == nullptr;
+  if (tid < 32) {
+    skc[0][tid] = tid < p.sk_NC ? p.sk_bias[tid] : 0.f;
+    if (!own_wd) skc[1][tid] = tid < p.sk_NC ? p.sk_wd[tid] : 0.f;
+    else if (tid >= p.sk_NC) skc[1][tid] = 0.f;
+  }
+  if (own_wd) {
+    WdDelta wdd;
+    wdd.load(p.sums, p.Din, lane);
+    for (int j = wave; j < p.sk_NC + 2 * p.sk_heads; j += CLS_NW) {
+      const float* row = j < p.sk_NC ? p.sk_Wp + (int64_t)j * p.Din : p.sk_g + (int64_t)(j - p.sk_NC) * 2 * p.Din + p.Din;
+      const float acc = wdd.dot(row, p.Din, lane);
+      if (lane == 0) {
+        if (j < p.sk_NC) skc[1][j] = acc;
+        else skgc[j - p.sk_NC] = acc + (p.sk_gate_const ? p.sk_gate_const[j - p.sk_NC] : 0.f);
+      }
+    }
+  }
   if (tid < DK) bias1[tid] = tid < NC ? p.bias[tid] : 0.f;
   __syncthreads();
   auto src_row = [&](int ct, int r) -> const float* {
@@ -147,7 +166,7 @@
   }
   float gcs[4];
 #pragma unroll
-  for (int h = 0; h < 4; ++h) gcs[h] = h < 2 * p.sk_heads ? p.sk_gc[h] : 0.f;
+  for (int h = 0; h < 4; ++h) gcs[h] = h < 2 * p.sk_heads ? (own_wd ? skgc[h] : p.sk_gc[h]) : 0.f;
 
   unsigned char* const sb = slots + wave * SLOT;
   float* const tsc = reinterpret_cast<float*>(sb);
@@ -399,7 +418,9 @@
 bool bgnn_tf_cls_supported(const GemmParams& p) {
   if (p.NC != 128 || p.Din > 128 || p.Din <= 64 || (p.Din & 3) || !p.mask || !p.w2 || !p.g2 || !p.raw) return false;
   if (p.sk_NC < 0 || p.sk_NC > 24 || (p.sk_NC & 3) || p.sk_heads < 0 || p.sk_heads > 2) return false;
-  if (p.sk_NC > 0 && (!p.sk_Wp || !p.sk_bias || !p.sk_wd || !p.sk_g || !p.sk_gc || (p.sk_ldh & 3) || p.sk_NC != p.sk_heads * 2 * p.sk_ldh)) return false;
+  if (p.sk_NC > 0 && (!p.sk_Wp || !p.sk_bias || !p.sk_g || (p.sk_ldh & 3) || p.sk_NC != p.sk_heads * 2 * p.sk_ldh)) return false;
+  if (p.sk_NC > 0 && (p.sk_wd == nullptr) != (p.sk_gc == nullptr)) return false;
+  if (p.sk_NC > 0 && !p.sk_wd && !p.sums) return false;
   return true;
 }
 
diff --git a/bridged_gnn_amd/csrc/bgnn_transform_params.h b/bridged_gnn_amd/csrc/bgnn_transform_params.h
--- a/bridged_gnn_amd/csrc/bgnn_transform_params.h
+++ b/bridged_gnn_amd/csrc/bgnn_transform_params.h
@@ -26,6 +26,29 @@
   const int32_t* tile_need;
   const float* sk_Wp; const float* sk_bias; const float* sk_wd; const float* sk_g; const float* sk_gc;
   float* sk_out[MAXH][2]; int64_t sk_ldh; int64_t sk_row_stride; int32_t sk_NC; int32_t sk_heads;
+  const double* sums; const float* gate_const; const float* sk_gate_const;
+};
+
+constexpr int WD_MAXC = 4;
+struct WdDelta {
+  float d[WD_MAXC];
+  __device__ __forceinline__ void load(const double* __restrict__ sums, int32_t Din, int lane) {
+    const double ns = sums[2 * Din], nt = sums[2 * Din + 1];
+#pragma unroll
+    for (int i = 0; i < WD_MAXC; ++i) {
+      const int c = lane + 64 * i;
+      d[i] = c < Din ? (float)(sums[c] / ns) - (float)(sums[Din + c] / nt) : 0.f;
+    }
+  }
+  __device__ __forceinline__ float dot(const float* __restrict__ row, int32_t Din, int lane) const {
+    float acc = 0.f;
+#pragma unroll
+    for (int i = 0; i < WD_MAXC; ++i) {
+      const int c = lane + 64 * i;
+      if (c < Din) acc = fmaf(row[c], d[i], acc);
+    }
+    return bgnn::group_sum<64>(acc);
+  }
 };
 
 __device__ __forceinline__ float tanh_fast(float z) { return 1.f - 2.f * __builtin_amdgcn_rcpf(__expf(2.f * z) + 1.f); }
diff --git a/bridged_gnn_amd/csrc/bgnn_transform_stream.hip b/bridged_gnn_amd/csrc/bgnn_transform_stream.hip
--- a/bridged_gnn_amd/csrc/bgnn_transform_stream.hip
+++ b/bridged_gnn_amd/csrc/bgnn_transform_stream.hip
@@ -6,6 +6,7 @@
 using bgnn_tf::GemmParams;
 using bgnn_tf::f32x16;
 using bgnn_tf::tanh_fast;
+using bgnn_tf::WdDelta;
 
 namespace {
 
@@ -117,7 +118,16 @@
       gtab[2 * k + 1] = k < p.Din ? p.g[2 * p.Din + k] : 0.f;
     }
   }
-  if constexpr (MODE == 0) { gcs[0] = p.gc[0]; gcs[1] = p.gc[1]; }
+  WdDelta wdd;
+  const bool own_wd = MODE == 0 && p.wd == nullptr;
+  if constexpr (MODE == 0) {
+    if (!own_wd) { gcs[0] = p.gc[0]; gcs[1] = p.gc[1]; }
+    else {
+      wdd.load(p.sums, p.Din, lane);
+#pragma unroll
+      for (int t = 0; t < 2; ++t) gcs[t] = wdd.dot(p.g + (int64_t)t * 2 * p.Din + p.Din, p.Din, lane) + (p.gate_const ? p.gate_const[t] : 0.f);
+    }
+  }
   __syncthreads();
   const bool din_full = p.Din == DK;
   int woff[GPW][CPT], xoff[GPW][CPT], moff[GPW], coff[GPW];
@@ -277,7 +287,15 @@
     const int ld2 = 2 * (int)p.ldh;
     const int h = col_base / ld2, rem = col_base % ld2, t = rem >= p.ldh ? 1 : 0;
     bias_n = p.bias[n];
-    if constexpr (MODE == 0) wd_n = p.wd[n];
+    if constexpr (MODE == 0) {
+      if (!own_wd) wd_n = p.wd[n];
+      else {
+        for (int j = 0; j < 32; ++j) {
+          const float acc = wdd.dot(p.Wp + (int64_t)(col_base + j) * p.Din, p.Din, lane);
+          wd_n = fr == j ? acc : wd_n;
+        }
+      }
+    }
     otab = h == 0 ? (t == 0 ? p.out[0][0] : p.out[0][1]) : (t == 0 ? p.out[1][0] : p.out[1][1]);
     ooff = (int)((4 * fh * p.row_stride + (rem - t * (int)p.ldh) + fr) * 4);
     if constexpr (MODE == 0) my_table = __builtin_amdgcn_readfirstlane(t);
@@ -936,6 +954,7 @@
   if (mode != 0) return false;
   if (p.n_heads != 1 || p.Din > 128 || p.Din <= 64 || (p.Din & 3) || (p.ldh & 31)) return false;
   if (p.NC != 2 * p.ldh || (p.NC != 256 && p.NC != 128) || p.col_off != 0) return false;
+  if ((p.wd == nullptr) != (p.gc == nullptr) || (!p.wd && !p.sums)) return false;
   if (p.ldx * 4 * 32 > 0x7fffffff || p.row_stride * 4 * 36 > 0x7fffffff) return false;
   return true;
 }
diff --git a/bridged_gnn_amd/ktgnn.py b/bridged_gnn_amd/ktgnn.py
--- a/bridged_gnn_amd/ktgnn.py
+++ b/bridged_gnn_amd/ktgnn.py
@@ -716,8 +716,7 @@
             logits_hat = self.clf_target(xt.contiguous(), None, central_mask=central_mask, csr=csr)
             return (F.log_softmax(logits_base, dim=1), F.log_softmax(logits_target, dim=1),
                     F.log_softmax(logits_hat, dim=1), None)
-        t2s = torch.empty(x.shape[0], 3 * stage.ld, dtype=torch.float32, device=x.device)
-        s2t = torch.empty_like(t2s)
+        t2s, s2t = ops.table_pair(x.shape[0], 3 * stage.ld, x.device)
         stage.eval_tables(x, mask_u8, sums_h, stage.views(t2s, s2t), self._arena)
         a_t2s, a_s2t = stage.attention()
         out3 = ops.adaptedconv_aggregate(t2s, s2t, a_t2s, a_s2t, csr, mask_u8, stage.C, stage.slope, heads=3,
diff --git a/bridged_gnn_amd/ops.py b/bridged_gnn_amd/ops.py
--- a/bridged_gnn_amd/ops.py
+++ b/bridged_gnn_amd/ops.py
@@ -239,31 +239,39 @@
             and os.environ.get("BGNN_FUSED_CLS", "1") != "0")
 
 
-def classifier_stage(x, mask_u8, sums_x, packed_pair, outs, weight, bias, colsum, packed_t, relu=True):
+def classifier_stage(x, mask_u8, sums_x, packed_pair, outs, weight, bias, colsum, packed_t, relu=True, fused=True):
     N, din = x.shape
     Wp, bp, gates, D, ldh, gconst = packed_pair
     H = gates.shape[0]
     Wp2, _, gates2, _, _, _ = packed_t
     raw = torch.empty(N, 12, dtype=torch.float32, device=x.device)
-    small = torch.empty(H * (2 * ldh + 2) + 8, dtype=torch.float32, device=x.device)
     row_stride = outs[0][0].stride(0)
     for a, b in outs:
         assert a.shape[0] >= N and b.shape[0] >= N and a.stride(0) == row_stride and b.stride(0) == row_stride
     o1 = outs[1] if H > 1 else (None, None)
-    rc = L.lib().bgnn_classifier_stage_f32(L.ptr_rows(x), N, din, x.stride(0), L.ptr(mask_u8), L.ptr(sums_x), H, D, L.ptr(Wp), L.ptr(bp),
-                                           L.ptr(gates), L.ptr(gconst), L.ptr_rows(outs[0][1]), L.ptr_rows(outs[0][0]),
-                                           L.ptr_rows(o1[1]), L.ptr_rows(o1[0]), ldh, row_stride, L.ptr(weight), L.ptr(bias),
-                                           weight.shape[0], 1 if relu else 0, L.ptr(colsum), L.ptr(Wp2), L.ptr(gates2), L.ptr(raw),
-                                           L.ptr(small), L.stream())
-    L.check(rc, "bgnn_classifier_stage_f32")
+    args = (L.ptr_rows(x), N, din, x.stride(0), L.ptr(mask_u8), L.ptr(sums_x), H, D, L.ptr(Wp), L.ptr(bp),
+            L.ptr(gates), L.ptr(gconst), L.ptr_rows(outs[0][1]), L.ptr_rows(outs[0][0]),
+            L.ptr_rows(o1[1]), L.ptr_rows(o1[0]), ldh, row_stride, L.ptr(weight), L.ptr(bias),
+            weight.shape[0], 1 if relu else 0, L.ptr(colsum), L.ptr(Wp2), L.ptr(gates2), L.ptr(raw))
+    if fused:
+        L.check(L.lib().bgnn_classifier_stage_fused_f32(*args, L.stream()), "bgnn_classifier_stage_fused_f32")
+        return raw
+    small = torch.empty(H * (2 * ldh + 2) + 8, dtype=torch.float32, device=x.device)
+    L.check(L.lib().bgnn_classifier_stage_f32(*args, L.ptr(small), L.stream()), "bgnn_classifier_stage_f32")
     return raw
 
 
-def narrow_transform_finish(raw, mask_u8, sums, packed, out):
+def narrow_transform_finish(raw, mask_u8, sums, packed, out, fused=True):
     Wp, bp, gates, D, ldh, gconst = packed
     h_t2s, h_s2t = out
     N = raw.shape[0]
     assert h_t2s.stride(0) == h_s2t.stride(0) and sums.dtype == torch.float64 and sums.numel() == 2 * Wp.shape[1] + 2
+    if fused and Wp.shape[1] <= 256:
+        rc = L.lib().bgnn_narrow_transform_finish_fused_f32(L.ptr(raw), N, L.ptr(mask_u8), L.ptr(sums), Wp.shape[1], L.ptr(Wp), L.ptr(bp),
+                                                            L.ptr(gates), L.ptr(gconst), L.ptr_rows(h_s2t), L.ptr_rows(h_t2s),
+                                                            h_t2s.stride(0), L.stream())
+        L.check(rc, "bgnn_narrow_transform_finish_fused_f32")
+        return out
     small = torch.empty(16, dtype=torch.float32, device=raw.device)
     rc = L.lib().bgnn_narrow_transform_finish_f32(L.ptr(raw), N, L.ptr(mask_u8), L.ptr(sums), Wp.shape[1], L.ptr(Wp), L.ptr(bp),
                                                   L.ptr(gates), L.ptr(gconst), L.ptr_rows(h_s2t), L.ptr_rows(h_t2s),
@@ -461,15 +469,20 @@
     return Wp, bp, gates, D, ldh, gconst
 
 
-def adaptedconv_transform(x, mask_u8, delta, packed, out=None, sums=None, tail_single=(0, 0), tile_need=None):
+def table_pair(n_rows, width, device):
+    per = (int(n_rows) * int(width) + 63) // 64 * 64
+    buf = torch.empty(2 * per, dtype=torch.float32, device=device)
+    return buf[:n_rows * width].view(n_rows, width), buf[per: per + n_rows * width].view(n_rows, width)
+
+
+def adaptedconv_transform(x, mask_u8, delta, packed, out=None, sums=None, tail_single=(0, 0), tile_need=None, fused=True):
     lib = L.lib()
     Wp, bp, gates, D, ldh, gconst = packed
     H = gates.shape[0]
     N, Din = x.shape
     dev = x.device
     if out is None:
-        out = [(torch.empty(N, ldh, dtype=torch.float32, device=dev), torch.empty(N, ldh, dtype=torch.float32, device=dev))
-               for _ in range(H)]
+        out = [table_pair(N, ldh, dev) for _ in range(H)]
     row_stride = out[0][0].stride(0)
     for a, b in out:
         assert a.shape[0] >= N and b.shape[0] >= N and a.stride(0) == row_stride and b.stride(0) == row_stride
@@ -490,6 +503,8 @@
         if tile_need.dtype != torch.int32 or tile_need.numel() != (N + 31) // 32:
             raise ValueError("tile_need: one int32 per 32-row tile")
         fn, name, tail = lib.bgnn_adaptedconv_transform_need_f32, "bgnn_adaptedconv_transform_need_f32", (L.ptr(tile_need),)
+    if fused and delta is None and (tile_need is not None or tail == (0, 0)):
+        fn, name, tail = lib.bgnn_adaptedconv_transform_fused_f32, "bgnn_adaptedconv_transform_fused_f32", (L.ptr(tile_need),)
     rc = fn(L.ptr(x), N, Din, x.stride(0), L.ptr(mask_u8), L.ptr(first), H, D, L.ptr(Wp), L.ptr(bp), L.ptr(gates), L.ptr(gconst),
             L.ptr_rows(out[0][1]), L.ptr_rows(out[0][0]), L.ptr_rows(o1[1]), L.ptr_rows(o1[0]), ldh, row_stride, *tail,
             L.ptr(small), L.stream())
@@ -500,8 +515,32 @@
 _P2_STATIC = os.environ.get("BGNN_P2_STATIC", "1") != "0"
 
 
+TILE_QUEUE_WORDS = 64
+_TILE_QUEUES = {}
+_TILE_QUEUE_SPARES = {}
+
+
 def _tile_queue(dev):
     return torch.empty(8, dtype=torch.int32, device=dev)
+
+
+def _stream_tile_queue(dev):
+    dev = torch.device(dev)
+    idx = dev.index if dev.index is not None else torch.cuda.current_device()
+    capturing = torch.cuda.is_current_stream_capturing()
+    key = (idx, torch.cuda.current_stream(dev).cuda_stream, capturing)
+    q = _TILE_QUEUES.get(key)
+    if q is not None:
+        return q
+    spares = _TILE_QUEUE_SPARES.setdefault(idx, [])
+    if capturing:
+        q = spares.pop() if spares else torch.zeros(TILE_QUEUE_WORDS, dtype=torch.int32, device=dev)
+    else:
+        q = torch.zeros(TILE_QUEUE_WORDS, dtype=torch.int32, device=dev)
+        while len(spares) < 2:
+            spares.append(torch.zeros(TILE_QUEUE_WORDS, dtype=torch.int32, device=dev))
+    _TILE_QUEUES[key] = q
+    return q
 
 
 def heads_log_softmax_supported(heads, D):
@@ -528,9 +567,9 @@
         out = torch.empty(n_dst, heads * ldo, dtype=torch.float32, device=dev)
     assert h_t2s.stride(0) == h_s2t.stride(0) and h_t2s.stride(0) % heads == 0 and out.stride(0) % heads == 0
     alpha = torch.empty(csr.num_edges, dtype=torch.float32, device=dev) if want_alpha else None
-    tq = _tile_queue(dev) if heads == 1 else None
     if row_end <= int(row_begin):
         return (out, alpha) if want_alpha else out
+    tq = _stream_tile_queue(dev) if heads == 1 else None
     if ((not want_alpha or heads == 1) and part in (0, 3) and int(row_begin) == 0 and row_end == csr.num_nodes == n_dst and h_t2s.shape[0] == n_dst
             and (ep_scale is None or heads == 1) and _hub_shape_ok(D, ldh, out.stride(0) // heads, heads, negative_slope)
             and os.environ.get("BGNN_HUB_ROWS", "1") != "0"):
@@ -540,23 +579,23 @@
             nseg = int(seg_node.numel())
             wsb = lib.bgnn_aggregate_hub_workspace_bytes(nseg, heads, out.stride(0) // heads)
             ws = torch.empty(wsb, dtype=torch.uint8, device=dev)
-            rc = lib.bgnn_adaptedconv_aggregate_hub_f32(
+            rc = lib.bgnn_adaptedconv_aggregate_hub_queued_f32(
                 L.ptr_rows(h_t2s), L.ptr_rows(h_s2t), ldh, L.ptr(a_t2s), L.ptr(a_s2t), L.ptr(csr.rowptr), L.ptr(csr.col),
                 L.ptr(mask_u8), n_dst, D, float(negative_slope), L.ptr_rows(out), out.stride(0) // heads,
                 L.ptr(ep_scale), L.ptr(ep_shift), 2 if log_softmax else (1 if ep_relu else 0),
                 L.ptr(state_ms) if part == 3 else None, int(heads), L.ptr(colsum),
                 L.ptr(tq), HUB_THRESHOLD, L.ptr(hub_rows), int(hub_rows.numel()),
                 L.ptr(seg_ptr), L.ptr(seg_bounds), L.ptr(seg_node), nseg, L.ptr(alpha), L.ptr(ws), wsb, L.stream())
-            L.check(rc, "bgnn_adaptedconv_aggregate_hub_f32")
+            L.check(rc, "bgnn_adaptedconv_aggregate_hub_queued_f32")
             return (out, alpha) if want_alpha else out
-    rc = lib.bgnn_adaptedconv_aggregate_bounded_f32(
+    rc = lib.bgnn_adaptedconv_aggregate_queued_f32(
         L.ptr_rows(h_t2s), L.ptr_rows(h_s2t), ldh, L.ptr(a_t2s), L.ptr(a_s2t), L.ptr(csr.rowptr), L.ptr(csr.col),
         L.ptr(mask_u8), int(row_begin), row_end, D, float(negative_slope), L.ptr_rows(out), out.stride(0) // heads, L.ptr(alpha),
         L.ptr(ep_scale), L.ptr(ep_shift), 2 if log_softmax else (1 if ep_relu else 0), L.ptr(state_ms), int(part),
         int(row_begin) if park_begin is None else int(park_begin), int(heads), L.ptr(colsum),
         L.ptr(tq) if not (part == 2 and _P2_STATIC) else None, min(int(h_t2s.shape[0]), int(h_s2t.shape[0])),
         csr.gather_hint() if (heads == 1 and D > 32 and part == 0) else 0, L.stream())
-    L.check(rc, "bgnn_adaptedconv_aggregate_bounded_f32")
+    L.check(rc, "bgnn_adaptedconv_aggregate_queued_f32")
     return (out, alpha) if want_alpha else out
 
 
diff --git a/include/bgnn.h b/include/bgnn.h
--- a/include/bgnn.h
+++ b/include/bgnn.h
@@ -46,6 +46,16 @@
                                      int32_t Din, const float* Wp2, const float* bias2, const float* gates2,
                                      const float* gate_const_opt, float* h_s2t, float* h_t2s, int64_t row_stride,
                                      float* small_ws, void* stream);
+int bgnn_classifier_stage_fused_f32(const float* x, int64_t N, int32_t Din, int64_t ldx, const uint8_t* mask,
+                                    const double* sums_x, int32_t sk_heads, int32_t sk_D, const float* sk_Wp,
+                                    const float* sk_bias, const float* sk_gates, const float* sk_gate_const_opt,
+                                    float* h_s2t_0, float* h_t2s_0, float* h_s2t_1, float* h_t2s_1, int64_t sk_ldh,
+                                    int64_t sk_row_stride, const float* W, const float* bias, int32_t Dout, int relu,
+                                    double* colsum, const float* Wp2, const float* gates2, float* raw, void* stream);
+int bgnn_narrow_transform_finish_fused_f32(const float* raw, int64_t N, const uint8_t* mask, const double* sums,
+                                           int32_t Din, const float* Wp2, const float* bias2, const float* gates2,
+                                           const float* gate_const_opt, float* h_s2t, float* h_t2s, int64_t row_stride,
+                                           void* stream);
 size_t bgnn_gram_workspace_bytes(int32_t p, int32_t q);
 int bgnn_gram_f32(const float* A, int64_t lda, int32_t p, const float* B, int64_t ldb, int32_t q, int64_t N,
                   float* out , void* ws, size_t ws_bytes, void* stream);
@@ -107,6 +117,13 @@
                                         float* h_s2t_0, float* h_t2s_0, float* h_s2t_1, float* h_t2s_1,
                                         int64_t ldh, int64_t row_stride, const int32_t* tile_need_opt,
                                         float* small_ws, void* stream);
+int bgnn_adaptedconv_transform_fused_f32(const float* x, int64_t N, int32_t Din, int64_t ldx,
+                                         const uint8_t* mask, const double* sums,
+                                         int32_t n_heads, int32_t D, const float* Wp, const float* bias_p,
+                                         const float* gates, const float* gate_const_opt,
+                                         float* h_s2t_0, float* h_t2s_0, float* h_s2t_1, float* h_t2s_1,
+                                         int64_t ldh, int64_t row_stride, const int32_t* tile_need_opt,
+                                         float* small_ws, void* stream);
 
 int bgnn_adaptedconv_aggregate_f32(const float* h_t2s, const float* h_s2t, int64_t ldh,
                                    const float* a_t2s, const float* a_s2t,
@@ -125,6 +142,26 @@
                                            const float* ep_scale_opt, const float* ep_shift_opt, int ep_relu,
                                            float* state_ms_opt, int part, int64_t park_begin, int32_t heads, double* colsum_opt,
                                            uint32_t* tile_queue_opt, int64_t table_rows, int32_t gather_hint, void* stream);
+
+#define BGNN_TILE_QUEUE_WORDS 64
+int bgnn_adaptedconv_aggregate_queued_f32(const float* h_t2s, const float* h_s2t, int64_t ldh,
+                                          const float* a_t2s, const float* a_s2t,
+                                          const int32_t* rowptr, const int32_t* col, const uint8_t* mask,
+                                          int64_t row_begin, int64_t row_end, int32_t D, float negative_slope,
+                                          float* out, int64_t ldo, float* alpha_opt,
+                                          const float* ep_scale_opt, const float* ep_shift_opt, int ep_relu,
+                                          float* state_ms_opt, int part, int64_t park_begin, int32_t heads, double* colsum_opt,
+                                          uint32_t* tile_queue_opt, int64_t table_rows, int32_t gather_hint, void* stream);
+int bgnn_adaptedconv_aggregate_hub_queued_f32(const float* h_t2s, const float* h_s2t, int64_t ldh,
+                                              const float* a_t2s, const float* a_s2t,
+                                              const int32_t* rowptr, const int32_t* col, const uint8_t* mask,
+                                              int64_t N, int32_t D, float negative_slope, float* out, int64_t ldo,
+                                              const float* ep_scale_opt, const float* ep_shift_opt, int ep_relu,
+                                              float* state_ms_opt, int32_t heads, double* colsum_opt,
+                                              uint32_t* tile_queue_opt, int32_t hub_threshold, const int32_t* hub_rows,
+                                              int64_t n_hubs, const int32_t* hub_seg_ptr, const int32_t* seg_bounds,
+                                              const int32_t* seg_node, int64_t n_segments, float* alpha_opt,
+                                              void* ws, size_t ws_bytes, void* stream);
 
 size_t bgnn_aggregate_hub_workspace_bytes(int64_t n_segments, int32_t heads, int64_t ldo);
 int bgnn_adaptedconv_aggregate_hub_f32(const float* h_t2s, const float* h_s2t, int64_t ldh,
```

Measured after the change: 49.35 billion edges/s. 2.0% lower.
